# arpg/NID-Pose-Estimation

Hardware: NVIDIA B200
Metric: NID cost+Jacobian evals/s @640x480 (higher is better)
Workload: dtype f64

## Files before the change

### nid-pose-estimation_b200/csrc/nid_api.cu

```cuda
#include <math.h>
#include <stdio.h>
#include <string.h>

#include <algorithm>
#include <limits>
#include <string>
#include <chrono>
#include <vector>

#include "../host/nid_host_math.hpp"
#include "nid_ctx.h"

namespace nid {

static thread_local std::string g_err;
void set_error(const std::string& s) { g_err = s; }
int check_cuda(cudaError_t e, const char* what) {
  if (e == cudaSuccess) return NID_OK;
  g_err = std::string(what) + ": " + cudaGetErrorString(e);
  return NID_ERR_CUDA;
}

#define CU(call, what)                                   \
  do {                                                   \
    cudaError_t e_ = (call);                             \
    if (e_ != cudaSuccess) return check_cuda(e_, what);  \
  } while (0)
#define OKR(call)               \
  do {                          \
    int r_ = (call);            \
    if (r_ != NID_OK) return r_; \
  } while (0)

static int strips_for(const nid_ctx* c, int n_jobs) {
  int S;
  if (c->opt_force_strips > 0) S = std::min(c->opt_force_strips, c->rb);
  else {
    long long want = 2LL * c->sm_count;
    long long per = (long long)c->ncell * n_jobs;
    S = (int)((want + per - 1) / per);
    S = std::max(1, std::min(S, std::min(c->rb, 32)));
  }
  if (c->part_slots > 0 && n_jobs > 0) S = (int)std::max<size_t>(1, std::min<size_t>((size_t)S, c->part_slots / (size_t)n_jobs));
  return S;
}

EvalParams make_params(nid_ctx* c, int n_jobs) {
  EvalParams p;
  memset(&p, 0, sizeof(p));
  p.rows = c->rows; p.cols = c->cols; p.cell = c->cell; p.bins = c->bins;
  p.rb = c->rb; p.cb = c->cb; p.N = c->N; p.ncell = c->ncell;
  p.S = strips_for(c, n_jobs);
  p.strip_rows = (c->rb + p.S - 1) / p.S;
  p.hist_stride = c->bins * c->bins + c->bins;
  p.pwx = c->pwx; p.pwy = c->pwy; p.pwz = c->pwz;
  p.im0 = c->im0; p.im1 = c->im1; p.inb0 = c->inb0;
  p.n_c = c->n_c; p.href = c->href; p.cam = c->cam;
  p.lut_w = c->lut_w; p.lut_k = c->lut_k;
  p.poses = c->poses; p.job_pair = c->job_pair;
  const bool sorted = use_sorted(c);
  p.part = c->part; p.jpart = sorted ? c->jpart_s : c->jpart; p.hist = c->opt_keep_hist ? c->hist : nullptr;
  p.ht = c->ht; p.hj = c->hj; p.err = c->err; p.der = c->der; p.gn = c->gn;
  p.sd0 = c->sd0; p.sd1 = c->sd1; p.sd2 = c->sd2; p.sid = c->sid;
  p.stage_bulk = (c->opt_stage_bulk < 0 ? (long long)c->rb * c->cb < NID_SMALL_CELL_PX : c->opt_stage_bulk) ? 1 : 0;
  p.sl_off = c->sl_off; p.sl_task = c->sl_task; p.sl_desc = c->sl_desc; p.task_cls = c->task_cls; p.sl_cell = c->sl_cell; p.nslices = c->nslices;
  p.sell_cap = c->sell_cap; p.max_slices = c->max_slices; p.Twc0 = c->Twc0;
  p.tasks = c->tasks; p.ntasks = c->ntasks; p.cell_task_start = c->cell_task_start; p.cell_slice_start = c->cell_slice_start;
  p.cls_task_start = c->cls_task_start; p.span_start = c->span_start; p.wv = c->wv;
  p.max_tasks = c->max_tasks; p.g_stride = (int)c->g_stride;
  p.G = c->G; p.fp1 = c->fp1; p.tex2 = c->d_tex2; p.k1tex = c->d_k1tex;
  return p;
}

bool use_sorted(const nid_ctx* c) {
  if (c->bins > NID_SORTED_MAX_BINS || c->bins < NID_SORTED_MIN_BINS) return false;
  if (c->opt_path == 1) return false;
  return true;
}

template <typename T>
static int dalloc(T** p, size_t n, const char* what) {
  cudaError_t e = cudaMalloc((void**)p, sizeof(T) * (n ? n : 1));
  if (e != cudaSuccess) return check_cuda(e, what);
  return NID_OK;
}

int ensure_job_buffers(nid_ctx* c) {
  const size_t J = c->job_cap, NC = c->ncell;
  const size_t hs = (size_t)c->bins * c->bins + c->bins;
  if (c->opt_keep_hist && !c->hist) OKR(dalloc(&c->hist, J * NC * hs, "hist"));
  if (use_sorted(c)) {
    const size_t need = (size_t)std::max(c->max_ntasks_prepared, 1);
    if (c->g_stride < need) {
      CU(cudaStreamSynchronize(c->stream), "sync before growing job buffers");
      if (c->G) cudaFree(c->G);
      c->G = nullptr;
      OKR(dalloc(&c->G, J * need * c->bins, "G"));
      c->g_stride = need;
    }
    if (!c->jpart_s) OKR(dalloc(&c->jpart_s, J * (size_t)c->max_slices * 6, "jpart_s"));
    if (!c->wv) {
      OKR(dalloc(&c->wv, J * NC * (size_t)nid::wv_stride(c->bins), "wv"));
      CU(cudaMemset(c->wv, 0, sizeof(double) * J * NC * (size_t)nid::wv_stride(c->bins)), "memset wv");
    }
  } else if (!c->part) {
    c->part_slots = J + 2 * (size_t)c->sm_count + 64;
    OKR(dalloc(&c->part, c->part_slots * NC * hs, "part"));
    OKR(dalloc(&c->jpart, c->part_slots * NC * 6, "jpart"));
  }
  return NID_OK;
}

static int update_textures(nid_ctx* c, int pair0, int n) {
  for (int i = 0; i < n; i++) c->k1_ready[pair0 + i] = 0;
  for (int p0 = pair0; p0 < pair0 + n; p0 += c->setup_batch) {
    const int nb = std::min(c->setup_batch, pair0 + n - p0);
    OKR(launch_pack(c, p0, nb));
    for (int i = 0; i < nb; i++)
      CU(cudaMemcpy2DToArrayAsync(c->tex2_arrays[p0 + i], 0, 0, c->d_pack + (size_t)i * c->N, sizeof(unsigned) * c->cols,
                                  sizeof(unsigned) * c->cols, c->rows, cudaMemcpyDeviceToDevice, c->stream), "packed im1 -> texture array");
  }
  return NID_OK;
}
static int update_texture(nid_ctx* c, int pair) { return update_textures(c, pair, 1); }

static int arena_take(nid_ctx* c, size_t bytes, void** out) {
  bytes = (bytes + 63) & ~(size_t)63;
  if (bytes > c->h_arena_cap) {
    CU(cudaStreamSynchronize(c->stream), "sync before growing the staging arena");
    if (c->h_arena) cudaFreeHost(c->h_arena);
    c->h_arena = nullptr; c->h_arena_cap = 0; c->h_arena_used = 0;
    const size_t cap = std::max(bytes * 4, (size_t)1 << 20);
    CU(cudaMallocHost((void**)&c->h_arena, cap), "pinned staging arena");
    c->h_arena_cap = cap;
  }
  if (c->h_arena_used + bytes > c->h_arena_cap) {
    CU(cudaStreamSynchronize(c->stream), "sync to recycle the staging arena");
    c->h_arena_used = 0;
  }
  *out = c->h_arena + c->h_arena_used;
  c->h_arena_used += bytes;
  return NID_OK;
}

static int stage_jobs(nid_ctx* c, int n_jobs, const int* job_pair, const double* poses, int mode = 0) {
  if (n_jobs < 1 || n_jobs > c->max_jobs) { set_error("n_jobs out of range"); return NID_ERR_ARG; }
  for (int j = 0; j < n_jobs; j++) {
    int pr = job_pair ? job_pair[j] : 0;
    if (pr < 0 || pr >= c->n_pairs) { set_error("job_pair out of range"); return NID_ERR_ARG; }
    if (mode == 1) {
      if (!c->pair_set[pr]) { set_error("job_pair invalid or pair not set"); return NID_ERR_ARG; }
      continue;
    }
    if (!c->pair_prepared[pr]) { set_error("pair not prepared (call nid_prepare)"); return NID_ERR_STATE; }
    if (use_sorted(c) && !c->pair_sorted[pr]) {
      set_error("pair not prepared for the sorted path (call nid_prepare after selecting the path)");
      return NID_ERR_STATE;
    }
  }
  const int slot = (c->stage_slot + 1) % NID_STAGE_RING;
  CU(cudaEventSynchronize(c->stage_ev[slot]), "wait for the staging slot");
  c->stage_slot = slot;
  c->h_poses = c->h_poses_ring + (size_t)slot * 16 * c->job_cap;
  c->h_job_pair = c->h_job_pair_ring + (size_t)slot * c->job_cap;
  for (int j = 0; j < n_jobs; j++) c->h_job_pair[j] = job_pair ? job_pair[j] : 0;
  memcpy(c->h_poses, poses, sizeof(double) * 16 * n_jobs);
  CU(cudaMemcpyAsync(c->poses, c->h_poses, sizeof(double) * 16 * n_jobs, cudaMemcpyHostToDevice, c->stream), "H2D poses");
  CU(cudaMemcpyAsync(c->job_pair, c->h_job_pair, sizeof(int) * n_jobs, cudaMemcpyHostToDevice, c->stream), "H2D job_pair");
  CU(cudaEventRecord(c->stage_ev[slot], c->stream), "record staging event");
  c->staged_jobs = n_jobs;
  return NID_OK;
}

static int fetch(nid_ctx* c, int n_jobs, int want_jac, double* Ht, double* Hj, double* der) {
  const size_t nc = (size_t)n_jobs * c->ncell;
  double* h = c->h_out;
  if (Ht) CU(cudaMemcpyAsync(h, c->ht, sizeof(double) * nc, cudaMemcpyDeviceToHost, c->stream), "D2H ht");
  if (Hj) CU(cudaMemcpyAsync(h + nc, c->hj, sizeof(double) * nc, cudaMemcpyDeviceToHost, c->stream), "D2H hj");
  if (want_jac && der) CU(cudaMemcpyAsync(h + 2 * nc, c->der, sizeof(double) * 6 * nc, cudaMemcpyDeviceToHost, c->stream), "D2H der");
  CU(cudaStreamSynchronize(c->stream), "sync");
  if (Ht) memcpy(Ht, h, sizeof(double) * nc);
  if (Hj) memcpy(Hj, h + nc, sizeof(double) * nc);
  if (want_jac && der) memcpy(der, h + 2 * nc, sizeof(double) * 6 * nc);
  return NID_OK;
}

}

using namespace nid;

extern "C" {

const char* nid_last_error(void) { return g_err.c_str(); }
int nid_version(void) { return 100; }

int nid_create(nid_ctx** out, int device, int rows, int cols, int cell, int bins, int degree, int n_pairs, int max_jobs) {
  cudaGetLastError();
  if (!out) { set_error("ctx out pointer is NULL"); return NID_ERR_ARG; }
  *out = nullptr;
  if (degree != 3) { set_error("only bs_degree == 3 (order-4 B-splines) is supported, as in the reference"); return NID_ERR_UNSUPPORTED; }
  if (rows > 65535 || cols > 65535) { set_error("rows, cols must be < 65536"); return NID_ERR_ARG; }
  if (cell > 90) { set_error("cell must be <= 90 (the task descriptors keep the cell index in 13 bits)"); return NID_ERR_ARG; }
  if (rows < 8 || cols < 8 || cell < 1 || bins < 6 || bins > 64 || n_pairs < 1 || max_jobs < 1 || cell > rows || cell > cols) {
    set_error("bad geometry (need rows,cols>=8, 1<=cell<=min(rows,cols), 6<=bins<=64, n_pairs,max_jobs>=1)");
    return NID_ERR_ARG;
  }
  int ndev = 0;
  cudaError_t e = cudaGetDeviceCount(&ndev);
  if (e != cudaSuccess || ndev == 0) {
    set_error(std::string("no CUDA device: ") + cudaGetErrorString(e) + " (this library has no CPU path)");
    return NID_ERR_CUDA;
  }
  if (device < 0 || device >= ndev) { set_error("device index out of range"); return NID_ERR_ARG; }
  CU(cudaSetDevice(device), "cudaSetDevice");
  nid_ctx* c = new nid_ctx();
  c->device = device; c->rows = rows; c->cols = cols; c->cell = cell; c->bins = bins; c->degree = degree;
  c->N = rows * cols; c->ncell = cell * cell; c->rb = rows / cell; c->cb = cols / cell;
  c->n_pairs = n_pairs; c->max_jobs = max_jobs;
  c->job_cap = std::max(max_jobs, NID_MIN_JOB_SLOTS);
  cudaDeviceProp prop;
  CU(cudaGetDeviceProperties(&prop, device), "cudaGetDeviceProperties");
  c->sm_count = prop.multiProcessorCount;
  CU(cudaStreamCreateWithFlags(&c->stream, cudaStreamNonBlocking), "cudaStreamCreate");
  const size_t N = c->N, P = n_pairs, J = c->job_cap, NC = c->ncell;
  const size_t hs = (size_t)bins * bins + bins;
  OKR(dalloc(&c->pwx, P * N, "pwx")); OKR(dalloc(&c->pwy, P * N, "pwy")); OKR(dalloc(&c->pwz, P * N, "pwz"));
  OKR(dalloc(&c->im0, P * N, "im0")); OKR(dalloc(&c->im1, P * N, "im1")); OKR(dalloc(&c->inb0, P * N, "inb0"));
  OKR(dalloc(&c->n_c, P * NC, "n_c")); OKR(dalloc(&c->href, P * NC, "href"));
  OKR(dalloc(&c->cam, P * 4, "cam")); OKR(dalloc(&c->Twc0, P * 16, "Twc0"));
  OKR(dalloc(&c->cnt, P * NC * NID_NCLS, "cnt"));
  c->task_px = (long long)c->rb * c->cb < NID_SMALL_CELL_PX ? 16 : 32;
  const int min_task_px = 8;
  c->max_tasks = (int)(N / min_task_px + NC * NID_NCLS + 1);
  c->max_slices = c->max_tasks / 32 + (int)NC + 1;
  c->sell_cap = (N + 3 * (size_t)c->max_tasks + NC * 32 * (size_t)(NID_TASK_PX_MAX + 4) + 255) / 128 * 128;
  OKR(dalloc(&c->depth, P * N, "depth"));
  OKR(dalloc(&c->sl_off, P * ((size_t)c->max_slices + 1), "sl_off"));
  OKR(dalloc(&c->sl_task, P * (size_t)c->max_slices * 32, "sl_task"));
  OKR(dalloc(&c->sl_desc, P * (size_t)c->max_slices * 32, "sl_desc"));
  OKR(dalloc(&c->task_cls, P * (size_t)c->max_tasks, "task_cls"));
  OKR(dalloc(&c->sl_cell, P * (size_t)c->max_slices, "sl_cell"));
  OKR(dalloc(&c->task_pos, P * (size_t)c->max_tasks, "task_pos"));
  OKR(dalloc(&c->nslices, P, "nslices"));
  CU(cudaMemset(c->nslices, 0, sizeof(int) * P), "memset nslices");
  c->h_nslices.assign(P, 0);
  OKR(dalloc(&c->tasks, P * (size_t)c->max_tasks, "tasks"));
  OKR(dalloc(&c->ntasks, P, "ntasks"));
  CU(cudaMemset(c->ntasks, 0, sizeof(int) * P), "memset ntasks");
  OKR(dalloc(&c->cell_task_start, P * (NC + 1), "cell_task_start"));
  OKR(dalloc(&c->cell_slice_start, P * (NC + 1), "cell_slice_start"));
  OKR(dalloc(&c->cls_task_start, P * NC * (NID_NCLS + 1), "cls_task_start"));
  {
    const int NS = bins - 3;
    std::vector<int> ss(NS + 1, 256);
    auto kr = [bins](int v) { double o = v >= 255 ? 254.999 : (double)v; return (int)std::floor(o * (bins - 3) / 255.0); };
    for (int v = 255; v >= 0; v--)
      for (int k = 0; k <= kr(v) && k <= NS; k++) ss[k] = v;
    ss[NS] = 256;
    OKR(dalloc(&c->span_start, ss.size(), "span_start"));
    CU(cudaMemcpy(c->span_start, ss.data(), sizeof(int) * ss.size(), cudaMemcpyHostToDevice), "H2D span_start");
  }
  c->h_ntasks.assign(P, 0);
  {
    bool ok = true;
    c->tex2_arrays.assign(P, nullptr);
    c->h_tex2.assign(P, 0);
    cudaChannelFormatDesc cd2 = cudaCreateChannelDesc<unsigned int>();
    for (size_t i = 0; i < P && ok; i++) {
      if (cudaMallocArray(&c->tex2_arrays[i], &cd2, cols, rows, cudaArrayTextureGather) != cudaSuccess) { ok = false; break; }
      cudaResourceDesc rd;
      memset(&rd, 0, sizeof(rd));
      rd.resType = cudaResourceTypeArray;
      rd.res.array.array = c->tex2_arrays[i];
      cudaTextureDesc td;
      memset(&td, 0, sizeof(td));
      td.addressMode[0] = td.addressMode[1] = cudaAddressModeClamp;
      td.filterMode = cudaFilterModePoint;
      td.readMode = cudaReadModeElementType;
      td.normalizedCoords = 0;
      if (cudaCreateTextureObject(&c->h_tex2[i], &rd, &td, nullptr) != cudaSuccess) ok = false;
    }
    if (!ok) {
      cudaGetLastError();
      set_error("could not create the packed gather textures for the target images");
      return NID_ERR_CUDA;
    }
    OKR(dalloc(&c->d_tex2, P, "d_tex2"));
    OKR(dalloc(&c->d_k1tex, P, "d_k1tex"));
    CU(cudaMemset(c->d_k1tex, 0, sizeof(cudaTextureObject_t) * P), "memset k1tex");
    c->k1_arrays.assign(P, nullptr);
    c->h_k1tex.assign(P, 0);
    c->k1_ready.assign(P, 0);
    CU(cudaMemcpy(c->d_tex2, c->h_tex2.data(), sizeof(cudaTextureObject_t) * P, cudaMemcpyHostToDevice), "H2D tex2 handles");
    c->setup_batch = (int)std::min<size_t>(P, 32);
    OKR(dalloc(&c->d_pack, N * (size_t)c->setup_batch, "d_pack"));
    OKR(dalloc(&c->lay_tot, (size_t)c->setup_batch * NC * 3, "lay_tot"));
    OKR(dalloc(&c->lay_base, (size_t)c->setup_batch * NC * 3, "lay_base"));
    OKR(dalloc(&c->prep_poses, (size_t)c->setup_batch * 16, "prep_poses"));
    OKR(dalloc(&c->depth_factor, P, "depth_factor"));
    c->pair_u16.assign(P, 0);
    OKR(dalloc(&c->fp1, P * N, "fp1"));
    c->h_Twc0.assign(P * 16, 0.0);
    c->h_cam.assign(P * 4, 1.0);
  }
  OKR(dalloc(&c->d_depth, N, "d_depth")); OKR(dalloc(&c->d_img64, N, "d_img64")); OKR(dalloc(&c->d_flag, 2, "d_flag"));
  CU(cudaMemset(c->d_flag, 0, sizeof(int) * 2), "memset flag");
  OKR(dalloc(&c->lut_w, 256 * 4, "lut_w")); OKR(dalloc(&c->lut_k, 256, "lut_k"));
  OKR(dalloc(&c->poses, J * 16, "poses")); OKR(dalloc(&c->job_pair, J, "job_pair"));
  CU(cudaMemset(c->job_pair, 0, sizeof(int) * J), "memset job_pair");
  CU(cudaMemset(c->poses, 0, sizeof(double) * 16 * J), "memset poses");
  OKR(dalloc(&c->aux_pose, 16, "aux_pose"));
  (void)hs;
  OKR(dalloc(&c->ht, J * NC, "ht")); OKR(dalloc(&c->hj, J * NC, "hj")); OKR(dalloc(&c->err, J * NC, "err"));
  OKR(dalloc(&c->der, J * NC * 6, "der")); OKR(dalloc(&c->gn, J * 44, "gn"));
  OKR(dalloc(&c->hard, J * (NC + 1), "hard"));
  CU(cudaMallocHost((void**)&c->h_poses_ring, sizeof(double) * 16 * J * NID_STAGE_RING), "pinned poses");
  CU(cudaMallocHost((void**)&c->h_job_pair_ring, sizeof(int) * J * NID_STAGE_RING), "pinned job_pair");
  memset(c->h_poses_ring, 0, sizeof(double) * 16 * J * NID_STAGE_RING);
  memset(c->h_job_pair_ring, 0, sizeof(int) * J * NID_STAGE_RING);
  c->h_poses = c->h_poses_ring;
  c->h_job_pair = c->h_job_pair_ring;
  for (int i = 0; i < NID_STAGE_RING; i++) CU(cudaEventCreateWithFlags(&c->stage_ev[i], cudaEventDisableTiming), "cudaEventCreate (staging)");
  CU(cudaMallocHost((void**)&c->h_aux_pose, sizeof(double) * 16), "pinned aux pose");
  CU(cudaMallocHost((void**)&c->h_out, sizeof(double) * J * (NC * 8 + 44)), "pinned out");
  c->pair_set.assign(P, 0);
  c->pair_prepared.assign(P, 0);
  c->pair_sorted.assign(P, 0);
  OKR(launch_build_lut(c));
  OKR(sorted_init(c));
  CU(cudaStreamSynchronize(c->stream), "sync after lut");
  *out = c;
  return NID_OK;
}

int nid_destroy(nid_ctx* c) {
  if (!c) return NID_OK;
  cudaSetDevice(c->device);
  cudaStreamSynchronize(c->stream);
  void* ptrs[] = {c->pwx, c->pwy, c->pwz, c->im0, c->im1, c->inb0, c->n_c, c->href, c->cam, c->Twc0, c->cnt, c->d_depth,
                  c->d_img64, c->d_flag, c->d_pix, c->d_pix4, c->d_pix4_jobs, c->chunk_cnt, c->d_bsv, c->d_bsi, c->lut_w, c->lut_k, c->poses,
                  c->job_pair, c->aux_pose, c->part, c->jpart, c->hist, c->ht, c->hj, c->err, c->der, c->gn, c->hard,
                  c->depth, c->sd0, c->sd1, c->sd2, c->sid, c->sl_off, c->sl_task, c->sl_desc, c->task_cls, c->sl_cell, c->nslices, c->task_pos,
                  c->lay_tot, c->lay_base, c->prep_poses, c->depth16, c->depth_factor, c->d_tex2, c->d_pack, c->tasks, c->ntasks, c->cell_task_start, c->cell_slice_start, c->G, c->jpart_s, c->fp1, c->cls_task_start, c->span_start, c->wv};
  for (auto t : c->h_k1tex) if (t) cudaDestroyTextureObject(t);
  for (auto arr : c->k1_arrays) if (arr) cudaFreeArray(arr);
  if (c->d_k1tex) cudaFree(c->d_k1tex);
  if (c->d_k1pack) cudaFree(c->d_k1pack);
  for (auto t : c->h_tex2) if (t) cudaDestroyTextureObject(t);
  for (auto arr : c->tex2_arrays) if (arr) cudaFreeArray(arr);
  for (void* p : ptrs) if (p) cudaFree(p);
  if (c->h_poses_ring) cudaFreeHost(c->h_poses_ring);
  if (c->h_job_pair_ring) cudaFreeHost(c->h_job_pair_ring);
  if (c->h_aux_pose) cudaFreeHost(c->h_aux_pose);
  if (c->h_lm_lists) cudaFreeHost(c->h_lm_lists);
  destroy_latency_graph(c);
  if (c->h_lm_stage) cudaFreeHost(c->h_lm_stage);
  if (c->d_lm_stage) cudaFree(c->d_lm_stage);
  if (c->d_lm_lists) cudaFree(c->d_lm_lists);
  for (int i = 0; i < NID_STAGE_RING; i++) if (c->stage_ev[i]) cudaEventDestroy(c->stage_ev[i]);
  if (c->h_out) cudaFreeHost(c->h_out);
  if (c->h_arena) cudaFreeHost(c->h_arena);
  if (c->h_res) cudaFreeHost(c->h_res);
  for (int i = 0; i < 2; i++) if (c->ev[i]) cudaEventDestroy(c->ev[i]);
  for (int i = 0; i < 2; i++) if (c->ds_ev[i]) cudaEventDestroy(c->ds_ev[i]);
  for (int i = 0; i < 5; i++) if (c->kev[i]) cudaEventDestroy(c->kev[i]);
  cudaStreamDestroy(c->stream);
  if (c->stream2) cudaStreamDestroy(c->stream2);
  delete c;
  return NID_OK;
}

int nid_sync(nid_ctx* c) {
  if (!c) { set_error("NULL ctx"); return NID_ERR_ARG; }
  CU(cudaSetDevice(c->device), "cudaSetDevice");
  CU(cudaStreamSynchronize(c->stream), "nid_sync");
  c->h_arena_used = 0;
  return NID_OK;
}

static int set_pairs_geometry(nid_ctx* c, int pair0, int n, const double* depth64, const uint16_t* depth16, const double* T_wc0,
                              const double* intr) {
  if (pair0 < 0 || n < 1 || pair0 + n > c->n_pairs) { set_error("pair range out of bounds"); return NID_ERR_ARG; }
  if ((!depth64 && !depth16) || !T_wc0 || !intr) { set_error("NULL argument"); return NID_ERR_ARG; }
  CU(cudaSetDevice(c->device), "cudaSetDevice");
  const size_t N = c->N;
  if (depth16) {
    if (!c->depth16) OKR(dalloc(&c->depth16, (size_t)c->n_pairs * N, "depth16"));
    CU(cudaMemcpyAsync(c->depth16 + (size_t)pair0 * N, depth16, sizeof(uint16_t) * N * n, cudaMemcpyDefault, c->stream), "H2D depth (u16)");
  } else {
    CU(cudaMemcpyAsync(c->depth + (size_t)pair0 * N, depth64, sizeof(double) * N * n, cudaMemcpyDefault, c->stream), "H2D depth");
  }
  double* a = nullptr;
  OKR(arena_take(c, sizeof(double) * 21 * n, (void**)&a));
  double *aT = a, *acam = a + 16 * (size_t)n, *afac = a + 20 * (size_t)n;
  memcpy(aT, T_wc0, sizeof(double) * 16 * n);
  for (int i = 0; i < n; i++) {
    memcpy(acam + 4 * i, intr + 5 * (size_t)i, sizeof(double) * 4);
    afac[i] = intr[5 * (size_t)i + 4];
  }
  CU(cudaMemcpyAsync(c->Twc0 + 16 * (size_t)pair0, aT, sizeof(double) * 16 * n, cudaMemcpyHostToDevice, c->stream), "H2D Twc0");
  CU(cudaMemcpyAsync(c->cam + 4 * (size_t)pair0, acam, sizeof(double) * 4 * n, cudaMemcpyHostToDevice, c->stream), "H2D intr");
  CU(cudaMemcpyAsync(c->depth_factor + pair0, afac, sizeof(double) * n, cudaMemcpyHostToDevice, c->stream), "H2D depth factor");
  memcpy(c->h_Twc0.data() + 16 * (size_t)pair0, aT, sizeof(double) * 16 * n);
  memcpy(c->h_cam.data() + 4 * (size_t)pair0, acam, sizeof(double) * 4 * n);
  OKR(launch_points(c, pair0, n, depth16 != nullptr));
  for (int i = 0; i < n; i++) { c->pair_prepared[pair0 + i] = 0; c->pair_u16[pair0 + i] = depth16 ? 1 : 0; }
  return NID_OK;
}
static int set_pair_common(nid_ctx* c, int pair, const double* depth, const double T_wc0[16], const double intr[5]) {
  if (pair < 0 || pair >= c->n_pairs) { set_error("pair index out of range"); return NID_ERR_ARG; }
  return set_pairs_geometry(c, pair, 1, depth, nullptr, T_wc0, intr);
}

int nid_set_pair(nid_ctx* c, int pair, const double* depth, const uint8_t* im0, const uint8_t* im1, const double T_wc0[16],
                 const double intr[5]) {
  if (!c) { set_error("NULL ctx"); return NID_ERR_ARG; }
  if (!im0 || !im1) { set_error("NULL image"); return NID_ERR_ARG; }
  OKR(set_pair_common(c, pair, depth, T_wc0, intr));
  CU(cudaMemcpyAsync(c->im0 + (size_t)pair * c->N, im0, c->N, cudaMemcpyDefault, c->stream), "H2D im0");
  CU(cudaMemcpyAsync(c->im1 + (size_t)pair * c->N, im1, c->N, cudaMemcpyDefault, c->stream), "H2D im1");
  OKR(update_texture(c, pair));
  CU(cudaStreamSynchronize(c->stream), "sync set_pair");
  c->pair_set[pair] = 1;
  return NID_OK;
}

int nid_set_pairs_u16(nid_ctx* c, int pair0, int n, const uint16_t* depth_raw, const uint8_t* im0, const uint8_t* im1,
                      const double* T_wc0, const double* intr) {
  if (!c) { set_error("NULL ctx"); return NID_ERR_ARG; }
  if (!im0 || !im1 || !depth_raw) { set_error("NULL image"); return NID_ERR_ARG; }
  if (c->sell_points) { set_error("this context holds caller-supplied world points (nid_set_pair_points)"); return NID_ERR_STATE; }
  OKR(set_pairs_geometry(c, pair0, n, nullptr, depth_raw, T_wc0, intr));
  const size_t N = c->N;
  CU(cudaMemcpyAsync(c->im0 + (size_t)pair0 * N, im0, N * n, cudaMemcpyDefault, c->stream), "H2D im0");
  CU(cudaMemcpyAsync(c->im1 + (size_t)pair0 * N, im1, N * n, cudaMemcpyDefault, c->stream), "H2D im1");
  OKR(update_textures(c, pair0, n));
  for (int i = 0; i < n; i++) c->pair_set[pair0 + i] = 1;
  return NID_OK;
}

int nid_set_pairs_downsampled(nid_ctx* dst, int dst_pair0, const nid_ctx* src, int src_pair0, int n) {
  if (!dst || !src) { set_error("NULL context"); return NID_ERR_ARG; }
  if (dst->rows != src->rows / 2 || dst->cols != src->cols / 2) {
    set_error("destination geometry must be (source rows / 2, source cols / 2)");
    return NID_ERR_ARG;
  }
  if (n < 1 || n > dst->n_pairs || n > src->n_pairs || dst_pair0 < 0 || src_pair0 < 0 || dst_pair0 > dst->n_pairs - n ||
      src_pair0 > src->n_pairs - n) {
    set_error("pair range out of bounds");
    return NID_ERR_ARG;
  }
  if (dst->device != src->device) { set_error("source and destination contexts live on different devices"); return NID_ERR_ARG; }
  if (src->sell_points || dst->sell_points) {
    set_error("downsampling needs depth pairs on both sides, not caller-supplied world points (nid_set_pair_points)");
    return NID_ERR_STATE;
  }
  for (int i = 0; i < n; i++)
    if (!src->pair_set[src_pair0 + i]) { set_error("source pair not set"); return NID_ERR_STATE; }
  CU(cudaSetDevice(dst->device), "cudaSetDevice");
  for (int i = 0; i < 2; i++)
    if (!dst->ds_ev[i]) CU(cudaEventCreateWithFlags(&dst->ds_ev[i], cudaEventDisableTiming), "cudaEventCreate (downsample)");
  double* a = nullptr;
  OKR(arena_take(dst, sizeof(double) * 5 * n, (void**)&a));
  double *acam = a, *afac = a + 4 * (size_t)n;
  for (int i = 0; i < n; i++) {
    const double* k = src->h_cam.data() + 4 * (size_t)(src_pair0 + i);
    acam[4 * i] = k[0] * 0.5; acam[4 * i + 1] = k[1] * 0.5;
    acam[4 * i + 2] = (k[2] - 0.5) * 0.5; acam[4 * i + 3] = (k[3] - 0.5) * 0.5;
    afac[i] = 1.0;
  }
  CU(cudaEventRecord(dst->ds_ev[0], src->stream), "record source event");
  CU(cudaStreamWaitEvent(dst->stream, dst->ds_ev[0], 0), "wait for the source");
  CU(cudaMemcpyAsync(dst->cam + 4 * (size_t)dst_pair0, acam, sizeof(double) * 4 * n, cudaMemcpyHostToDevice, dst->stream), "H2D intr");
  CU(cudaMemcpyAsync(dst->depth_factor + dst_pair0, afac, sizeof(double) * n, cudaMemcpyHostToDevice, dst->stream), "H2D depth factor");
  CU(cudaMemcpyAsync(dst->Twc0 + 16 * (size_t)dst_pair0, src->Twc0 + 16 * (size_t)src_pair0, sizeof(double) * 16 * n,
                     cudaMemcpyDeviceToDevice, dst->stream), "D2D Twc0");
  memcpy(dst->h_cam.data() + 4 * (size_t)dst_pair0, acam, sizeof(double) * 4 * n);
  memcpy(dst->h_Twc0.data() + 16 * (size_t)dst_pair0, src->h_Twc0.data() + 16 * (size_t)src_pair0, sizeof(double) * 16 * n);
  OKR(launch_downsample2(dst, dst_pair0, src, src_pair0, n));
  OKR(launch_points(dst, dst_pair0, n, false));
  OKR(update_textures(dst, dst_pair0, n));
  CU(cudaEventRecord(dst->ds_ev[1], dst->stream), "record destination event");
  CU(cudaStreamWaitEvent(src->stream, dst->ds_ev[1], 0), "order the source after the kernel");
  for (int i = 0; i < n; i++) {
    dst->pair_set[dst_pair0 + i] = 1;
    dst->pair_prepared[dst_pair0 + i] = 0;
    dst->pair_u16[dst_pair0 + i] = 0;
  }
  return NID_OK;
}

int nid_set_target(nid_ctx* c, int pair, const uint8_t* im1) {
  if (!c || !im1) { set_error("bad argument"); return NID_ERR_ARG; }
  if (pair < 0 || pair >= c->n_pairs) { set_error("pair index out of range"); return NID_ERR_ARG; }
  if (!c->pair_set[pair]) { set_error("pair not set (nid_set_target replaces the target of an existing pair)"); return NID_ERR_STATE; }
  CU(cudaSetDevice(c->device), "cudaSetDevice");
  CU(cudaMemcpyAsync(c->im1 + (size_t)pair * c->N, im1, c->N, cudaMemcpyDefault, c->stream), "H2D im1");
  OKR(update_texture(c, pair));
  CU(cudaStreamSynchronize(c->stream), "sync set_target");
  c->pair_prepared[pair] = 0;
  return NID_OK;
}

static int upload_images_f64(nid_ctx* c, int pair, const double* im0, const double* im1);
static int build_sorted_layout(nid_ctx* c, int pair0, int n);
static int finish_sorted_layout(nid_ctx* c, int pair0, int n, int* bs_counter, double* Href);

int nid_set_pair_f64(nid_ctx* c, int pair, const double* depth, const double* im0, const double* im1,
                     const double T_wc0[16], const double intr[5]) {
  if (!c) { set_error("NULL ctx"); return NID_ERR_ARG; }
  OKR(set_pair_common(c, pair, depth, T_wc0, intr));
  OKR(upload_images_f64(c, pair, im0, im1));
  c->pair_set[pair] = 1;
  return NID_OK;
}

static int upload_images_f64(nid_ctx* c, int pair, const double* im0, const double* im1) {
  CU(cudaMemsetAsync(c->d_flag, 0, sizeof(int), c->stream), "memset flag");
  if (im0) {
    CU(cudaMemcpyAsync(c->d_img64, im0, sizeof(double) * c->N, cudaMemcpyDefault, c->stream), "H2D im0 f64");
    OKR(launch_check_integral(c, c->d_img64, c->im0 + (size_t)pair * c->N, 1));
  }
  if (im1) {
    CU(cudaMemcpyAsync(c->d_img64, im1, sizeof(double) * c->N, cudaMemcpyDefault, c->stream), "H2D im1 f64");
    OKR(launch_check_integral(c, c->d_img64, c->im1 + (size_t)pair * c->N, 0));
    OKR(update_texture(c, pair));
  }
  int flag = 0;
  CU(cudaMemcpyAsync(&flag, c->d_flag, sizeof(int), cudaMemcpyDeviceToHost, c->stream), "D2H flag");
  CU(cudaStreamSynchronize(c->stream), "sync upload images");
  if (flag) {
    set_error("image holds non-8-bit values (non-integral or outside [0,255]); only 8-bit gray is supported");
    return NID_ERR_UNSUPPORTED;
  }
  return NID_OK;
}

int nid_set_pair_points(nid_ctx* c, int pair, const double* points_3d, const double* im0, const double* im1,
                        const double intr[5]) {
  if (!c || pair < 0 || pair >= c->n_pairs) { set_error("bad argument"); return NID_ERR_ARG; }
  CU(cudaSetDevice(c->device), "cudaSetDevice");
  if (points_3d) {
    if (!intr) { set_error("intr required with points"); return NID_ERR_ARG; }
    if (!c->d_pix) OKR(dalloc(&c->d_pix, (size_t)8 * c->N, "d_pix"));
    CU(cudaMemcpyAsync(c->d_pix, points_3d, sizeof(double) * 3 * c->N, cudaMemcpyDefault, c->stream), "H2D points3d");
    CU(cudaMemcpyAsync(c->cam + 4 * pair, intr, sizeof(double) * 4, cudaMemcpyDefault, c->stream), "H2D intr");
    memcpy(c->h_cam.data() + 4 * (size_t)pair, intr, sizeof(double) * 4);
    OKR(launch_points_soa(c, pair, c->d_pix));
    c->pair_prepared[pair] = 0;
    if (!c->sell_points) {
      CU(cudaStreamSynchronize(c->stream), "sync before switching to the point form");
      c->sell_points = true;
      std::fill(c->pair_prepared.begin(), c->pair_prepared.end(), 0);
    }
  }
  OKR(upload_images_f64(c, pair, im0, im1));
  c->pair_set[pair] = 1;
  return NID_OK;
}

int nid_import_prepare(nid_ctx* c, int pair, const double* bs_value, const int* bs_counter, const double* Href) {
  if (!c || pair < 0 || pair >= c->n_pairs || !bs_value || !bs_counter || !Href) { set_error("bad argument"); return NID_ERR_ARG; }
  if (!c->pair_set[pair]) { set_error("pair not set"); return NID_ERR_STATE; }
  CU(cudaSetDevice(c->device), "cudaSetDevice");
  if (!c->d_bsv) { OKR(dalloc(&c->d_bsv, (size_t)4 * c->N, "d_bsv")); OKR(dalloc(&c->d_bsi, (size_t)c->N, "d_bsi")); }
  CU(cudaMemcpyAsync(c->d_bsv, bs_value, sizeof(double) * 4 * c->N, cudaMemcpyDefault, c->stream), "H2D bs_value");
  OKR(launch_import_flags(c, pair, c->d_bsv));
  CU(cudaMemcpyAsync(c->n_c + pair * c->ncell, bs_counter, sizeof(int) * c->ncell, cudaMemcpyDefault, c->stream), "H2D n_c");
  CU(cudaMemcpyAsync(c->href + pair * c->ncell, Href, sizeof(double) * c->ncell, cudaMemcpyDefault, c->stream), "H2D href");
  CU(cudaMemsetAsync(c->cnt + (size_t)pair * c->ncell * NID_NCLS, 0, sizeof(unsigned int) * c->ncell * NID_NCLS, c->stream), "memset cnt");
  OKR(launch_count_classes(c, pair));
  OKR(build_sorted_layout(c, pair, 1));
  OKR(finish_sorted_layout(c, pair, 1, nullptr, nullptr));
  c->pair_prepared[pair] = 1;
  return NID_OK;
}

int nid_get_inbounds(nid_ctx* c, int pair, uint8_t* flags) {
  if (!c || pair < 0 || pair >= c->n_pairs || !flags) { set_error("bad argument"); return NID_ERR_ARG; }
  if (!c->pair_prepared[pair]) { set_error("pair not prepared"); return NID_ERR_STATE; }
  CU(cudaSetDevice(c->device), "cudaSetDevice");
  CU(cudaMemcpyAsync(flags, c->inb0 + (size_t)pair * c->N, c->N, cudaMemcpyDefault, c->stream), "D2H inb0");
  CU(cudaStreamSynchronize(c->stream), "sync inb0");
  return NID_OK;
}

int nid_get_points3d(nid_ctx* c, int pair, double* points_3d) {
  if (!c || pair < 0 || pair >= c->n_pairs || !points_3d) { set_error("bad argument"); return NID_ERR_ARG; }
  if (!c->pair_set[pair]) { set_error("pair not set"); return NID_ERR_STATE; }
  CU(cudaSetDevice(c->device), "cudaSetDevice");
  if (!c->d_pix) OKR(dalloc(&c->d_pix, (size_t)8 * c->N, "d_pix"));
  OKR(launch_points_aos(c, pair, c->d_pix));
  CU(cudaMemcpyAsync(points_3d, c->d_pix, sizeof(double) * 3 * c->N, cudaMemcpyDefault, c->stream), "copy points3d");
  CU(cudaStreamSynchronize(c->stream), "sync points3d");
  return NID_OK;
}

static int build_sorted_layout(nid_ctx* c, int pair0, int n) {
  for (int i = 0; i < n; i++) c->pair_sorted[pair0 + i] = 0;
  if (!use_sorted(c)) return NID_OK;
  if (!c->sd0) {
    OKR(dalloc(&c->sd0, (size_t)c->n_pairs * c->sell_cap, "sd0"));
    OKR(dalloc(&c->sid, (size_t)c->n_pairs * c->sell_cap, "sid"));
  }
  if (c->sell_points && !c->sd1) {
    OKR(dalloc(&c->sd1, (size_t)c->n_pairs * c->sell_cap, "sd1"));
    OKR(dalloc(&c->sd2, (size_t)c->n_pairs * c->sell_cap, "sd2"));
  }
  if (!c->chunk_cnt) {
    const size_t nchunks = ((size_t)c->rb * c->cb + 255) / 256;
    OKR(dalloc(&c->chunk_cnt, (size_t)c->setup_batch * c->ncell * nchunks * NID_NCLS, "chunk_cnt"));
  }
  for (int p0 = pair0; p0 < pair0 + n; p0 += c->setup_batch)
    OKR(launch_layout_and_scatter(c, p0, std::min(c->setup_batch, pair0 + n - p0)));
  return NID_OK;
}

static int finish_sorted_layout(nid_ctx* c, int pair0, int n, int* bs_counter, double* Href) {
  const size_t NC = c->ncell;
  const size_t bytes = (size_t)n * (NC * (sizeof(double) + sizeof(int)) + 2 * sizeof(int)) + sizeof(int) + 64;
  if (c->h_res_cap < bytes) {
    CU(cudaStreamSynchronize(c->stream), "sync before growing the result buffer");
    if (c->h_res) cudaFreeHost(c->h_res);
    c->h_res = nullptr; c->h_res_cap = 0;
    CU(cudaMallocHost((void**)&c->h_res, bytes * 2), "pinned prepare results");
    c->h_res_cap = bytes * 2;
  }
  double* h_href = (double*)c->h_res;
  int* h_nc = (int*)(h_href + (size_t)n * NC);
  int* h_nt = h_nc + (size_t)n * NC;
  int* h_ns = h_nt + n;
  int* h_ovf = h_ns + n;
  CU(cudaMemcpyAsync(h_nc, c->n_c + (size_t)pair0 * NC, sizeof(int) * NC * n, cudaMemcpyDeviceToHost, c->stream), "D2H n_c");
  CU(cudaMemcpyAsync(h_href, c->href + (size_t)pair0 * NC, sizeof(double) * NC * n, cudaMemcpyDeviceToHost, c->stream), "D2H href");
  const bool sorted = use_sorted(c);
  if (sorted) {
    CU(cudaMemcpyAsync(h_nt, c->ntasks + pair0, sizeof(int) * n, cudaMemcpyDeviceToHost, c->stream), "D2H ntasks");
    CU(cudaMemcpyAsync(h_ns, c->nslices + pair0, sizeof(int) * n, cudaMemcpyDeviceToHost, c->stream), "D2H nslices");
    CU(cudaMemcpyAsync(h_ovf, c->d_flag + 1, sizeof(int), cudaMemcpyDeviceToHost, c->stream), "D2H overflow flag");
  }
  CU(cudaStreamSynchronize(c->stream), "sync prepare");
  c->h_arena_used = 0;
  if (sorted) {
    if (*h_ovf) { set_error("sliced pixel store overflow"); return NID_ERR_STATE; }
    for (int i = 0; i < n; i++) {
      c->h_ntasks[pair0 + i] = h_nt[i];
// ... 624 lines not shown
```

### nid-pose-estimation_b200/csrc/nid_ctx.h

```cpp
#pragma once
#include <cuda_runtime.h>
#include <stdint.h>
#include <string>
#include <vector>

#include "../../include/nid_b200.h"

#define NID_NCLS 257
#define NID_SORTED_MIN_BINS 6
#define NID_SORTED_MAX_BINS 40
#define NID_STAGE_RING 4
#define NID_MIN_JOB_SLOTS 8
#define NID_TASK_PX_MAX 256

namespace nid {

struct EvalParams {
  int rows, cols, cell, bins, rb, cb, N, ncell;
  int job0;
  const int* job_list;
  int S;
  int strip_rows;
  int hist_stride;
  const double* pwx;
  const double* pwy;
  const double* pwz;
  const uint8_t* im0;
  const uint8_t* im1;
  const uint8_t* inb0;
  const int* n_c;
  const double* href;
  const double* cam;
  const double* lut_w;
  const int* lut_k;
  const double* poses;
  const int* job_pair;
  double* part;
  double* jpart;
  double* hist;
  double* ht;
  double* hj;
  double* err;
  double* der;
  double* gn;
  double huber_delta;
  double huber_dsqr;
  const double* sd0;
  const double* sd1;
  const double* sd2;
  const unsigned* sid;
  int stage_bulk;
  const int* sl_off;
  const int* sl_task;
  const int* sl_desc;
  const unsigned short* task_cls;
  const int* sl_cell;
  const int* nslices;
  size_t sell_cap;
  int max_slices;
  const double* Twc0;
  const int2* tasks;
  const int* ntasks;
  const int* cell_task_start;
  const int* cell_slice_start;
  const int* cls_task_start;
  const int* span_start;
  double* wv;
  int max_tasks;
  int g_stride;
  double* G;
  const unsigned* fp1;
  const cudaTextureObject_t* tex2;
  const cudaTextureObject_t* k1tex;
};

}

namespace nid { struct LatencyGraph; }
struct nid_ctx {
  int device = 0;
  int rows = 0, cols = 0, cell = 0, bins = 0, degree = 3;
  int N = 0, ncell = 0, rb = 0, cb = 0;
  int n_pairs = 0, max_jobs = 0;
  int job_cap = 0;
  int sm_count = 148;
  cudaStream_t stream = nullptr;
  int* chunk_cnt = nullptr;
  int setup_batch = 1;
  int* lay_tot = nullptr;
  int* lay_base = nullptr;
  double* prep_poses = nullptr;
  uint16_t* depth16 = nullptr;
  double* depth_factor = nullptr;
  std::vector<char> pair_u16;
  char* h_arena = nullptr;
  size_t h_arena_cap = 0, h_arena_used = 0;
  char* h_res = nullptr;
  size_t h_res_cap = 0;
  cudaStream_t stream2 = nullptr;
  long long launches = 0;

  double *pwx = nullptr, *pwy = nullptr, *pwz = nullptr;
  uint8_t *im0 = nullptr, *im1 = nullptr, *inb0 = nullptr;
  int* n_c = nullptr;
  double* href = nullptr;
  double* cam = nullptr;
  double* Twc0 = nullptr;
  unsigned int* cnt = nullptr;
  double* depth = nullptr;
  double *sd0 = nullptr, *sd1 = nullptr, *sd2 = nullptr;
  unsigned* sid = nullptr;
  size_t sell_cap = 0;
  int* sl_desc = nullptr;
  unsigned short* task_cls = nullptr;
  int *sl_off = nullptr, *sl_task = nullptr, *sl_cell = nullptr, *nslices = nullptr, *task_pos = nullptr;
  int max_slices = 0;
  std::vector<int> h_nslices;
  int max_nslices_prepared = 0;
  int task_px = 32;
  bool sell_points = false;
  int2* tasks = nullptr;
  int* ntasks = nullptr;
  int* cell_task_start = nullptr;
  int* cell_slice_start = nullptr;
  int* cls_task_start = nullptr;
  int* span_start = nullptr;
  double* wv = nullptr;
  int max_tasks = 0;
  std::vector<int> h_ntasks;
  int max_ntasks_prepared = 0;
  double *G = nullptr, *jpart_s = nullptr;
  std::vector<cudaArray_t> tex2_arrays;
  std::vector<cudaTextureObject_t> h_tex2;
  cudaTextureObject_t* d_tex2 = nullptr;
  std::vector<cudaArray_t> k1_arrays;
  std::vector<cudaTextureObject_t> h_k1tex;
  cudaTextureObject_t* d_k1tex = nullptr;
  std::vector<char> k1_ready;
  unsigned short* d_k1pack = nullptr;
  unsigned* fp1 = nullptr;
  std::vector<double> h_Twc0, h_cam;
  unsigned* d_pack = nullptr;
  size_t g_stride = 0;
  int opt_path = 0;
  int opt_keep_hist = 0;
  std::vector<char> pair_set, pair_prepared, pair_sorted;
  double* d_depth = nullptr;
  double* d_img64 = nullptr;
  int* d_flag = nullptr;
  double* d_pix = nullptr;
  float* d_pix4 = nullptr;
  float* d_pix4_jobs = nullptr;
  double* d_bsv = nullptr;
  int* d_bsi = nullptr;
  double* lut_w = nullptr;
  int* lut_k = nullptr;
  double* poses = nullptr;
  int* job_pair = nullptr;
  double *part = nullptr, *jpart = nullptr, *hist = nullptr;
  double *ht = nullptr, *hj = nullptr, *err = nullptr, *der = nullptr, *gn = nullptr;
  double* hard = nullptr;
  size_t part_slots = 0;
  double* h_poses = nullptr;
  int* h_job_pair = nullptr;
  double* h_poses_ring = nullptr;
  int* h_job_pair_ring = nullptr;
  cudaEvent_t stage_ev[NID_STAGE_RING] = {};
  int stage_slot = 0;
  int staged_jobs = 0;
  double* h_aux_pose = nullptr;
  double* aux_pose = nullptr;
  double* h_out = nullptr;
  int opt_force_strips = 0;
  int* h_lm_lists = nullptr;
  int* d_lm_lists = nullptr;
  void* h_lm_stage = nullptr;
  void* d_lm_stage = nullptr;
  nid::LatencyGraph* lm_graph = nullptr;
  const void* last_hist_func = nullptr;
  const void* last_jac_func = nullptr;
  int opt_lm_graph = 1;
  int opt_stage_bulk = -1;
  int opt_asm_wide = 1;
  int opt_lm_spec = 4;
  int opt_lm_reuse = 1;
  double* lm_trace = nullptr;
  int lm_trace_cap = 0;
  cudaEvent_t ev[2] = {nullptr, nullptr};
  cudaEvent_t ds_ev[2] = {nullptr, nullptr};
  int opt_time_kernels = 0;
  cudaEvent_t kev[5] = {nullptr, nullptr, nullptr, nullptr, nullptr};
  double kernel_ms[4] = {0, 0, 0, 0};
  long long kernel_calls[4] = {0, 0, 0, 0};
};

namespace nid {
#define NID_FEW_BINS(bins) ((bins) <= 20)
#ifndef NID_SMALL_CELL_PX
#define NID_SMALL_CELL_PX 2560
#endif
__host__ __device__ inline int wv_row(int B) { return NID_FEW_BINS(B) ? B + 1 : B; }
__host__ __device__ inline int wv_stride(int B) { return (B * wv_row(B) + B + 1) & ~1; }
__host__ __device__ inline int job_at(const EvalParams& p, int i) { return p.job_list ? p.job_list[p.job0 + i] : p.job0 + i; }
#ifdef __CUDACC__
__device__ __forceinline__ void huber_weights(double ec, double dsqr, double delta, double& rho0, double& rho1) {
  const double chi = ec * ec;
  if (chi <= dsqr) { rho0 = chi; rho1 = 1.0; }
  else { const double sq = sqrt(chi); rho0 = 2 * sq * delta - dsqr; rho1 = delta / sq; }
}
__device__ __forceinline__ void gn_accumulate(double& acc, const double* e, const double* r0, const double* r1, const double* act,
                                              const double* J, int n, int ent) {
  if (ent == 0) {
    for (int c = 0; c < n; c++) acc += r0[c];
  } else if (ent <= 36) {
    const int i = (ent - 1) / 6, j = (ent - 1) % 6;
    for (int c = 0; c < n; c++) acc += J[6 * c + i] * r1[c] * J[6 * c + j];
  } else if (ent <= 42) {
    const int i = ent - 37;
    for (int c = 0; c < n; c++) acc -= r1[c] * J[6 * c + i] * e[c];
  } else {
    for (int c = 0; c < n; c++) acc += act[c];
  }
}
#define NID_GN_CHUNK 256
__device__ __forceinline__ void gn_block(const EvalParams& p, int job, int want_jac, double* __restrict__ out) {
  __shared__ double s_e[NID_GN_CHUNK], s_r0[NID_GN_CHUNK], s_r1[NID_GN_CHUNK], s_act[NID_GN_CHUNK];
  __shared__ double s_J[6 * NID_GN_CHUNK];
  const double* e = p.err + (size_t)job * p.ncell;
  const double* J = p.der + (size_t)job * p.ncell * 6;
  const int t = threadIdx.x;
  const int ent = t < 36 ? t + 1 : (t >= 64 && t < 70) ? t - 64 + 37 : t == 96 ? 0 : t == 97 ? 43 : -1;
  const bool mine = ent >= 0 && (want_jac || ent == 0 || ent == 43);
  double acc = 0.0;
  for (int c0 = 0; c0 < p.ncell; c0 += NID_GN_CHUNK) {
    const int n = min(NID_GN_CHUNK, p.ncell - c0);
    for (int i = threadIdx.x; i < n; i += blockDim.x) {
      const double ec = e[c0 + i];
      const bool active = !isnan(ec);
      double rho0 = 0.0, rho1 = 0.0;
      if (active) huber_weights(ec, p.huber_dsqr, p.huber_delta, rho0, rho1);
      s_e[i] = active ? ec : 0.0; s_r0[i] = rho0; s_r1[i] = rho1; s_act[i] = active ? 1.0 : 0.0;
    }
    if (want_jac)
      for (int i = threadIdx.x; i < 6 * n; i += blockDim.x) {
        const double v = J[6 * c0 + i];
        s_J[i] = isnan(e[c0 + i / 6]) ? 0.0 : v;
      }
    __syncthreads();
    if (mine) gn_accumulate(acc, s_e, s_r0, s_r1, s_act, s_J, n, ent);
    __syncthreads();
  }
  if (mine) out[job * 44 + ent] = acc;
}
#endif
void set_error(const std::string& s);
int check_cuda(cudaError_t e, const char* what);
EvalParams make_params(nid_ctx* c, int n_jobs);

inline void ktime_mark(nid_ctx* c, int i) {
  if (!c->opt_time_kernels) return;
  if (!c->kev[i]) cudaEventCreate(&c->kev[i]);
  cudaEventRecord(c->kev[i], c->stream);
}
inline void ktime_collect(nid_ctx* c, int n, const int* slot) {
  if (!c->opt_time_kernels) return;
  cudaEventSynchronize(c->kev[n]);
  for (int i = 0; i < n; i++) {
    if (slot[i] < 0) continue;
    float ms = 0.f;
    cudaEventElapsedTime(&ms, c->kev[i], c->kev[i + 1]);
    c->kernel_ms[slot[i]] += ms;
    c->kernel_calls[slot[i]]++;
  }
}
bool use_sorted(const nid_ctx* c);
int ensure_job_buffers(nid_ctx* c);

struct JobSet { const int* d_list; const int* h_list; int first, n; int slots; };
enum class Pass2 { none, some, all };
int launch_pass1(nid_ctx* c, const JobSet& js, Pass2 p2);
int launch_pass2(nid_ctx* c, const JobSet& js);
int launch_gn(nid_ctx* c, const JobSet& js, double delta, int want_jac);

int sorted_init(nid_ctx* c);
int launch_count_classes(nid_ctx* c, int pair);
int launch_layout_and_scatter(nid_ctx* c, int pair0, int n);
int launch_pack(nid_ctx* c, int pair0, int n);
int launch_pack_k1(nid_ctx* c, int pair, unsigned short* d_out);
int launch_sorted_tail_gn(nid_ctx* c, const int* d_list, const int* h_list, int first, int n, double delta, double* gn_out);
int launch_latency_round(nid_ctx* c, int nslots, const int* d_list, const int* h_list, size_t h2d_bytes, double delta, double* gn_out);
void destroy_latency_graph(nid_ctx* c);
int launch_href(nid_ctx* c, int pair0, int n);

int launch_build_lut(nid_ctx* c);
int launch_points(nid_ctx* c, int pair0, int n, bool u16);
int launch_downsample2(nid_ctx* dst, int dst_pair0, const nid_ctx* src, int src_pair0, int n);
int launch_prepare(nid_ctx* c, int pair0, int n, const double* d_poses16);
int launch_ref_weights(nid_ctx* c, int pair);
int launch_points_aos(nid_ctx* c, int pair, double* d_out);
int launch_hard(nid_ctx* c, int n_jobs);
int launch_warp_sample(nid_ctx* c, int pair, const double* d_pose16, int f64);
int launch_warp_sample_jobs(nid_ctx* c, int n_jobs, float4* d_out, bool u16);
int launch_check_integral(nid_ctx* c, const double* d_src, uint8_t* d_dst, int is_ref);
int launch_points_soa(nid_ctx* c, int pair, const double* d_in);
int launch_import_flags(nid_ctx* c, int pair, const double* d_bsv);
}
```

### nid-pose-estimation_b200/csrc/nid_sorted.cu

```cuda
#include <cuda_fp16.h>
#include <math.h>
#include <stdlib.h>

#include <algorithm>
#include <vector>

#include "nid_ctx.h"
#include "nid_device.cuh"

namespace nid {

#define NID_LAUNCH_CHECK(c, what)                         \
  do {                                                    \
    (c)->launches++;                                      \
    cudaError_t e__ = cudaGetLastError();                 \
    if (e__ != cudaSuccess) return check_cuda(e__, what); \
  } while (0)

#define NID_PAD_ID 0xFFFFFFFFu
#define NID_BLK_JOB blockIdx.x
#define NID_BLK_CHUNK blockIdx.y
#define NID_GRID(jobs, chunks) dim3(jobs, chunks)
#ifndef NID_PREFETCH_L2
#define NID_PREFETCH_L2 2
#endif

__global__ void k_count_classes(EvalParams p, int pair, unsigned int* __restrict__ cnt) {
  const size_t base = (size_t)pair * p.N;
  for (int i = blockIdx.x * blockDim.x + threadIdx.x; i < p.N; i += gridDim.x * blockDim.x) {
    int row = i / p.cols, col = i % p.cols;
    if (isnan(p.pwx[base + i]) || row >= p.rb * p.cell || col >= p.cb * p.cell) continue;
    int c = (row / p.rb) * p.cell + (col / p.cb);
    int key = p.inb0[base + i] ? (int)p.im0[base + i] : 256;
    atomicAdd(&cnt[((size_t)pair * p.ncell + c) * NID_NCLS + key], 1u);
  }
}

__device__ __forceinline__ int sell_key(const EvalParams& p, size_t base, int c, int t, int& row, int& col) {
  const int npx = p.rb * p.cb;
  if (t >= npx) return -1;
  row = (c / p.cell) * p.rb + t / p.cb;
  col = (c % p.cell) * p.cb + t % p.cb;
  const size_t i = base + (size_t)row * p.cols + col;
  if (isnan(p.pwx[i])) return -1;
  return p.inb0[i] ? (int)p.im0[i] : 256;
}

__global__ void __launch_bounds__(256) k_chunk_count(EvalParams p, int pair0, int* __restrict__ chunk_cnt_all) {
  __shared__ int s_cnt[NID_NCLS];
  const int chunk = blockIdx.x, c = blockIdx.y, pair = pair0 + blockIdx.z;
  int* chunk_cnt = chunk_cnt_all + (size_t)blockIdx.z * p.ncell * gridDim.x * NID_NCLS;
  for (int k = threadIdx.x; k < NID_NCLS; k += blockDim.x) s_cnt[k] = 0;
  __syncthreads();
  int row, col;
  const int key = sell_key(p, (size_t)pair * p.N, c, chunk * 256 + threadIdx.x, row, col);
  if (key >= 0) atomicAdd(&s_cnt[key], 1);
  __syncthreads();
  int* out = chunk_cnt + ((size_t)c * gridDim.x + chunk) * NID_NCLS;
  for (int k = threadIdx.x; k < NID_NCLS; k += blockDim.x) out[k] = s_cnt[k];
}

__global__ void __launch_bounds__(256) k_chunk_scan(int ncell, int nchunks, int* __restrict__ chunk_cnt_all) {
  const int i = blockIdx.x * blockDim.x + threadIdx.x;
  if (i >= ncell * NID_NCLS) return;
  int* chunk_cnt = chunk_cnt_all + (size_t)blockIdx.y * ncell * nchunks * NID_NCLS;
  const int c = i / NID_NCLS, k = i - c * NID_NCLS;
  int* q = chunk_cnt + (size_t)c * nchunks * NID_NCLS + k;
  int run = 0, j = 0;
  for (; j + 16 <= nchunks; j += 16) {
    int v[16];
#pragma unroll
    for (int u = 0; u < 16; u++) v[u] = q[(size_t)(j + u) * NID_NCLS];
#pragma unroll
    for (int u = 0; u < 16; u++) { q[(size_t)(j + u) * NID_NCLS] = run; run += v[u]; }
  }
  for (; j < nchunks; j++) { const int v = q[(size_t)j * NID_NCLS]; q[(size_t)j * NID_NCLS] = run; run += v; }
}

template <bool PTS>
__global__ void __launch_bounds__(256) k_scatter_sell(EvalParams p, int pair0, int L, const double* __restrict__ depth_all,
                                                      const int* __restrict__ task_pos_all, const int* __restrict__ chunk_off_all,
                                                      double* __restrict__ sd0, double* __restrict__ sd1,
                                                      double* __restrict__ sd2, unsigned* __restrict__ sid) {
  __shared__ int run[NID_NCLS];
  __shared__ int s_cts[NID_NCLS + 1];
  const int chunk = blockIdx.x, c = blockIdx.y, pair = pair0 + blockIdx.z;
  const double* depth = depth_all + (size_t)pair * p.N;
  const int* task_pos = task_pos_all + (size_t)pair * p.max_tasks;
  const int* chunk_off = chunk_off_all + (size_t)blockIdx.z * p.ncell * gridDim.x * NID_NCLS;
  if (p.n_c[pair * p.ncell + c] < NID_MIN_CELL_POINTS) return;
  const size_t base = (size_t)pair * p.N;
  const int* cts = p.cls_task_start + ((size_t)pair * p.ncell + c) * (NID_NCLS + 1);
  const int* off = chunk_off + ((size_t)c * gridDim.x + chunk) * NID_NCLS;
  for (int k = threadIdx.x; k < NID_NCLS; k += blockDim.x) run[k] = off[k];
  for (int k = threadIdx.x; k <= NID_NCLS; k += blockDim.x) s_cts[k] = cts[k];
  __syncthreads();
  const int lane = threadIdx.x & 31, warp = threadIdx.x >> 5;
  const size_t sbase = (size_t)pair * p.sell_cap;
  int row = 0, col = 0;
  const int key = sell_key(p, base, c, chunk * 256 + threadIdx.x, row, col);
  const unsigned mask = __match_any_sync(0xffffffffu, key);
  const int leader = __ffs(mask) - 1;
  const int rank = __popc(mask & ((1u << lane) - 1u));
  const int cnt = __popc(mask);
  int pos = 0;
  for (int w = 0; w < (int)(blockDim.x >> 5); w++) {
    if (warp == w && lane == leader && key >= 0) {
      pos = run[key];
      run[key] = pos + cnt;
    }
    __syncthreads();
  }
  pos = __shfl_sync(0xffffffffu, pos, leader) + rank;
  if (key >= 0) {
    const size_t i = base + (size_t)row * p.cols + col;
    const int task = s_cts[key] + pos / L, o = pos % L;
    const size_t dst = sbase + (size_t)task_pos[task] + (size_t)(o >> 2) * 128 + (o & 3);
    if (PTS) { sd0[dst] = p.pwx[i]; sd1[dst] = p.pwy[i]; sd2[dst] = p.pwz[i]; }
    else sd0[dst] = depth[(size_t)row * p.cols + col];
    sid[dst] = ((unsigned)row << 16) | (unsigned)col;
  }
}


#define NID_LAYOUT_THREADS 288
struct CellLayoutSm {
  int ts[NID_NCLS + 1];
  int fs[NID_NCLS + 1];
  int nf[NID_NCLS];
  int r[NID_NCLS];
  int prank[NID_NCLS];
  int sorted_r[NID_NCLS];
  int tail_off[NID_NCLS / 32 + 4];
  int wsum[2][NID_LAYOUT_THREADS / 32];
  int T, F, S, SF, slots;
};

__device__ __forceinline__ void cell_layout(const unsigned* __restrict__ cnt, int L, CellLayoutSm& s) {
  const int v = threadIdx.x, lane = v & 31, w = v >> 5;
  constexpr int NW = NID_LAYOUT_THREADS / 32;
  const int c = v < NID_NCLS ? (int)cnt[v] : 0;
  {
    int n = v < 256 ? c : 0;
#pragma unroll
    for (int o = 16; o > 0; o >>= 1) n += __shfl_xor_sync(0xffffffffu, n, o);
    if (lane == 0) s.wsum[0][w] = n;
  }
  __syncthreads();
  int n_c = 0;
#pragma unroll
  for (int i = 0; i < NW; i++) n_c += s.wsum[0][i];
  __syncthreads();
  const int cc = n_c >= NID_MIN_CELL_POINTS ? c : 0;
  const int nf = cc / L, r = cc - nf * L, nt = nf + (r > 0 ? 1 : 0);
  int a = nt, b = nf;
#pragma unroll
  for (int o = 1; o < 32; o <<= 1) {
    const int x = __shfl_up_sync(0xffffffffu, a, o), y = __shfl_up_sync(0xffffffffu, b, o);
    if (lane >= o) { a += x; b += y; }
  }
  if (lane == 31) { s.wsum[0][w] = a; s.wsum[1][w] = b; }
  __syncthreads();
  int oa = 0, ob = 0;
  for (int i = 0; i < w; i++) { oa += s.wsum[0][i]; ob += s.wsum[1][i]; }
  if (v < NID_NCLS) {
    s.ts[v] = oa + a - nt; s.fs[v] = ob + b - nf;
    s.nf[v] = nf; s.r[v] = r;
    if (v == NID_NCLS - 1) { s.ts[NID_NCLS] = oa + a; s.fs[NID_NCLS] = ob + b; }
  }
  __syncthreads();
  if (v < NID_NCLS && r > 0) {
    int g = 0;
    for (int q = 0; q < NID_NCLS; q++) {
      const int rq = s.r[q];
      g += (rq > r || (rq == r && q < v)) ? 1 : 0;
    }
    s.prank[v] = g;
    s.sorted_r[g] = r;
  }
  __syncthreads();
  if (v == 0) {
    const int T = s.ts[NID_NCLS], F = s.fs[NID_NCLS];
    const int S = (T + 31) >> 5, SF = (F + 31) >> 5;
    int off = SF * 32 * L;
    s.tail_off[0] = off;
    for (int j = 0; SF + j < S; j++) {
      off += ((s.sorted_r[32 * (SF + j) - F] + 3) >> 2) * 128;
      s.tail_off[j + 1] = off;
    }
    s.T = T; s.F = F; s.S = S; s.SF = SF; s.slots = off;
  }
  __syncthreads();
}

__global__ void __launch_bounds__(NID_LAYOUT_THREADS) k_layout_totals(int pair0, int ncell, int L, const unsigned* __restrict__ cnt,
                                                                      int* __restrict__ tot) {
  __shared__ CellLayoutSm s;
  const int c = blockIdx.x, pair = pair0 + blockIdx.y;
  cell_layout(cnt + ((size_t)pair * ncell + c) * NID_NCLS, L, s);
  if (threadIdx.x == 0) {
    int* o = tot + ((size_t)blockIdx.y * ncell + c) * 3;
    o[0] = s.T; o[1] = s.S; o[2] = s.slots;
  }
}

__global__ void __launch_bounds__(256) k_layout_scan(EvalParams p, int pair0, const int* __restrict__ tot, int* __restrict__ base,
                                                     int* __restrict__ cell_task_start, int* __restrict__ cell_slice_start,
                                                     int* __restrict__ ntasks, int* __restrict__ nslices, int* __restrict__ sl_off,
                                                     int* __restrict__ overflow) {
  __shared__ int wsum[3][8];
  __shared__ int carry[3];
  const int pair = pair0 + blockIdx.x, lane = threadIdx.x & 31, w = threadIdx.x >> 5;
  const int* t = tot + (size_t)blockIdx.x * p.ncell * 3;
  int* bs = base + (size_t)blockIdx.x * p.ncell * 3;
  if (threadIdx.x < 3) carry[threadIdx.x] = 0;
  __syncthreads();
  for (int c0 = 0; c0 < p.ncell; c0 += 256) {
    const int c = c0 + threadIdx.x;
    int x[3], a[3];
#pragma unroll
    for (int k = 0; k < 3; k++) { x[k] = c < p.ncell ? t[3 * c + k] : 0; a[k] = x[k]; }
#pragma unroll
    for (int o = 1; o < 32; o <<= 1)
#pragma unroll
      for (int k = 0; k < 3; k++) {
        const int y = __shfl_up_sync(0xffffffffu, a[k], o);
        if (lane >= o) a[k] += y;
      }
    if (lane == 31)
#pragma unroll
      for (int k = 0; k < 3; k++) wsum[k][w] = a[k];
    __syncthreads();
#pragma unroll
    for (int k = 0; k < 3; k++) {
      int o = carry[k];
      for (int i = 0; i < w; i++) o += wsum[k][i];
      a[k] += o - x[k];
    }
    if (c < p.ncell) {
      bs[3 * c] = a[0]; bs[3 * c + 1] = a[1]; bs[3 * c + 2] = a[2];
      cell_task_start[(size_t)pair * (p.ncell + 1) + c] = a[0];
      cell_slice_start[(size_t)pair * (p.ncell + 1) + c] = a[1];
    }
    __syncthreads();
    if (threadIdx.x == 255)
#pragma unroll
      for (int k = 0; k < 3; k++) carry[k] = a[k] + x[k];
    __syncthreads();
  }
  if (threadIdx.x == 0) {
    const int nt = carry[0], ns = carry[1], slots = carry[2];
    cell_task_start[(size_t)pair * (p.ncell + 1) + p.ncell] = nt;
    cell_slice_start[(size_t)pair * (p.ncell + 1) + p.ncell] = ns;
    ntasks[pair] = nt;
    nslices[pair] = ns;
    sl_off[(size_t)pair * (p.max_slices + 1) + min(ns, p.max_slices)] = slots;
    if (nt > p.max_tasks || ns > p.max_slices || (size_t)slots > p.sell_cap) atomicExch(overflow, 1);
  }
}

__global__ void __launch_bounds__(NID_LAYOUT_THREADS) k_layout_write(EvalParams p, int pair0, int L, const unsigned* __restrict__ cnt,
                                                                     const int* __restrict__ base, int2* __restrict__ tasks,
                                                                     int* __restrict__ task_pos, int* __restrict__ sl_task,
                                                                     int* __restrict__ sl_off, int* __restrict__ sl_cell,
                                                                     int* __restrict__ cls_task_start) {
  __shared__ CellLayoutSm s;
  const int c = blockIdx.x, pair = pair0 + blockIdx.y;
  cell_layout(cnt + ((size_t)pair * p.ncell + c) * NID_NCLS, L, s);
  const int* bs = base + ((size_t)blockIdx.y * p.ncell + c) * 3;
  const int tb = bs[0], sb = bs[1], pb = bs[2];
  if (tb + s.T > p.max_tasks || sb + s.S > p.max_slices) return;
  for (int v = threadIdx.x; v <= NID_NCLS; v += blockDim.x)
    cls_task_start[((size_t)pair * p.ncell + c) * (NID_NCLS + 1) + v] = tb + s.ts[v];
  int2* tk = tasks + (size_t)pair * p.max_tasks + tb;
  int* tp = task_pos + (size_t)pair * p.max_tasks + tb;
  int* st = sl_task + ((size_t)pair * p.max_slices + sb) * 32;
  int* sd = const_cast<int*>(p.sl_desc) + ((size_t)pair * p.max_slices + sb) * 32;
  unsigned short* tc = const_cast<unsigned short*>(p.task_cls) + (size_t)pair * p.max_tasks + tb;
  for (int t = threadIdx.x; t < s.T; t += blockDim.x) {
    int lo = 0, hi = NID_NCLS;
    while (hi - lo > 1) {
      const int mid = (lo + hi) >> 1;
      if (s.ts[mid] <= t) lo = mid; else hi = mid;
    }
    const int v = lo, i = t - s.ts[v];
    const bool full = i < s.nf[v];
    const int len = full ? L : s.r[v];
    const int rank = full ? s.fs[v] + i : s.F + s.prank[v];
    const int slice = rank >> 5, ln = rank & 31;
    const int off = slice < s.SF ? slice * 32 * L : s.tail_off[slice - s.SF];
    tk[t] = make_int2(i * L, len | (v << 9) | (c << 18));
    tp[t] = pb + off + 4 * ln;
    st[rank] = tb + t;
    sd[rank] = len | (v << 9) | (c << 18);
    tc[t] = (unsigned short)v;
  }
  for (int q = s.T + threadIdx.x; q < s.S * 32; q += blockDim.x) { st[q] = -1; sd[q] = 0; }
  for (int sl = threadIdx.x; sl < s.S; sl += blockDim.x) {
    sl_off[(size_t)pair * (p.max_slices + 1) + sb + sl] = pb + (sl < s.SF ? sl * 32 * L : s.tail_off[sl - s.SF]);
    sl_cell[(size_t)pair * p.max_slices + sb + sl] = c;
  }
}

__global__ void k_pack_tex(int rows, int cols, int pair0, const uint8_t* __restrict__ im_all, unsigned* __restrict__ out_all) {
  const int N = rows * cols;
  const uint8_t* im = im_all + (size_t)(pair0 + blockIdx.y) * N;
  unsigned* out = out_all + (size_t)blockIdx.y * N;
  for (int i = blockIdx.x * blockDim.x + threadIdx.x; i < N; i += gridDim.x * blockDim.x) {
    const int y = i / cols, x = i % cols;
    const int xm = max(x - 1, 0), xp = min(x + 1, cols - 1), ym = max(y - 1, 0), yp = min(y + 1, rows - 1);
    const int I = im[i];
    const int gx = (int)im[y * cols + xp] - (int)im[y * cols + xm];
    const int gy = (int)im[yp * cols + x] - (int)im[ym * cols + x];
    out[i] = (unsigned)I | ((unsigned)(gx + 256) << 8) | ((unsigned)(gy + 256) << 17);
  }
}

__global__ void k_pack_fp(int rows, int cols, int pair0, const uint8_t* __restrict__ im_all, unsigned* __restrict__ out_all) {
  const int N = rows * cols;
  const uint8_t* im = im_all + (size_t)(pair0 + blockIdx.y) * N;
  unsigned* out = out_all + (size_t)(pair0 + blockIdx.y) * N;
  for (int i = blockIdx.x * blockDim.x + threadIdx.x; i < N; i += gridDim.x * blockDim.x) {
    const int y = i / cols, x = i % cols;
    const int xp = min(x + 1, cols - 1), yp = min(y + 1, rows - 1);
    out[i] = (unsigned)im[y * cols + x] | ((unsigned)im[y * cols + xp] << 8) | ((unsigned)im[yp * cols + x] << 16) |
             ((unsigned)im[yp * cols + xp] << 24);
  }
}

#define NID_GEO_STRIDE 20
template <int NG>
struct GeoTable {
  double g[NG][NID_GEO_STRIDE];
  unsigned long long tex[NG];
  int job[NG], pair[NG], nsl[NG];
};

template <bool PTS>
__device__ __noinline__ void exact_uv(const double* __restrict__ T1g, const double* __restrict__ T0g,
                                      const double* __restrict__ camg, double a0, double a1, double a2, unsigned id,
                                      double* out5) {
  const Cam cam{camg[0], camg[1], camg[2], camg[3]};
  double xw = a0, yw = a1, zw = a2;
  if (!PTS) backproject(T0g, cam, a0, (int)(id >> 16), (int)(id & 0xffffu), xw, yw, zw);
  const Pose P = load_pose(T1g);
  double x1, y1, z1, u, v;
  warp_project(P, cam, xw, yw, zw, x1, y1, z1, u, v);
  out5[0] = x1; out5[1] = y1; out5[2] = z1; out5[3] = u; out5[4] = v;
}

struct Px {
  double xn, yn, rz;
  double dx, dy;
  int ix, iy;
  bool ok;
  bool jac;
  bool exact;
  bool fix;
};

__device__ __forceinline__ bool frac_is_safe(double d) {
  return (unsigned)(__double2hiint(d) - 0x3E700000) < (unsigned)(0x3FEFFFFF - 0x3E700000);
}

__device__ __forceinline__ void px_from_exact(const double* e, int rows, int cols, Px& r) {
  r.rz = 1.0 / e[2];
  r.xn = e[0] * r.rz; r.yn = e[1] * r.rz;
  const double u = e[3], v = e[4];
  r.ok = inb_cost(u, v, rows, cols);
  r.jac = inb_jac(u, v, rows, cols);
  r.ix = 0; r.iy = 0; r.dx = 0.0; r.dy = 0.0;
  if (r.ok) {
    r.ix = (int)u; r.iy = (int)v;
    r.dx = u - (double)r.ix; r.dy = v - (double)r.iy;
  }
  r.exact = true;
  r.fix = false;
}

template <bool PTS, bool P1>
__device__ __forceinline__ void front(const double* __restrict__ g, int rows, int cols, double a0, double a1, double a2,
                                      unsigned id, Px& r) {
  double x1, y1, z1;
  if (PTS) {
    x1 = fma(g[0], a0, fma(g[3], a1, fma(g[6], a2, g[9])));
    y1 = fma(g[1], a0, fma(g[4], a1, fma(g[7], a2, g[10])));
    z1 = fma(g[2], a0, fma(g[5], a1, fma(g[8], a2, g[11])));
  } else {
    const double cxn = fma(u2d(id & 0xffffu), g[12], g[13]);
    const double cyn = fma(u2d(id >> 16), g[14], g[15]);
    const double d0 = fma(g[0], cxn, fma(g[3], cyn, g[6]));
    const double d1 = fma(g[1], cxn, fma(g[4], cyn, g[7]));
    const double d2 = fma(g[2], cxn, fma(g[5], cyn, g[8]));
    x1 = fma(a0, d0, g[9]);
    y1 = fma(a0, d1, g[10]);
    z1 = fma(a0, d2, g[11]);
  }
  double y;
  asm("rcp.approx.ftz.f64 %0, %1;" : "=d"(y) : "d"(z1));
  double e = fma(-z1, y, 1.0);
  y = fma(y, e, y);
  e = fma(-z1, y, 1.0);
  y = fma(y, e, y);
  double u, v;
  if (P1) {
    u = fma(x1, y, g[18]);
    v = fma(y1, y, g[19]);
  } else {
    r.xn = x1 * y; r.yn = y1 * y; r.rz = y;
    u = fma(g[16], r.xn, g[18]);
    v = fma(g[17], r.yn, g[19]);
  }
  r.exact = false;
  const int ix = __double2int_rz(u), iy = __double2int_rz(v);
  const double dx = u - u2d((unsigned)ix), dy = v - u2d((unsigned)iy);
  const bool inr = id != NID_PAD_ID && (unsigned)ix <= (unsigned)(cols - 3) && (unsigned)iy <= (unsigned)(rows - 3);
  const bool safe = frac_is_safe(dx) && frac_is_safe(dy);
  r.ok = inr && safe && ix <= cols - 4 && iy <= rows - 4;
  r.jac = r.ok && ix <= cols - 5;
  r.fix = inr && !safe;
  const bool keep = P1 ? r.ok : r.jac;
  r.ix = keep ? ix : 0; r.iy = keep ? iy : 0;
  r.dx = dx; r.dy = dy;
}

__device__ __forceinline__ double bilinear_ref(double dx, double dy, unsigned p00, unsigned p01, unsigned p10, unsigned p11) {
  const double dxdy = __dmul_rn(dx, dy);
  const double w00 = __dadd_rn(__dsub_rn(__dsub_rn(1.0, dx), dy), dxdy);
  double a = __dmul_rn(dxdy, u2d(p11));
  a = __dadd_rn(a, __dmul_rn(__dsub_rn(dy, dxdy), u2d(p10)));
  a = __dadd_rn(a, __dmul_rn(__dsub_rn(dx, dxdy), u2d(p01)));
  return __dadd_rn(a, __dmul_rn(w00, u2d(p00)));
}

__device__ __forceinline__ double bilinear_fast(double dx, double dy, double p00, double d0, double p10, double d1) {
  const double a = fma(dx, d0, p00), b = fma(dx, d1, p10);
  return fma(dy, b - a, a);
}

__device__ __forceinline__ uint4 gather_u32(cudaTextureObject_t tex, int ix, int iy) {
  return tex2Dgather<uint4>(tex, (float)(ix + 1), (float)(iy + 1), 0);
}

__device__ __forceinline__ void bspline4_uniform(double f, double w[4]) {
  const double s6 = 1.0 / 6.0, h = 0.5;
  w[0] = fma(f, fma(f, fma(f, -s6, h), -h), s6);
  w[1] = fma(f * f, fma(f, h, -1.0), 2.0 / 3.0);
  w[2] = fma(f, fma(f, fma(f, -h, h), h), s6);
  w[3] = f * f * f * s6;
}
__device__ __forceinline__ void fold_row(double* h, int stride, int B, double n0) {
  const double u0 = h[0], u1 = h[stride], u2 = h[2 * stride];
  h[0] = fma(6.0, u0, n0);
  h[stride] = fma(1.5, u1, -6.0 * u0);
  h[2 * stride] = (u0 - 0.5 * u1) + u2;
  const double t1 = h[(B - 1) * stride], t2 = h[(B - 2) * stride], t3 = h[(B - 3) * stride];
  h[(B - 1) * stride] = 6.0 * t1;
  h[(B - 2) * stride] = fma(1.5, t2, -6.0 * t1);
  h[(B - 3) * stride] = (t1 - 0.5 * t2) + t3;
}
__device__ __forceinline__ void fold_table(double* w, int stride, int B) {
  const double w0 = w[0], w1 = w[stride], w2 = w[2 * stride];
  w[0] = fma(6.0, w0 - w1, w2);
  w[stride] = fma(1.5, w1, -0.5 * w2);
  const double v1 = w[(B - 1) * stride], v2 = w[(B - 2) * stride], v3 = w[(B - 3) * stride];
  w[(B - 1) * stride] = fma(6.0, v1 - v2, v3);
  w[(B - 2) * stride] = fma(1.5, v2, -0.5 * v3);
}

template <bool PTS>
struct Group {
  unsigned id[4];
  double a0[4], a1[4], a2[4];
  __device__ __forceinline__ void load(const double* q0, const double* q1, const double* q2, const unsigned* qi, size_t o) {
    const uint4 i4 = __ldcs(reinterpret_cast<const uint4*>(qi + o));
    id[0] = i4.x; id[1] = i4.y; id[2] = i4.z; id[3] = i4.w;
    const double2 xa = __ldcs(reinterpret_cast<const double2*>(q0 + o)), xb = __ldcs(reinterpret_cast<const double2*>(q0 + o + 2));
    a0[0] = xa.x; a0[1] = xa.y; a0[2] = xb.x; a0[3] = xb.y;
    if (PTS) {
      const double2 ya = __ldcs(reinterpret_cast<const double2*>(q1 + o)), yb = __ldcs(reinterpret_cast<const double2*>(q1 + o + 2));
      const double2 za = __ldcs(reinterpret_cast<const double2*>(q2 + o)), zb = __ldcs(reinterpret_cast<const double2*>(q2 + o + 2));
      a1[0] = ya.x; a1[1] = ya.y; a1[2] = yb.x; a1[3] = yb.y;
      a2[0] = za.x; a2[1] = za.y; a2[2] = zb.x; a2[3] = zb.y;
    } else {
#pragma unroll
      for (int j = 0; j < 4; j++) { a1[j] = 0.0; a2[j] = 0.0; }
    }
  }
};

__device__ __forceinline__ unsigned smem_u32(const void* ptr) { return (unsigned)__cvta_generic_to_shared(ptr); }
__device__ __forceinline__ void mbar_init(unsigned long long* bar, int count) {
  asm volatile("mbarrier.init.shared::cta.b64 [%0], %1;" ::"r"(smem_u32(bar)), "r"(count) : "memory");
}
__device__ __forceinline__ void mbar_expect_tx(unsigned long long* bar, unsigned bytes) {
  asm volatile("mbarrier.arrive.expect_tx.shared::cta.b64 _, [%0], %1;" ::"r"(smem_u32(bar)), "r"(bytes) : "memory");
}
__device__ __forceinline__ void bulk_g2s(void* dst, const void* src, unsigned bytes, unsigned long long* bar) {
  asm volatile("cp.async.bulk.shared::cluster.global.mbarrier::complete_tx::bytes [%0], [%1], %2, [%3];"
               ::"r"(smem_u32(dst)), "l"(src), "r"(bytes), "r"(smem_u32(bar)) : "memory");
}
__device__ __forceinline__ void mbar_wait(unsigned long long* bar, unsigned parity) {
  asm volatile(
      "{\n"
      ".reg .pred P1;\n"
      "LAB_WAIT:\n"
      "mbarrier.try_wait.parity.shared::cta.b64 P1, [%0], %1;\n"
      "@P1 bra DONE;\n"
      "bra LAB_WAIT;\n"
      "DONE:\n"
      "}" ::"r"(smem_u32(bar)), "r"(parity) : "memory");
}

struct ExactSrc {
  const double* T1;
  const double* T0;
  const double* cam;
};

struct GroupAddr {
  const double *q0, *q1, *q2;
  const unsigned* qi;
};

template <bool PTS>
__device__ __forceinline__ void make_exact(const ExactSrc& xs, int rows, int cols, const GroupAddr& ga, int j, Px& r) {
  double ex[5];
  const double a0 = ga.q0[j], a1 = PTS ? ga.q1[j] : 0.0, a2 = PTS ? ga.q2[j] : 0.0;
  const unsigned id = ga.qi[j];
  exact_uv<PTS>(xs.T1, xs.T0, xs.cam, a0, a1, a2, id, ex);
  px_from_exact(ex, rows, cols, r);
}

template <bool PTS, int W, int T>
__device__ __forceinline__ void hist_pixels(const double* __restrict__ g, const ExactSrc& xs, int rows, int cols,
                                            const Group<PTS>& G, int j0, const GroupAddr& ga,
                                            const unsigned* __restrict__ fp, double s, int NS, double* __restrict__ h,
                                            int& n0) {
  Px r[W];
  bool anyexact = false;
#pragma unroll
  for (int j = 0; j < W; j++) {
    front<PTS, true>(g, rows, cols, G.a0[j0 + j], G.a1[j0 + j], G.a2[j0 + j], G.id[j0 + j], r[j]);
    anyexact |= r[j].fix;
  }
  if (anyexact) {
#pragma unroll
    for (int j = 0; j < W; j++)
      if (r[j].fix) make_exact<PTS>(xs, rows, cols, ga, j0 + j, r[j]);
  }
  unsigned t[W];
#pragma unroll
  for (int j = 0; j < W; j++) t[j] = __ldg(fp + (unsigned)(r[j].iy * cols + r[j].ix));
  bool sat = false;
#pragma unroll
  for (int j = 0; j < W; j++) sat |= t[j] == 0xffffffffu;
  if (sat) {
#pragma unroll
    for (int j = 0; j < W; j++)
      if (r[j].ok && !r[j].exact && t[j] == 0xffffffffu) {
        anyexact = true;
        make_exact<PTS>(xs, rows, cols, ga, j0 + j, r[j]);
        t[j] = __ldg(fp + (unsigned)(r[j].iy * cols + r[j].ix));
      }
  }
  double ic[W];
#pragma unroll
  for (int j = 0; j < W; j++) {
    const int p00 = t[j] & 0xffu, p01 = (t[j] >> 8) & 0xffu, p10 = (t[j] >> 16) & 0xffu, p11 = t[j] >> 24;
    ic[j] = bilinear_fast(r[j].dx, r[j].dy, u2d(p00), i2d_small(p01 - p00), u2d(p10), i2d_small(p11 - p10));
  }
  if (anyexact) {
#pragma unroll
    for (int j = 0; j < W; j++)
      if (r[j].exact) {
        const unsigned p00 = t[j] & 0xffu, p01 = (t[j] >> 8) & 0xffu, p10 = (t[j] >> 16) & 0xffu, p11 = t[j] >> 24;
        ic[j] = clamp_intensity(bilinear_ref(r[j].dx, r[j].dy, p00, p01, p10, p11));
      }
  }
  double wt[W][4];
  int kt[W];
  bool acc[W];
#pragma unroll
  for (int j = 0; j < W; j++) {
    const double ub = ic[j] * s;
    kt[j] = min((int)ub, NS - 1);
    bspline4_uniform(ub - u2d((unsigned)kt[j]), wt[j]);
    const bool zero = ub == 0.0;
    acc[j] = r[j].ok && !zero;
    n0 += (r[j].ok && zero) ? 1 : 0;
  }
#pragma unroll
  for (int j = 0; j < W; j++) {
    if (!acc[j]) continue;
    double* hk = h + kt[j] * T;
#pragma unroll
    for (int n = 0; n < 4; n++) hk[n * T] += wt[j][n];
  }
}

template <int T>
__device__ __forceinline__ void store_task_rows(double* hw, int B, int lane, int task, double* __restrict__ Gj, size_t gstride) {
  for (int b0 = 0; b0 < B; b0 += 8) {
    double v[8];
#pragma unroll
    for (int i = 0; i < 8; i++) v[i] = (b0 + i < B) ? hw[(b0 + i) * T + lane] : 0.0;
    __syncwarp();
#pragma unroll
    for (int i = 0; i < 8; i++)
      if (b0 + i < B) hw[(b0 + i) * T + ((lane + b0 + i) & 31)] = v[i];
  }
  __syncwarp();
  const int BP2 = B <= 8 ? 8 : (B <= 16 ? 16 : 32);
  const int rpi = 32 / BP2;
  const int b = lane & (BP2 - 1), sub = lane / BP2;
  {
    const double* src = hw + min(b, B - 1) * T;
    double* dst = Gj + b;
    const int nit = 32 / rpi;
    for (int i0 = 0; i0 < nit; i0 += 8) {
      double v[8];
      int tk[8];
#pragma unroll
      for (int i = 0; i < 8; i++) {
        const int tl = (i0 + i) * rpi + sub;
        tk[i] = __shfl_sync(0xffffffffu, task, tl);
        v[i] = src[(tl + b) & 31];
      }
#pragma unroll
      for (int i = 0; i < 8; i++)
        if (b < B && tk[i] >= 0) dst[(size_t)tk[i] * gstride] = v[i];
    }
  }
  for (int b1 = BP2; b1 < B; b1 += BP2) {
    for (int t0 = 0; t0 < 32; t0 += rpi) {
      const int tl = t0 + sub, bb = b1 + b;
      const int tk = __shfl_sync(0xffffffffu, task, tl);
      if (bb < B && tk >= 0) Gj[(size_t)tk * gstride + bb] = hw[bb * T + ((tl + bb) & 31)];
    }
  }
  __syncwarp();
}

#ifndef NID_HIST_W
#define NID_HIST_W 4
#endif
#ifndef NID_JAC_W
#define NID_JAC_W 2
#endif
#ifndef NID_HIST_TMAX
#define NID_HIST_TMAX 32
#endif
#ifndef NID_JAC_TMAX
#define NID_JAC_TMAX 64
#endif
#ifndef NID_HIST_MINB
#define NID_HIST_MINB 2
#endif
#ifndef NID_JAC_MINB
#define NID_JAC_MINB 4
#endif
#ifndef NID_HIST_WARPS
#define NID_HIST_WARPS 18
#endif
#ifndef NID_JAC_WARPS
#define NID_JAC_WARPS (NID_JAC_MINB * 4)
#endif
#ifndef NID_JAC_REGS_SMALL
#define NID_JAC_REGS_SMALL 96
#endif
#define NID_JAC_WARPS_SMALL (2048 / NID_JAC_REGS_SMALL)
template <bool PTS, int NG, int T>
__global__ void __launch_bounds__(T, NID_HIST_WARPS * 32 / T)
k_hist_sell(const __grid_constant__ EvalParams p, const __grid_constant__ GeoTable<NG> gt) {
  extern __shared__ __align__(16) double sm[];
  const int B = p.bins, NS = B - 3;
  const int lane = threadIdx.x & 31, warp = threadIdx.x >> 5;
  const int job = job_at(p, NID_BLK_JOB);
  const int pair = p.job_pair[job];
  const double* g = gt.g[NID_BLK_JOB];
  const int slice = NID_BLK_CHUNK * (T >> 5) + warp;
  if (slice >= p.nslices[pair]) return;
  const int* so = p.sl_off + (size_t)pair * (p.max_slices + 1) + slice;
  const int off0 = so[0], ngroups = (so[1] - off0) >> 7;
  const int task = p.sl_task[((size_t)pair * p.max_slices + slice) * 32 + lane];
  double* h = sm + threadIdx.x;
  for (int b = 0; b < B; b++) h[b * T] = 0.0;
  const size_t sbase = (size_t)pair * p.sell_cap + off0 + lane * 4;
  const double* q0 = p.sd0 + sbase;
  const double* q1 = PTS ? p.sd1 + sbase : nullptr;
  const double* q2 = PTS ? p.sd2 + sbase : nullptr;
  const unsigned* qi = p.sid + sbase;
  const unsigned* fp = p.fp1 + (size_t)pair * p.N;
  const ExactSrc xs{p.poses + 16 * job, p.Twc0 + 16 * pair, p.cam + 4 * pair};
  const double s = (double)NS / 255.0;
  int n0 = 0;
  Group<PTS> G;
  G.load(q0, q1, q2, qi, 0);
  for (int gi = 0; gi < ngroups; gi++) {
    Group<PTS> Gn = G;
    if (gi + 1 < ngroups) Gn.load(q0, q1, q2, qi, (size_t)(gi + 1) * 128);
#if NID_PREFETCH_L2 > 0
    if (gi + 1 + NID_PREFETCH_L2 < ngroups) {
      const size_t po = (size_t)(gi + 1 + NID_PREFETCH_L2) * 128;
      asm volatile("prefetch.global.L2 [%0];" ::"l"(q0 + po));
      asm volatile("prefetch.global.L2 [%0];" ::"l"(qi + po));
    }
#endif
    const size_t go = (size_t)gi * 128;
    const GroupAddr ga{q0 + go, PTS ? q1 + go : nullptr, PTS ? q2 + go : nullptr, qi + go};
#pragma unroll
    for (int j0 = 0; j0 < 4; j0 += NID_HIST_W) hist_pixels<PTS, NID_HIST_W, T>(g, xs, p.rows, p.cols, G, j0, ga, fp, s, NS, h, n0);
    G = Gn;
  }
  fold_row(h, T, B, (double)n0);
  __syncwarp();
  store_task_rows<T>(sm + (threadIdx.x & ~31), B, lane, task, p.G + (size_t)job * p.g_stride * B, B);
}

#ifndef NID_ASM_THREADS
#define NID_ASM_THREADS 256
#endif
#define NID_ASM_SMALL 128
#ifndef NID_ASM_BATCH
#define NID_ASM_BATCH 12
#endif
#ifndef NID_ASM_CHUNK
#define NID_ASM_CHUNK 16
#endif
#ifndef NID_ASM_MINB
#define NID_ASM_MINB 4
#endif
template <int NT>
__device__ __forceinline__ void assemble_body(const EvalParams& p, int want_jac) {
  extern __shared__ __align__(16) double sm[];
  __shared__ double scratch[8];
  __shared__ int s_cts[NID_NCLS + 1];
  __shared__ int s_bnd[NT / 3 + 2];
  __shared__ int s_span[NID_SORTED_MAX_BINS];
  const int B = p.bins, BB = B * B, NS = B - 3;
  double* Pall = sm;
  double* red = sm + BB + B;
  double* hvs = red + NT;
  double* part = hvs + NID_NCLS * B;
  double* wl = part + 4 * BB;
  const int c = blockIdx.x, job = job_at(p, blockIdx.y);
  const int pair = p.job_pair[job];
  const int nc = p.n_c[pair * p.ncell + c];
  const size_t o = (size_t)job * p.ncell + c;
  if (nc < NID_MIN_CELL_POINTS) {
    if (threadIdx.x == 0) { p.ht[o] = nan(""); p.hj[o] = nan(""); p.err[o] = nan(""); }
    return;
  }
  {
    const int* cts = p.cls_task_start + ((size_t)pair * p.ncell + c) * (NID_NCLS + 1);
    for (int i = threadIdx.x; i <= NID_NCLS; i += blockDim.x) s_cts[i] = cts[i];
    for (int i = threadIdx.x; i <= NS; i += blockDim.x) s_span[i] = p.span_start[i];
    if (NID_FEW_BINS(B)) for (int i = threadIdx.x; i < 1024; i += blockDim.x) wl[i] = p.lut_w[i];
    __syncthreads();
    const bool pairs = (B & 1) == 0;
    const int tpr = pairs ? B >> 1 : B;
    const int ng = NT / tpr;
    const int tfirst = s_cts[0], tlast = s_cts[NID_NCLS], ntask = tlast - tfirst;
    if ((int)threadIdx.x <= ng) {
      int bnd = tlast;
      if ((int)threadIdx.x < ng) {
        const int target = tfirst + (int)(((long long)threadIdx.x * ntask) / ng);
        int lo = 0, hi = NID_NCLS;
        while (hi - lo > 1) {
          const int mid = (lo + hi) >> 1;
          if (s_cts[mid] <= target) lo = mid; else hi = mid;
        }
        bnd = s_cts[lo] + ((target - s_cts[lo]) / NID_ASM_CHUNK) * NID_ASM_CHUNK;
      }
      s_bnd[threadIdx.x] = bnd;
    }
    for (int i = threadIdx.x; i < NID_NCLS * B; i += blockDim.x) {
      const int v = (int)(((unsigned)i * ((1048576u + (unsigned)B - 1u) / (unsigned)B)) >> 20);
      if (s_cts[v + 1] == s_cts[v]) hvs[i] = 0.0;
    }
    __syncthreads();
    const int g = threadIdx.x / tpr, tt = (threadIdx.x % tpr) * (pairs ? 2 : 1);
    double* Gjob = p.G + (size_t)job * p.g_stride * B;
    if (g < ng && s_bnd[g] < s_bnd[g + 1]) {
      int t = s_bnd[g];
      const int tend = s_bnd[g + 1];
      int v;
      {
        int lo = 0, hi = NID_NCLS;
        while (hi - lo > 1) {
          const int mid = (lo + hi) >> 1;
          if (s_cts[mid] <= t) lo = mid; else hi = mid;
        }
        v = lo;
      }
      int cend = s_cts[v + 1];
      bool multi = cend - s_cts[v] > NID_ASM_CHUNK;
      int seg0 = t, nxt = min(cend, seg0 + NID_ASM_CHUNK);
      const double* gp = Gjob + (size_t)t * B + tt;
      double a0 = 0.0, a1 = 0.0;
      auto close_segment = [&]() {
        double* dst = multi ? Gjob + (size_t)seg0 * B + tt : hvs + v * B + tt;
        if (pairs) *reinterpret_cast<double2*>(dst) = make_double2(a0, a1);
        else *dst = a0;
        a0 = 0.0; a1 = 0.0;
      };
      auto next_segment = [&]() {
        seg0 = nxt;
        if (nxt == cend) {
          do v++; while (s_cts[v + 1] == s_cts[v]);
          cend = s_cts[v + 1];
          multi = cend - s_cts[v] > NID_ASM_CHUNK;
        }
        nxt = min(cend, seg0 + NID_ASM_CHUNK);
      };
      if (pairs) {
        while (t < tend) {
          const int rem = tend - t;
          double2 x[8];
#pragma unroll
          for (int i = 0; i < 8; i++) x[i] = (i < rem) ? *reinterpret_cast<const double2*>(gp + i * B) : make_double2(0.0, 0.0);
#pragma unroll
          for (int i = 0; i < 8; i++) {
            if (i < rem) {
              if (t + i >= nxt) { close_segment(); next_segment(); }
              a0 += x[i].x; a1 += x[i].y;
            }
          }
          t += 8;
          gp += 8 * B;
        }
      } else {
        while (t < tend) {
          const int rem = tend - t;
          double x[NID_ASM_BATCH];
#pragma unroll
          for (int i = 0; i < NID_ASM_BATCH; i++) x[i] = (i < rem) ? __ldcs(gp + i * B) : 0.0;
#pragma unroll
          for (int i = 0; i < NID_ASM_BATCH; i++) {
            if (i < rem) {
              if (t + i >= nxt) { close_segment(); next_segment(); }
              a0 += x[i];
            }
          }
          t += NID_ASM_BATCH;
          gp += NID_ASM_BATCH * B;
        }
      }
      close_segment();
    }
    __syncthreads();
    if (g < ng) {
      for (int v = g; v < NID_NCLS; v += ng) {
        const int m = s_cts[v + 1] - s_cts[v];
        if (m <= NID_ASM_CHUNK) continue;
        const int nch = (m + NID_ASM_CHUNK - 1) / NID_ASM_CHUNK;
        const double* gp = Gjob + (size_t)s_cts[v] * B + tt;
        double a0 = 0.0, a1 = 0.0;
        for (int j0 = 0; j0 < nch; j0 += 8) {
          double2 x[8];
#pragma unroll
          for (int i = 0; i < 8; i++) {
            x[i] = make_double2(0.0, 0.0);
            if (j0 + i < nch) {
              const double* q = gp + (size_t)(j0 + i) * NID_ASM_CHUNK * B;
              if (pairs) x[i] = __ldcg(reinterpret_cast<const double2*>(q));
              else x[i].x = __ldcg(q);
            }
          }
#pragma unroll
          for (int i = 0; i < 8; i++)
            if (j0 + i < nch) { a0 += x[i].x; a1 += x[i].y; }
        }
        if (pairs) *reinterpret_cast<double2*>(hvs + v * B + tt) = make_double2(a0, a1);
        else hvs[v * B + tt] = a0;
      }
    }
  }
  __syncthreads();
  {
    const unsigned mdiv = (1048576u + (unsigned)B - 1u) / (unsigned)B;
    for (int item = threadIdx.x; item < 4 * BB; item += blockDim.x) {
      const int kk = item / BB, idx = item - kk * BB;
      {
        const int r = (int)(((unsigned)idx * mdiv) >> 20), tt = idx - r * B;
        const int k = r - kk;
        double a = 0.0;
        if (k >= 0 && k < NS) {
          const int vlo = s_span[k], vhi = s_span[k + 1];
          const double* ph = hvs + vlo * B + tt;
          int n = vhi - vlo;
          if (NID_FEW_BINS(B)) {
            const double* pw = wl + 4 * vlo + kk;
            for (; n >= 4; n -= 4, pw += 16, ph += 4 * B) {
              a = fma(pw[0], ph[0], a); a = fma(pw[4], ph[B], a); a = fma(pw[8], ph[2 * B], a); a = fma(pw[12], ph[3 * B], a);
            }
            for (; n > 0; n--, pw += 4, ph += B) a = fma(pw[0], ph[0], a);
          } else {
            const double* pw = p.lut_w + 4 * vlo + kk;
            for (; n > 0; n--, pw += 4, ph += B) a = fma(__ldg(pw), ph[0], a);
          }
        }
        part[kk * BB + idx] = a;
      }
    }
  }
  const int ngt = max(1, 128 / B);
  if ((int)threadIdx.x < ngt * B) {
    const int g = threadIdx.x / B, tt = threadIdx.x % B;
    double a = 0.0;
    for (int v = g; v < NID_NCLS; v += ngt) a += hvs[v * B + tt];
    red[threadIdx.x] = a;
  }
  __syncthreads();
  for (int idx = threadIdx.x; idx < BB; idx += blockDim.x) {
    const double a = ((part[idx] + part[BB + idx]) + part[2 * BB + idx]) + part[3 * BB + idx];
    const double q = a / (double)nc;
    Pall[idx] = q;
    const double lg = (q < kSigma) ? 0.0 : log2(q);
    part[BB + idx] = -(q * lg);
    part[idx] = (q < kSigma) ? 0.0 : 1.0 + lg;
  }
  if ((int)threadIdx.x >= NT - B) {
    const int tt = threadIdx.x - (NT - B);
    double a = 0.0;
    for (int g = 0; g < ngt; g++) a += red[g * B + tt];
    const double q = a / (double)nc;
    Pall[BB + tt] = q;
    const double lg = (q < kSigma) ? 0.0 : log2(q);
    red[B + tt] = -(q * lg);
    red[tt] = (q < kSigma) ? 0.0 : 1.0 + lg;
  }
  __syncthreads();
  {
    double ej = 0.0, et = 0.0;
    if (threadIdx.x < 128) {
      for (int idx = threadIdx.x; idx < BB; idx += 128) ej += part[BB + idx];
      if (threadIdx.x < 32)
        for (int tt = threadIdx.x; tt < B; tt += 32) et += red[B + tt];
#pragma unroll
      for (int off = 16; off > 0; off >>= 1) {
        ej += __shfl_xor_sync(0xffffffffu, ej, off);
        et += __shfl_xor_sync(0xffffffffu, et, off);
      }
      if ((threadIdx.x & 31) == 0) scratch[threadIdx.x >> 5] = ej;
      if (threadIdx.x == 0) scratch[4] = et;
    }
  }
  __syncthreads();
  const double Hj = ((scratch[0] + scratch[1]) + scratch[2]) + scratch[3];
  const double Ht = scratch[4];
  const double Href = p.href[pair * p.ncell + c];
  if (threadIdx.x == 0) {
    p.ht[o] = Ht; p.hj[o] = Hj;
    p.err[o] = (2 * Hj - Href - Ht) / Hj;
  }
  __syncthreads();
  if (p.hist) for (int i = threadIdx.x; i < BB + B; i += blockDim.x) p.hist[o * (BB + B) + i] = Pall[i];
  if (want_jac) {
    const double s_over = ((double)(B - 3) / 255.0) / ((double)nc * Hj * Hj);
    const double coefJ = -s_over * (Ht + Href);
    const double coefT = s_over * Hj;
    const int BP = wv_row(B);
    const unsigned mdiv = (1048576u + (unsigned)B - 1u) / (unsigned)B;
    double* wv = p.wv + o * (size_t)wv_stride(B);
    for (int i = threadIdx.x; i < BB; i += blockDim.x) {
      const int r = (int)(((unsigned)i * mdiv) >> 20);
      wv[r * BP + (i - r * B)] = part[i] * coefJ;
    }
    if ((int)threadIdx.x < B) wv[B * BP + threadIdx.x] = red[threadIdx.x] * coefT;
  }
}

__global__ void __launch_bounds__(NID_ASM_THREADS, NID_ASM_MINB) k_assemble(EvalParams p, int want_jac) {
  assemble_body<NID_ASM_THREADS>(p, want_jac);
}
__global__ void __launch_bounds__(NID_ASM_SMALL, 2 * NID_ASM_MINB) k_assemble_small(EvalParams p, int want_jac) {
  assemble_body<NID_ASM_SMALL>(p, want_jac);
}
#define NID_ASM_WIDE 1024
__global__ void __launch_bounds__(NID_ASM_WIDE, 1) k_assemble_wide(EvalParams p, int want_jac) {
  assemble_body<NID_ASM_WIDE>(p, want_jac);
}

#define NID_ASMW_WARPS 8
#ifndef NID_ASMW_BATCH
#define NID_ASMW_BATCH 4
#endif
#ifndef NID_ASMW_MINB
#define NID_ASMW_MINB 4
#endif
#ifndef NID_ASMW_BATCH_LAT
#define NID_ASMW_BATCH_LAT 16
#endif
template <int BATCH>
__global__ void __launch_bounds__(NID_ASMW_WARPS * 32, BATCH > 8 ? 1 : NID_ASMW_MINB) k_assemble_warp(EvalParams p, int want_jac, int n_jobs) {
  extern __shared__ __align__(16) double sm[];
  const int B = p.bins, BB = B * B;
  const int lane = threadIdx.x & 31, warp = threadIdx.x >> 5;
  const int unit = blockIdx.x * NID_ASMW_WARPS + warp;
  if (unit >= n_jobs * p.ncell) return;
  const int c = unit % p.ncell, job = job_at(p, unit / p.ncell);
  const int pair = p.job_pair[job];
  const int nc = p.n_c[pair * p.ncell + c];
  const size_t o = (size_t)job * p.ncell + c;
  if (nc < NID_MIN_CELL_POINTS) {
    if (lane == 0) { p.ht[o] = nan(""); p.hj[o] = nan(""); p.err[o] = nan(""); }
    return;
  }
  const int NG = 32 / B;
  const int g = lane / B, t = lane - g * B;
  const bool mine = g < NG;
  const int stride = BB + B;
  double* cp = sm + (size_t)warp * NG * stride;
  for (int i = lane; i < NG * stride; i += 32) cp[i] = 0.0;
  __syncwarp();
  double* Pj = cp + (mine ? g : 0) * stride + t;
  double pt = 0.0;
  double acc[4] = {0.0, 0.0, 0.0, 0.0};
  int cur = -1;
  const int t0 = p.cell_task_start[pair * (p.ncell + 1) + c], t1 = p.cell_task_start[pair * (p.ncell + 1) + c + 1];
  const unsigned short* tcp = p.task_cls + (size_t)pair * p.max_tasks + t0 + g;
  const double* gp = p.G + ((size_t)job * p.g_stride + t0 + g) * B + t;
  const int rstep = NG * B;
  for (int tb = t0; tb < t1; tb += BATCH * NG, tcp += BATCH * NG, gp += BATCH * rstep) {
    double x[BATCH];
    int cls[BATCH];
#pragma unroll
    for (int i = 0; i < BATCH; i++) {
      const bool in = mine && tb + i * NG + g < t1;
      x[i] = in ? __ldcs(gp + i * rstep) : 0.0;
      cls[i] = in ? (int)__ldg(tcp + i * NG) : 256;
    }
#pragma unroll
    for (int i = 0; i < BATCH; i++) {
      pt += x[i];
      if (cls[i] < 256) {
        const int k = __ldg(p.lut_k + cls[i]);
        if (k != cur) {
          if (cur >= 0) {
            double* q = Pj + cur * B;
#pragma unroll
            for (int m = 0; m < 4; m++) { q[m * B] += acc[m]; acc[m] = 0.0; }
          }
          cur = k;
        }
        const double2* w = reinterpret_cast<const double2*>(p.lut_w + 4 * cls[i]);
        const double2 w01 = __ldg(w), w23 = __ldg(w + 1);
        acc[0] = fma(w01.x, x[i], acc[0]); acc[1] = fma(w01.y, x[i], acc[1]);
        acc[2] = fma(w23.x, x[i], acc[2]); acc[3] = fma(w23.y, x[i], acc[3]);
      }
    }
  }
  if (cur >= 0) {
    double* q = Pj + cur * B;
#pragma unroll
    for (int m = 0; m < 4; m++) q[m * B] += acc[m];
  }
  if (mine) cp[g * stride + BB + t] = pt;
  __syncwarp();
  for (int i = lane; i < stride; i += 32) {
    double a = cp[i];
    for (int k = 1; k < NG; k++) a += cp[k * stride + i];
    cp[i] = a;
  }
  __syncwarp();
  double ej = 0.0, et = 0.0;
  const double dn = (double)nc;
  double* hist = p.hist ? p.hist + o * (size_t)(BB + B) : nullptr;
  for (int i = lane; i < stride; i += 32) {
    const double q = cp[i] / dn;
    const double lg = (q < kSigma) ? 0.0 : log2(q);
    if (i < BB) ej -= q * lg; else et -= q * lg;
    cp[i] = (q < kSigma) ? 0.0 : 1.0 + lg;
    if (hist) hist[i] = q;
  }
#pragma unroll
  for (int off = 16; off > 0; off >>= 1) {
    ej += __shfl_xor_sync(0xffffffffu, ej, off);
    et += __shfl_xor_sync(0xffffffffu, et, off);
  }
  const double Hj = ej, Ht = et;
  const double Href = p.href[pair * p.ncell + c];
  if (lane == 0) {
    p.ht[o] = Ht; p.hj[o] = Hj;
    p.err[o] = (2 * Hj - Href - Ht) / Hj;
  }
  __syncwarp();
  if (want_jac) {
    const double s_over = ((double)(B - 3) / 255.0) / ((double)nc * Hj * Hj);
    const double coefJ = -s_over * (Ht + Href);
    const double coefT = s_over * Hj;
    const int BP = wv_row(B);
    const unsigned mdiv = (1048576u + (unsigned)B - 1u) / (unsigned)B;
    double* wv = p.wv + o * (size_t)wv_stride(B);
    for (int i = lane; i < stride; i += 32) {
      const int r = (int)(((unsigned)i * mdiv) >> 20);
      wv[r * BP + (i - r * B)] = cp[i] * (i < BB ? coefJ : coefT);
    }
  }
}

template <bool PTS>
__device__ __noinline__ bool jac_pixel_literal(const double* __restrict__ T1g, const double* __restrict__ T0g,
                                               const double* __restrict__ camg, int rows, int cols,
                                               const uint8_t* __restrict__ im, double a0, double a1, double a2, unsigned id,
                                               double* out6) {
  double e[5];
  exact_uv<PTS>(T1g, T0g, camg, a0, a1, a2, id, e);
  const Cam cam{camg[0], camg[1], camg[2], camg[3]};
  const double u = e[3], v = e[4];
  double u2, v2;
  project_jac(cam, e[0], e[1], e[2], u2, v2);
  if (!inb_cost(u, v, rows, cols) || !inb_jac(u2, v2, rows, cols)) return false;
  const double iz = 1.0 / e[2];
  out6[0] = e[0] * iz; out6[1] = e[1] * iz; out6[2] = iz;
  out6[3] = clamp_intensity(interp_u8(im, cols, u, v));
  out6[4] = interp_u8(im, cols, u2 + 1.0, v2) - interp_u8(im, cols, u2 - 1.0, v2);
  out6[5] = interp_u8(im, cols, u2, v2 + 1.0) - interp_u8(im, cols, u2, v2 - 1.0);
  return true;
}

__device__ __forceinline__ double tapd(unsigned v) { return __hiloint2double(0x43300000, (int)v); }

template <bool PTS, int W, int T>
__device__ __forceinline__ void jac_pixels(const double* __restrict__ g, const ExactSrc& xs, int rows, int cols,
                                           const Group<PTS>& G, int j0, cudaTextureObject_t tex2,
                                           const uint8_t* __restrict__ im1, double s, int NS, double hfx, double hfy,
                                           const double* __restrict__ wq, double acc[6]) {
  Px r[W];
#pragma unroll
  for (int j = 0; j < W; j++) front<PTS, false>(g, rows, cols, G.a0[j0 + j], G.a1[j0 + j], G.a2[j0 + j], G.id[j0 + j], r[j]);
  uint4 t[W];
#pragma unroll
  for (int j = 0; j < W; j++) t[j] = gather_u32(tex2, r[j].ix, r[j].iy);
#pragma unroll
  for (int j = 0; j < W; j++) {
    const double two52 = 4503599627370496.0;
    const double i00 = tapd(t[j].w & 0xffu), i01 = tapd(t[j].z & 0xffu), i10 = tapd(t[j].x & 0xffu), i11 = tapd(t[j].y & 0xffu);
    const double x00 = tapd((t[j].w >> 8) & 0x1ffu), x01 = tapd((t[j].z >> 8) & 0x1ffu);
    const double x10 = tapd((t[j].x >> 8) & 0x1ffu), x11 = tapd((t[j].y >> 8) & 0x1ffu);
    const double y00 = tapd(t[j].w >> 17), y01 = tapd(t[j].z >> 17), y10 = tapd(t[j].x >> 17), y11 = tapd(t[j].y >> 17);
    double ic = bilinear_fast(r[j].dx, r[j].dy, i00 - two52, i01 - i00, i10 - two52, i11 - i10);
    double gx2 = bilinear_fast(r[j].dx, r[j].dy, x00 - (two52 + 256.0), x01 - x00, x10 - (two52 + 256.0), x11 - x10);
    double gy2 = bilinear_fast(r[j].dx, r[j].dy, y00 - (two52 + 256.0), y01 - y00, y10 - (two52 + 256.0), y11 - y10);
    const bool sat = (t[j].w & t[j].z & t[j].x & t[j].y & 0xffu) == 0xffu;
    if (r[j].fix || (r[j].jac && (sat || r[j].ix < 1 || r[j].iy < 1))) {
      double o6[6];
      r[j].jac = jac_pixel_literal<PTS>(xs.T1, xs.T0, xs.cam, rows, cols, im1, G.a0[j0 + j], G.a1[j0 + j], G.a2[j0 + j], G.id[j0 + j], o6);
      if (r[j].jac) {
        r[j].xn = o6[0]; r[j].yn = o6[1]; r[j].rz = o6[2];
        ic = o6[3]; gx2 = o6[4]; gy2 = o6[5];
      }
    }
    const double ub = r[j].jac ? ic * s : 0.0;
    const int k = min((int)ub, NS - 1);
    const double f = ub - u2d((unsigned)k);
    const double dw0 = fma(f, fma(f, -0.5, 1.0), -0.5);
    const double dw1 = f * fma(f, 1.5, -2.0);
    const double dw2 = fma(f, fma(f, -1.5, 1.0), 0.5);
    const double dw3 = 0.5 * f * f;
    const double* q = wq + k * T;
    double ci = fma(dw3, q[3 * T], fma(dw2, q[2 * T], fma(dw1, q[T], dw0 * q[0])));
    if (ub == 0.0) ci = 0.0;
    if (!r[j].jac) continue;
    const double iz = r[j].rz, xn = r[j].xn, yn = r[j].yn;
    const double a = ci * gx2 * hfx, b = ci * gy2 * hfy;
    const double xy = xn * yn;
    acc[0] = fma(-b, fma(yn, yn, 1.0), fma(-a, xy, acc[0]));
    acc[1] = fma(b, xy, fma(a, fma(xn, xn, 1.0), acc[1]));
    acc[2] = fma(b, xn, fma(-a, yn, acc[2]));
    const double aiz = a * iz, biz = b * iz;
    acc[3] += aiz;
    acc[4] += biz;
    acc[5] = fma(-yn, biz, fma(-xn, aiz, acc[5]));
  }
}

template <bool PTS, int NG, int T, bool BULK>
__global__ void __launch_bounds__(T) __maxnreg__(BULK ? NID_JAC_REGS_SMALL : 65536 / (NID_JAC_WARPS * 32))
k_jac_sell(const __grid_constant__ EvalParams p, const __grid_constant__ GeoTable<NG> gt) {
  extern __shared__ __align__(16) double sm[];
  const int B = p.bins, NS = B - 3;
  const int lane = threadIdx.x & 31, warp = threadIdx.x >> 5;
  const int job = gt.job[NID_BLK_JOB], pair = gt.pair[NID_BLK_JOB];
  const double* g = gt.g[NID_BLK_JOB];
  const int slice = NID_BLK_CHUNK * (T >> 5) + warp;
  if (slice >= gt.nsl[NID_BLK_JOB]) return;
  const int* so = p.sl_off + (size_t)pair * (p.max_slices + 1) + slice;
  const int off0 = so[0], ngroups = (so[1] - off0) >> 7;
  const int desc = p.sl_desc[((size_t)pair * p.max_slices + slice) * 32 + lane];
  const int task = desc != 0 ? 0 : -1;
  const bool half_last = (((__shfl_sync(0xffffffffu, desc, 0) & 0x1ff) - 1) & 3) < 2;
  double* wq = sm + threadIdx.x;
  const size_t sbase = (size_t)pair * p.sell_cap + off0 + lane * 4;
  const double* q0 = p.sd0 + sbase;
  const double* q1 = PTS ? p.sd1 + sbase : nullptr;
  const double* q2 = PTS ? p.sd2 + sbase : nullptr;
  const unsigned* qi = p.sid + sbase;
  Group<PTS> G;
  G.load(q0, q1, q2, qi, 0);
  {
    const int cell = p.sl_cell[(size_t)pair * p.max_slices + slice];
    const double* wvg = p.wv + ((size_t)job * p.ncell + cell) * (size_t)wv_stride(B);
    double* Ww = sm + B * T + warp * wv_stride(B);
    unsigned long long* bar = reinterpret_cast<unsigned long long*>(sm + B * T + (T >> 5) * wv_stride(B)) + warp;
    constexpr bool bulk = BULK;
    if (bulk) {
      if (lane == 0) {
        mbar_init(bar, 1);
        asm volatile("fence.mbarrier_init.release.cluster;" ::: "memory");
        mbar_expect_tx(bar, (unsigned)(wv_stride(B) * sizeof(double)));
        bulk_g2s(Ww, wvg, (unsigned)(wv_stride(B) * sizeof(double)), bar);
      }
      __syncwarp();
    }
    const int cls = (desc >> 9) & 0x1ff;
    double wr[4] = {0.0, 0.0, 0.0, 0.0};
    int kr = 0;
    if (task >= 0 && cls < 256) {
      kr = p.lut_k[cls];
#pragma unroll
      for (int kk = 0; kk < 4; kk++) wr[kk] = p.lut_w[4 * cls + kk];
    }
    if (NID_FEW_BINS(B)) {
      const int BP = B + 1;
      const double* Vw = Ww + B * BP;
      if (bulk) {
        mbar_wait(bar, 0u);
      } else {
        for (int i = lane; i < B * BP + B; i += 32) Ww[i] = wvg[i];
        __syncwarp();
      }
      if (task >= 0) {
        const double* Wr = Ww + kr * BP;
        for (int t = 0; t < B; t++) {
          double a = Vw[t];
#pragma unroll
          for (int kk = 0; kk < 4; kk++) a += wr[kk] * Wr[kk * BP + t];
          wq[t * T] = a;
        }
      }
    } else if (task >= 0) {
      const double* Wr = wvg + kr * B;
      for (int t = 0; t < B; t++) {
        double a = __ldg(wvg + B * B + t);
#pragma unroll
        for (int kk = 0; kk < 4; kk++) a += wr[kk] * __ldg(Wr + kk * B + t);
        wq[t * T] = a;
      }
    }
    if (task >= 0) fold_table(wq, T, B);
  }
  const cudaTextureObject_t tex2 = (cudaTextureObject_t)gt.tex[NID_BLK_JOB];
  const uint8_t* im1 = p.im1 + (size_t)pair * p.N;
  const ExactSrc xs{p.poses + 16 * job, p.Twc0 + 16 * pair, p.cam + 4 * pair};
  const double s = (double)NS / 255.0;
  const double hfx = 0.5 * g[16], hfy = 0.5 * g[17];
  double acc[6] = {0, 0, 0, 0, 0, 0};
  for (int gi = 0; gi < ngroups; gi++) {
    Group<PTS> Gn = G;
    if (gi + 1 < ngroups) Gn.load(q0, q1, q2, qi, (size_t)(gi + 1) * 128);
#if NID_PREFETCH_L2 > 0
    if (gi + 1 + NID_PREFETCH_L2 < ngroups) {
      const size_t po = (size_t)(gi + 1 + NID_PREFETCH_L2) * 128;
      asm volatile("prefetch.global.L2 [%0];" ::"l"(q0 + po));
      asm volatile("prefetch.global.L2 [%0];" ::"l"(qi + po));
    }
#endif
#pragma unroll
    for (int j0 = 0; j0 < 4; j0 += NID_JAC_W) {
      if (BULK && j0 >= 2 && half_last && gi + 1 == ngroups) break;
      jac_pixels<PTS, NID_JAC_W, T>(g, xs, p.rows, p.cols, G, j0, tex2, im1, s, NS, hfx, hfy, wq, acc);
    }
    G = Gn;
  }
#pragma unroll
  for (int k = 0; k < 6; k++) {
    double vv = acc[k];
#pragma unroll
    for (int off = 16; off > 0; off >>= 1) vv += __shfl_xor_sync(0xffffffffu, vv, off);
    acc[k] = vv;
  }
  if (lane < 6) {
    double vv = acc[0];
#pragma unroll
    for (int k = 1; k < 6; k++) vv = lane == k ? acc[k] : vv;
    p.jpart[((size_t)job * p.max_slices + slice) * 6 + lane] = vv;
  }
}

__device__ __forceinline__ void jac_tail_cell(const EvalParams& p, int job, int pair, int c, int lane) {
  double* der = p.der + ((size_t)job * p.ncell + c) * 6;
  if (p.n_c[pair * p.ncell + c] < NID_MIN_CELL_POINTS) {
    if (lane < 6) der[lane] = nan("");
    return;
  }
  const int s0 = p.cell_slice_start[pair * (p.ncell + 1) + c];
  const int s1 = p.cell_slice_start[pair * (p.ncell + 1) + c + 1];
  const double* jp = p.jpart + (size_t)job * p.max_slices * 6;
  double acc[6] = {0, 0, 0, 0, 0, 0};
  for (int t = s0 + lane; t < s1; t += 32) {
#pragma unroll
    for (int k = 0; k < 6; k++) acc[k] += jp[(size_t)t * 6 + k];
  }
#pragma unroll
  for (int k = 0; k < 6; k++) {
    double vv = acc[k];
#pragma unroll
    for (int off = 16; off > 0; off >>= 1) vv += __shfl_xor_sync(0xffffffffu, vv, off);
    if (lane == 0) der[k] = vv;
  }
}

__device__ __forceinline__ void jac_tail_entry(const EvalParams& p, int job, int pair, int c, int k) {
  double* der = p.der + ((size_t)job * p.ncell + c) * 6;
  if (p.n_c[pair * p.ncell + c] < NID_MIN_CELL_POINTS) { der[k] = nan(""); return; }
  const int s0 = p.cell_slice_start[pair * (p.ncell + 1) + c];
  const int s1 = p.cell_slice_start[pair * (p.ncell + 1) + c + 1];
  const double* jp = p.jpart + ((size_t)job * p.max_slices + s0) * 6 + k;
  double acc = 0.0;
  int t = s0;
  for (; t + 8 <= s1; t += 8, jp += 48) {
    double v[8];
#pragma unroll
    for (int u = 0; u < 8; u++) v[u] = jp[6 * u];
#pragma unroll
    for (int u = 0; u < 8; u++) acc += v[u];
  }
  for (; t < s1; t++, jp += 6) acc += jp[0];
  der[k] = acc;
}

#define NID_TAIL_PER_THREAD(ncell) ((ncell) >= 64)
__global__ void __launch_bounds__(256) k_jac_final_sorted(EvalParams p, int n_jobs) {
  const int idx = blockIdx.x * blockDim.x + threadIdx.x;
  if (NID_TAIL_PER_THREAD(p.ncell)) {
    if (idx >= n_jobs * p.ncell * 6) return;
    const int k = idx % 6, c = (idx / 6) % p.ncell;
    const int job = job_at(p, idx / (6 * p.ncell));
    jac_tail_entry(p, job, p.job_pair[job], c, k);
  } else {
    const int wid = idx >> 5;
    if (wid >= n_jobs * p.ncell) return;
    const int job = job_at(p, wid / p.ncell), c = wid % p.ncell;
    jac_tail_cell(p, job, p.job_pair[job], c, threadIdx.x & 31);
  }
}
static int jac_final_blocks(const nid_ctx* c, int n) {
  const long long threads = NID_TAIL_PER_THREAD(c->ncell) ? (long long)n * c->ncell * 6 : (long long)n * c->ncell * 32;
  return (int)((threads + 255) / 256);
}

__global__ void __launch_bounds__(128) k_gn_out(EvalParams p, double* __restrict__ gn_out) {
  gn_block(p, job_at(p, blockIdx.x), 1, gn_out);
}

__global__ void __launch_bounds__(256) k_tail_gn(EvalParams p, double* __restrict__ gn_out) {
  const int job = job_at(p, blockIdx.x);
  const int pair = p.job_pair[job];
  for (int c = threadIdx.x >> 5; c < p.ncell; c += blockDim.x >> 5) jac_tail_cell(p, job, pair, c, threadIdx.x & 31);
  __syncthreads();
  gn_block(p, job, 1, gn_out);
}

__global__ void k_pack_k1(int rows, int cols, const uint8_t* __restrict__ im, unsigned short* __restrict__ out) {
  const int N = rows * cols;
  for (int i = blockIdx.x * blockDim.x + threadIdx.x; i < N; i += gridDim.x * blockDim.x) {
    const int y = i / cols, x = i % cols;
    const int xm = max(x - 1, 0), xp = min(x + 1, cols - 1), ym = max(y - 1, 0), yp = min(y + 1, rows - 1);
    const int gx = (int)im[y * cols + xp] - (int)im[y * cols + xm];
    const int gy = (int)im[yp * cols + x] - (int)im[ym * cols + x];
    out[i] = __half_as_ushort(__float2half_rn((float)im[i]));
    out[N + i] = __half_as_ushort(__float2half_rn(0.5f * (float)gx));
    out[2 * N + i] = __half_as_ushort(__float2half_rn(0.5f * (float)gy));
  }
}

#ifndef NID_WS_MINB
#define NID_WS_MINB 8
#endif
template <bool U16>
__device__ __noinline__ unsigned warp_sample_literal(const EvalParams& p, int job, int pair, int i, const double* __restrict__ depth64,
                                                     const uint16_t* __restrict__ depth16, const double* __restrict__ factor_all,
                                                     float* out3) {
  const size_t pbase = (size_t)pair * p.N;
  const double z = U16 ? __dmul_rn((double)depth16[pbase + i], factor_all[pair]) : depth64[pbase + i];
  const int row = i / p.cols, col = i - row * p.cols;
  const unsigned id = ((unsigned)row << 16) | (unsigned)col;
  const double* T1 = p.poses + 16 * job;
  const double* T0 = p.Twc0 + 16 * pair;
  const double* camg = p.cam + 4 * pair;
  double e[5];
  exact_uv<false>(T1, T0, camg, z, 0.0, 0.0, id, e);
  out3[0] = 0.f; out3[1] = 0.f; out3[2] = 0.f;
  if (!inb_cost(e[3], e[4], p.rows, p.cols)) return 0u;
  const uint8_t* im1 = p.im1 + pbase;
  out3[0] = (float)clamp_intensity(interp_u8(im1, p.cols, e[3], e[4]));
  double o6[6];
  if (!jac_pixel_literal<false>(T1, T0, camg, p.rows, p.cols, im1, z, 0.0, 0.0, id, o6)) return 1u;
  out3[1] = (float)o6[4]; out3[2] = (float)o6[5];
  return 3u;
}
#ifndef NID_WS_W
#define NID_WS_W 4
#endif
template <int NG, bool U16>
__global__ void __launch_bounds__(128, NID_WS_MINB)
k_warp_sample_jobs(const __grid_constant__ EvalParams p, const __grid_constant__ GeoTable<NG> gt,
                   const double* __restrict__ depth64, const uint16_t* __restrict__ depth16,
                   const double* __restrict__ factor_all, float4* __restrict__ out) {
  constexpr int W = NID_WS_W;
  const int jb = blockIdx.x, cb_ = blockIdx.y;
  const int job = job_at(p, jb);
  const int pair = p.job_pair[job];
  const double* g = gt.g[jb];
  const int i0 = cb_ * (128 * W) + threadIdx.x;
  const bool full = (cb_ + 1) * (128 * W) <= p.N;
  const size_t pbase = (size_t)pair * p.N;
  double z[W];
  if (U16) {
    const double factor = factor_all[pair];
    unsigned raw[W];
#pragma unroll
    for (int j = 0; j < W; j++) raw[j] = (full || i0 + j * 128 < p.N) ? (unsigned)__ldcs(depth16 + pbase + i0 + j * 128) : 0u;
#pragma unroll
    for (int j = 0; j < W; j++) z[j] = __dmul_rn(u2d(raw[j]), factor);
  } else {
#pragma unroll
    for (int j = 0; j < W; j++) z[j] = (full || i0 + j * 128 < p.N) ? __ldcs(depth64 + pbase + i0 + j * 128) : 0.0;
  }
  int row = i0 / p.cols, col = i0 - row * p.cols;
  double d0, d1, d2;
  {
    const double fc = u2d((unsigned)col), fr = u2d((unsigned)row);
    d0 = fma(g[0], fc, fma(g[3], fr, g[6]));
    d1 = fma(g[1], fc, fma(g[4], fr, g[7]));
    d2 = fma(g[2], fc, fma(g[5], fr, g[8]));
  }
  int jxs[W], jys[W];
  unsigned flags = 0;
  float dxf[W], dyf[W];
  const int c3 = p.cols - 3, r3 = p.rows - 3;
#pragma unroll
  for (int j = 0; j < W; j++) {
    const unsigned valid = (z[j] >= 0.01) & (z[j] <= 100.0);
    const double x1 = fma(z[j], d0, g[9]), y1 = fma(z[j], d1, g[10]), z1 = fma(z[j], d2, g[11]);
    double y;
    asm("rcp.approx.ftz.f64 %0, %1;" : "=d"(y) : "d"(z1));
    y = fma(y, fma(-z1, y, 1.0), y);
    const double u = fma(x1, y, g[18]), v = fma(y1, y, g[19]);
    const int jx = __double2int_rz(u), jy = __double2int_rz(v);
    const double dx = u - u2d((unsigned)jx), dy = v - u2d((unsigned)jy);
    const unsigned band = valid & ((unsigned)jx <= (unsigned)c3) & ((unsigned)jy <= (unsigned)r3);
    const unsigned safe = (unsigned)frac_is_safe(dx) & (unsigned)frac_is_safe(dy);
    const unsigned ok = band & safe & (jx < c3) & (jy < r3);
    const unsigned jac = ok & (jx < c3 - 1);
    const unsigned lit = (band & (safe ^ 1u)) | (ok & ((jx < 1) | (jy < 1)));
    flags |= (ok | (jac << 1) | (lit << 2)) << (4 * j);
    jxs[j] = ok ? jx : 0; jys[j] = ok ? jy : 0;
    dxf[j] = (float)dx; dyf[j] = (float)dy;
    if (j + 1 < W) {
      col += 128;
      d0 += g[12]; d1 += g[13]; d2 += g[14];
      while (col >= p.cols) { col -= p.cols; d0 += g[15]; d1 += g[16]; d2 += g[17]; }
    }
  }
  const cudaTextureObject_t tex = p.k1tex[pair];
  float4* o = out + (size_t)job * p.N + i0;
#pragma unroll
  for (int j = 0; j < W; j++) {
    const float gxc = (float)(jxs[j] + 1), gyc = (float)(jys[j] + 1);
    const float4 I = tex2Dgather<float4>(tex, gxc, gyc, 0);
    const float4 X = tex2Dgather<float4>(tex, gxc, gyc + (float)p.rows, 0);
    const float4 Y = tex2Dgather<float4>(tex, gxc, gyc + (float)(2 * p.rows), 0);
    const float fx_ = dxf[j], fy_ = dyf[j];
    const float w11 = fx_ * fy_, w01 = fx_ - w11, w10 = fy_ - w11, w00 = (1.0f - fx_) - w10;
    float ic = fmaf(w11, I.y, fmaf(w10, I.x, fmaf(w01, I.z, w00 * I.w)));
    float gx = fmaf(w11, X.y, fmaf(w10, X.x, fmaf(w01, X.z, w00 * X.w)));
    float gy = fmaf(w11, Y.y, fmaf(w10, Y.x, fmaf(w01, Y.z, w00 * Y.w)));
    const unsigned f = flags >> (4 * j);
    unsigned vc = f & 1u, vj = (f >> 1) & 1u;
    const unsigned sat = fminf(fminf(I.x, I.y), fminf(I.z, I.w)) == 255.0f;
    if (((f >> 2) | (vc & sat)) & 1u) {
      if (full || i0 + j * 128 < p.N) {
        float r3_[3];
        const unsigned vv = warp_sample_literal<U16>(p, job, pair, i0 + j * 128, depth64, depth16, factor_all, r3_);
        vc = vv & 1u; vj = (vv >> 1) & 1u;
        ic = r3_[0]; gx = 0.5f * r3_[1]; gy = 0.5f * r3_[2];
      }
    }
    ic = vc ? ic : 0.f;
    gx = vj ? gx : 0.f; gy = vj ? gy : 0.f;
    const float fl = vc ? (vj ? 3.f : 1.f) : 0.f;
    if (full || i0 + j * 128 < p.N) __stcs(o + j * 128, make_float4(ic, gx, gy, fl));
  }
}

int launch_count_classes(nid_ctx* c, int pair) {
  EvalParams p = make_params(c, 1);
  int g = (c->N + 255) / 256;
  if (g > c->sm_count * 8) g = c->sm_count * 8;
  k_count_classes<<<g, 256, 0, c->stream>>>(p, pair, c->cnt);
  NID_LAUNCH_CHECK(c, "k_count_classes");
  return NID_OK;
}

int launch_layout_and_scatter(nid_ctx* c, int pair0, int n) {
  EvalParams p = make_params(c, 1);
  const int L = c->task_px;
  const dim3 gcell(c->ncell, n);
  k_layout_totals<<<gcell, NID_LAYOUT_THREADS, 0, c->stream>>>(pair0, c->ncell, L, c->cnt, c->lay_tot);
  NID_LAUNCH_CHECK(c, "k_layout_totals");
  k_layout_scan<<<n, 256, 0, c->stream>>>(p, pair0, c->lay_tot, c->lay_base, c->cell_task_start, c->cell_slice_start, c->ntasks,
                                         c->nslices, c->sl_off, c->d_flag + 1);
  NID_LAUNCH_CHECK(c, "k_layout_scan");
  k_layout_write<<<gcell, NID_LAYOUT_THREADS, 0, c->stream>>>(p, pair0, L, c->cnt, c->lay_base, c->tasks, c->task_pos, c->sl_task,
                                                             c->sl_off, c->sl_cell, c->cls_task_start);
  NID_LAUNCH_CHECK(c, "k_layout_write");
  const size_t sb = (size_t)pair0 * c->sell_cap;
  cudaError_t e = cudaMemsetAsync(c->sid + sb, 0xFF, sizeof(unsigned) * c->sell_cap * n, c->stream);
  if (e != cudaSuccess) return check_cuda(e, "memset sid");
  e = cudaMemsetAsync(c->sd0 + sb, 0, sizeof(double) * c->sell_cap * n, c->stream);
  if (e != cudaSuccess) return check_cuda(e, "memset sd0");
  const int nchunks = (c->rb * c->cb + 255) / 256;
  const dim3 grid(nchunks, c->ncell, n);
  k_chunk_count<<<grid, 256, 0, c->stream>>>(p, pair0, c->chunk_cnt);
  NID_LAUNCH_CHECK(c, "k_chunk_count");
  k_chunk_scan<<<dim3((c->ncell * NID_NCLS + 255) / 256, n), 256, 0, c->stream>>>(c->ncell, nchunks, c->chunk_cnt);
  NID_LAUNCH_CHECK(c, "k_chunk_scan");
  if (c->sell_points) {
    cudaMemsetAsync(c->sd1 + sb, 0, sizeof(double) * c->sell_cap * n, c->stream);
    cudaMemsetAsync(c->sd2 + sb, 0, sizeof(double) * c->sell_cap * n, c->stream);
    k_scatter_sell<true><<<grid, 256, 0, c->stream>>>(p, pair0, L, c->depth, c->task_pos, c->chunk_cnt, c->sd0, c->sd1, c->sd2, c->sid);
  } else {
    k_scatter_sell<false><<<grid, 256, 0, c->stream>>>(p, pair0, L, c->depth, c->task_pos, c->chunk_cnt, c->sd0, nullptr, nullptr, c->sid);
  }
  NID_LAUNCH_CHECK(c, "k_scatter_sell");
  return NID_OK;
}

int launch_pack(nid_ctx* c, int pair0, int n) {
  int g = (c->N + 255) / 256;
  g = std::min(g, std::max(8, c->sm_count * 8 / n));
  k_pack_fp<<<dim3(g, n), 256, 0, c->stream>>>(c->rows, c->cols, pair0, c->im1, c->fp1);
  NID_LAUNCH_CHECK(c, "k_pack_fp");
  k_pack_tex<<<dim3(g, n), 256, 0, c->stream>>>(c->rows, c->cols, pair0, c->im1, c->d_pack);
  NID_LAUNCH_CHECK(c, "k_pack_tex");
  return NID_OK;
}

size_t hist_sell_smem(const nid_ctx* c, int T = 256) { return sizeof(double) * ((size_t)c->bins * T); }
size_t jac_sell_smem(const nid_ctx* c, int T = 128) {
  const size_t B = c->bins;
  return sizeof(double) * (B * T + (NID_FEW_BINS(c->bins) ? (size_t)(T / 32) * (wv_stride(c->bins) + 1) : 0));
}

static int pick_block(const nid_ctx* c, int ns, int n_jobs, int tmax) {
  for (int T = tmax; T > 32; T >>= 1)
    if ((long long)n_jobs * ((ns + T / 32 - 1) / (T / 32)) >= 2LL * c->sm_count) return T;
  return 32;
}
#ifndef NID_ASM_SMALL_PX
#define NID_ASM_SMALL_PX 8192
#endif
static bool assemble_small(const nid_ctx* c) { return (long long)c->rb * c->cb < NID_ASM_SMALL_PX; }
static bool assemble_warp(const nid_ctx* c) { return assemble_small(c) && c->bins <= 32; }
static size_t assemble_warp_smem(const nid_ctx* c) {
  return sizeof(double) * (size_t)NID_ASMW_WARPS * (32 / c->bins) * ((size_t)c->bins * c->bins + c->bins);
}
size_t assemble_smem(const nid_ctx* c, int threads) {
  return sizeof(double) * ((size_t)5 * c->bins * c->bins + c->bins + threads + (size_t)NID_NCLS * c->bins + (NID_FEW_BINS(c->bins) ? 1024 : 0));
}

template <int NG>
static void fill_geo(const nid_ctx* c, GeoTable<NG>& gt, int first, int n, bool pass1, const int* h_list = nullptr) {
  for (int i = 0; i < n; i++) {
    const int job = h_list ? h_list[first + i] : first + i;
    const double* T1 = c->h_poses + 16 * (size_t)job;
    const int pair = c->h_job_pair[job];
    const double* T0 = c->h_Twc0.data() + 16 * (size_t)pair;
    const double* cam = c->h_cam.data() + 4 * (size_t)pair;
    double* g = gt.g[i];
    gt.job[i] = job; gt.pair[i] = pair;
    gt.nsl[i] = c->h_nslices[pair];
    gt.tex[i] = c->h_tex2.empty() ? 0ull : (unsigned long long)c->h_tex2[pair];
    for (int col = 0; col < 4; col++)
      for (int r = 0; r < 3; r++) {
        double m;
        if (c->sell_points) m = T1[4 * col + r];
        else {
          m = T1[r] * T0[4 * col] + T1[4 + r] * T0[4 * col + 1] + T1[8 + r] * T0[4 * col + 2];
          if (col == 3) m += T1[12 + r];
        }
        if (pass1 && r < 2) m *= cam[r];
        g[3 * col + r] = m;
      }
    g[12] = 1.0 / cam[0]; g[13] = -cam[2] / cam[0]; g[14] = 1.0 / cam[1]; g[15] = -cam[3] / cam[1];
    g[16] = cam[0]; g[17] = cam[1]; g[18] = cam[2]; g[19] = cam[3];
  }
}

template <bool PTS, int NG>
static void launch_hist_chunks(nid_ctx* c, const EvalParams& p, int ns, int job0, int n_jobs, const int* h_list) {
  const int T = pick_block(c, ns, n_jobs, c->bins > 20 ? 128 : NID_HIST_TMAX);
  const size_t sm = hist_sell_smem(c, T);
  for (int s0 = 0; s0 < n_jobs; s0 += NG) {
    const int n = std::min(NG, n_jobs - s0);
    GeoTable<NG> gt;
    fill_geo(c, gt, job0 + s0, n, true, h_list);
    EvalParams q = p;
    q.job0 = job0 + s0;
    const dim3 grid = NID_GRID(n, (ns + T / 32 - 1) / (T / 32));
    switch (T) {
      case 256: k_hist_sell<PTS, NG, 256><<<grid, 256, sm, c->stream>>>(q, gt); c->last_hist_func = (const void*)k_hist_sell<PTS, NG, 256>; break;
      case 128: k_hist_sell<PTS, NG, 128><<<grid, 128, sm, c->stream>>>(q, gt); c->last_hist_func = (const void*)k_hist_sell<PTS, NG, 128>; break;
      case 64: k_hist_sell<PTS, NG, 64><<<grid, 64, sm, c->stream>>>(q, gt); c->last_hist_func = (const void*)k_hist_sell<PTS, NG, 64>; break;
      default: k_hist_sell<PTS, NG, 32><<<grid, 32, sm, c->stream>>>(q, gt); c->last_hist_func = (const void*)k_hist_sell<PTS, NG, 32>; break;
    }
    c->launches++;
  }
}
template <bool PTS, int NG>
static void launch_jac_chunks(nid_ctx* c, const EvalParams& p, int ns, int job0, int n_jobs, const int* h_list) {
  const int T = pick_block(c, ns, n_jobs, (long long)c->rb * c->cb < NID_SMALL_CELL_PX ? 32 : NID_JAC_TMAX);
  const size_t sm = jac_sell_smem(c, T);
  for (int s0 = 0; s0 < n_jobs; s0 += NG) {
    const int n = std::min(NG, n_jobs - s0);
    GeoTable<NG> gt;
    fill_geo(c, gt, job0 + s0, n, false, h_list);
    EvalParams q = p;
    q.job0 = job0 + s0;
    const dim3 grid = NID_GRID(n, (ns + T / 32 - 1) / (T / 32));
#define NID_JAC_LAUNCH(TT, BK)                                                 \
  do {                                                                         \
    k_jac_sell<PTS, NG, TT, BK><<<grid, TT, sm, c->stream>>>(q, gt);           \
    c->last_jac_func = (const void*)k_jac_sell<PTS, NG, TT, BK>;               \
  } while (0)
    const bool bulk = q.stage_bulk && NID_FEW_BINS(c->bins);
    switch (T) {
      case 128: if (bulk) NID_JAC_LAUNCH(128, true); else NID_JAC_LAUNCH(128, false); break;
      case 64: if (bulk) NID_JAC_LAUNCH(64, true); else NID_JAC_LAUNCH(64, false); break;
      default: if (bulk) NID_JAC_LAUNCH(32, true); else NID_JAC_LAUNCH(32, false); break;
    }
#undef NID_JAC_LAUNCH
    c->launches++;
  }
}
#define NID_GEO_SMALL 8
#define NID_GEO_LARGE 96
static void launch_hist_w(nid_ctx* c, const EvalParams& p, int ns, int job0, int n_jobs, const int* h_list) {
  if (c->sell_points) {
    if (n_jobs <= NID_GEO_SMALL) launch_hist_chunks<true, NID_GEO_SMALL>(c, p, ns, job0, n_jobs, h_list);
    else launch_hist_chunks<true, NID_GEO_LARGE>(c, p, ns, job0, n_jobs, h_list);
  } else {
    if (n_jobs <= NID_GEO_SMALL) launch_hist_chunks<false, NID_GEO_SMALL>(c, p, ns, job0, n_jobs, h_list);
    else launch_hist_chunks<false, NID_GEO_LARGE>(c, p, ns, job0, n_jobs, h_list);
  }
}
static void launch_jac_w(nid_ctx* c, const EvalParams& p, int ns, int job0, int n_jobs, const int* h_list) {
  if (c->sell_points) {
    if (n_jobs <= NID_GEO_SMALL) launch_jac_chunks<true, NID_GEO_SMALL>(c, p, ns, job0, n_jobs, h_list);
    else launch_jac_chunks<true, NID_GEO_LARGE>(c, p, ns, job0, n_jobs, h_list);
  } else {
    if (n_jobs <= NID_GEO_SMALL) launch_jac_chunks<false, NID_GEO_SMALL>(c, p, ns, job0, n_jobs, h_list);
    else launch_jac_chunks<false, NID_GEO_LARGE>(c, p, ns, job0, n_jobs, h_list);
  }
}

__global__ void k_hist(EvalParams p);
__global__ void k_entropy(EvalParams p);
__global__ void k_jac(EvalParams p);
__global__ void k_jac_final(EvalParams p, int n_jobs);

int launch_pass1(nid_ctx* c, const JobSet& js, Pass2 p2) {
  EvalParams p = make_params(c, js.slots);
  p.job0 = js.first;
  p.job_list = js.d_list;
  const int n = js.n;
  if (!use_sorted(c)) {
    const size_t smem = sizeof(double) * p.hist_stride;
    ktime_mark(c, 0);
    k_hist<<<dim3(p.S, p.ncell, n), 256, smem, c->stream>>>(p);
    NID_LAUNCH_CHECK(c, "k_hist");
    ktime_mark(c, 1);
    if (p2 != Pass2::all) {
      k_entropy<<<dim3(p.ncell, n), 256, smem, c->stream>>>(p);
      NID_LAUNCH_CHECK(c, "k_entropy");
    }
    ktime_mark(c, 2);
    return NID_OK;
  }
  const int tables = p2 != Pass2::none;
  const int ns = c->max_nslices_prepared;
  ktime_mark(c, 0);
  if (ns > 0) {
    launch_hist_w(c, p, ns, js.first, n, js.h_list);
    c->launches--;
    NID_LAUNCH_CHECK(c, "k_hist_sell");
  }
  ktime_mark(c, 1);
  if (assemble_warp(c)) {
    const int units = c->ncell * n;
    if (units <= 2 * c->sm_count * NID_ASMW_WARPS)
      k_assemble_warp<NID_ASMW_BATCH_LAT><<<(units + NID_ASMW_WARPS - 1) / NID_ASMW_WARPS, NID_ASMW_WARPS * 32, assemble_warp_smem(c), c->stream>>>(p, tables, n);
    else
      k_assemble_warp<NID_ASMW_BATCH><<<(units + NID_ASMW_WARPS - 1) / NID_ASMW_WARPS, NID_ASMW_WARPS * 32, assemble_warp_smem(c), c->stream>>>(p, tables, n);
  } else if (c->opt_asm_wide && (c->ncell * n <= c->sm_count || c->opt_asm_wide == 2 ||
                                 (!assemble_small(c) && assemble_smem(c, NID_ASM_THREADS) > (size_t)100 * 1024))) {
    k_assemble_wide<<<dim3(c->ncell, n), NID_ASM_WIDE, assemble_smem(c, NID_ASM_WIDE), c->stream>>>(p, tables);
  } else if (assemble_small(c)) k_assemble_small<<<dim3(c->ncell, n), NID_ASM_SMALL, assemble_smem(c, NID_ASM_THREADS), c->stream>>>(p, tables);
  else k_assemble<<<dim3(c->ncell, n), NID_ASM_THREADS, assemble_smem(c, NID_ASM_THREADS), c->stream>>>(p, tables);
  NID_LAUNCH_CHECK(c, "k_assemble");
  ktime_mark(c, 2);
  return NID_OK;
}

int launch_pass2(nid_ctx* c, const JobSet& js) {
  EvalParams p = make_params(c, js.slots);
  p.job0 = js.first;
  p.job_list = js.d_list;
  const int n = js.n;
  if (!use_sorted(c)) {
    k_jac<<<dim3(p.S, p.ncell, n), 256, sizeof(double) * p.hist_stride, c->stream>>>(p);
    NID_LAUNCH_CHECK(c, "k_jac");
    ktime_mark(c, 3);
    k_jac_final<<<(n * p.ncell * 6 + 255) / 256, 256, 0, c->stream>>>(p, n);
    NID_LAUNCH_CHECK(c, "k_jac_final");
    ktime_mark(c, 4);
    return NID_OK;
  }
  const int ns = c->max_nslices_prepared;
  if (ns > 0) {
    launch_jac_w(c, p, ns, js.first, n, js.h_list);
    c->launches--;
    NID_LAUNCH_CHECK(c, "k_jac_sell");
  }
  ktime_mark(c, 3);
  k_jac_final_sorted<<<jac_final_blocks(c, n), 256, 0, c->stream>>>(p, n);
  NID_LAUNCH_CHECK(c, "k_jac_final_sorted");
  ktime_mark(c, 4);
  return NID_OK;
}

int launch_sorted_tail_gn(nid_ctx* c, const int* d_list, const int* h_list, int first, int n, double delta, double* gn_out) {
  EvalParams p = make_params(c, n);
  p.job0 = first;
  p.job_list = d_list;
  p.huber_delta = delta;
  p.huber_dsqr = (double)(float)(delta * delta);
  const int ns = c->max_nslices_prepared;
  if (ns > 0) {
    launch_jac_w(c, p, ns, first, n, h_list);
    c->launches--;
    NID_LAUNCH_CHECK(c, "k_jac_sell");
  }
  if (c->ncell <= 32) {
    k_tail_gn<<<n, 256, 0, c->stream>>>(p, gn_out);
    NID_LAUNCH_CHECK(c, "k_tail_gn");
  } else {
    k_jac_final_sorted<<<jac_final_blocks(c, n), 256, 0, c->stream>>>(p, n);
    NID_LAUNCH_CHECK(c, "k_jac_final_sorted");
    k_gn_out<<<n, 128, 0, c->stream>>>(p, gn_out);
    NID_LAUNCH_CHECK(c, "k_gn_out");
  }
  return NID_OK;
}

struct LatencyGraph {
  cudaGraph_t graph = nullptr;
  cudaGraphExec_t exec = nullptr;
  cudaGraphNode_t hist_node = nullptr, jac_node = nullptr;
  cudaKernelNodeParams hist_np{}, jac_np{};
  EvalParams hist_q, jac_q;
  EvalParams sig;
  int nslots = 0, ns = 0, task_px = 0;
  size_t h2d_bytes = 0;
  double delta = 0.0;
  const int* d_list = nullptr;
  const double* gn_out = nullptr;
  const void* h_src = nullptr;
  cudaStream_t stream = nullptr;
};

void destroy_latency_graph(nid_ctx* c) {
  LatencyGraph* g = c->lm_graph;
  if (!g) return;
  if (g->exec) cudaGraphExecDestroy(g->exec);
  if (g->graph) cudaGraphDestroy(g->graph);
  delete g;
  c->lm_graph = nullptr;
}

static int capture_latency_graph(nid_ctx* c, LatencyGraph* g, int nslots, const int* d_list, const int* h_list, size_t h2d_bytes,
                                 double delta, double* gn_out) {
  if (g->exec) { cudaGraphExecDestroy(g->exec); g->exec = nullptr; }
  if (g->graph) { cudaGraphDestroy(g->graph); g->graph = nullptr; }
  cudaError_t e = cudaStreamBeginCapture(c->stream, cudaStreamCaptureModeThreadLocal);
  if (e != cudaSuccess) return check_cuda(e, "cudaStreamBeginCapture");
  int r = NID_OK;
  e = cudaMemcpyAsync(c->poses, c->h_poses, h2d_bytes, cudaMemcpyHostToDevice, c->stream);
  if (e != cudaSuccess) r = check_cuda(e, "H2D poses + list (capture)");
  if (r == NID_OK) r = launch_pass1(c, JobSet{d_list, h_list, 0, nslots, nslots}, Pass2::some);
  if (r == NID_OK) r = launch_sorted_tail_gn(c, d_list, h_list, 0, nslots, delta, gn_out);
  e = cudaStreamEndCapture(c->stream, &g->graph);
  if (r != NID_OK) return r;
  if (e != cudaSuccess) return check_cuda(e, "cudaStreamEndCapture");
  size_t nn = 0;
  e = cudaGraphGetNodes(g->graph, nullptr, &nn);
  if (e != cudaSuccess) return check_cuda(e, "cudaGraphGetNodes");
  std::vector<cudaGraphNode_t> nodes(nn);
  e = cudaGraphGetNodes(g->graph, nodes.data(), &nn);
  if (e != cudaSuccess) return check_cuda(e, "cudaGraphGetNodes");
  g->hist_node = g->jac_node = nullptr;
  for (cudaGraphNode_t nd : nodes) {
    cudaGraphNodeType ty;
    if (cudaGraphNodeGetType(nd, &ty) != cudaSuccess || ty != cudaGraphNodeTypeKernel) continue;
    cudaKernelNodeParams np{};
    if (cudaGraphKernelNodeGetParams(nd, &np) != cudaSuccess) continue;
    if (np.func == c->last_hist_func && !g->hist_node) {
      g->hist_node = nd; g->hist_np = np;
      memcpy(&g->hist_q, np.kernelParams[0], sizeof(EvalParams));
    } else if (np.func == c->last_jac_func && !g->jac_node) {
      g->jac_node = nd; g->jac_np = np;
      memcpy(&g->jac_q, np.kernelParams[0], sizeof(EvalParams));
    }
  }
  if (!g->hist_node || !g->jac_node) { set_error("latency graph: pixel-kernel nodes not found"); return NID_ERR_STATE; }
  e = cudaGraphInstantiate(&g->exec, g->graph, 0);
  if (e != cudaSuccess) return check_cuda(e, "cudaGraphInstantiate");
  return NID_OK;
}

int launch_latency_round(nid_ctx* c, int nslots, const int* d_list, const int* h_list, size_t h2d_bytes, double delta, double* gn_out) {
  const int ns = c->max_nslices_prepared;
  const bool graph_ok = c->opt_lm_graph && !c->opt_time_kernels && ns > 0 && nslots <= NID_GEO_SMALL;
  if (!graph_ok) {
    cudaError_t e = cudaMemcpyAsync(c->poses, c->h_poses, h2d_bytes, cudaMemcpyHostToDevice, c->stream);
    if (e != cudaSuccess) return check_cuda(e, "H2D poses + list");
    int r = launch_pass1(c, JobSet{d_list, h_list, 0, nslots, nslots}, Pass2::some);
    if (r != NID_OK) return r;
    return launch_sorted_tail_gn(c, d_list, h_list, 0, nslots, delta, gn_out);
  }
  if (!c->lm_graph) c->lm_graph = new LatencyGraph();
  LatencyGraph* g = c->lm_graph;
  const EvalParams sig = make_params(c, nslots);
  const bool same = g->exec && memcmp(&sig, &g->sig, sizeof(sig)) == 0 && g->nslots == nslots && g->ns == ns && g->task_px == c->task_px &&
                    g->h2d_bytes == h2d_bytes && g->delta == delta && g->d_list == d_list && g->gn_out == gn_out &&
                    g->h_src == (const void*)c->h_poses && g->stream == c->stream;
  if (!same) {
    const int r = capture_latency_graph(c, g, nslots, d_list, h_list, h2d_bytes, delta, gn_out);
    if (r != NID_OK) { destroy_latency_graph(c); return r; }
    g->sig = sig; g->nslots = nslots; g->ns = ns; g->task_px = c->task_px; g->h2d_bytes = h2d_bytes; g->delta = delta;
    g->d_list = d_list; g->gn_out = gn_out; g->h_src = c->h_poses; g->stream = c->stream;
  } else {
    GeoTable<NID_GEO_SMALL> gt;
    for (int pass = 0; pass < 2; pass++) {
      fill_geo(c, gt, 0, nslots, pass == 0, h_list);
      cudaKernelNodeParams np = pass == 0 ? g->hist_np : g->jac_np;
      void* args[2] = {pass == 0 ? (void*)&g->hist_q : (void*)&g->jac_q, (void*)&gt};
      np.kernelParams = args;
      np.extra = nullptr;
      const cudaError_t e = cudaGraphExecKernelNodeSetParams(g->exec, pass == 0 ? g->hist_node : g->jac_node, &np);
      if (e != cudaSuccess) return check_cuda(e, "cudaGraphExecKernelNodeSetParams");
    }
  }
  const cudaError_t e = cudaGraphLaunch(g->exec, c->stream);
  if (e != cudaSuccess) return check_cuda(e, "cudaGraphLaunch");
  c->launches += 4;
  return NID_OK;
}

template <int NG>
static void fill_geo_k1(const nid_ctx* c, GeoTable<NG>& gt, int first, int n) {
  fill_geo(c, gt, first, n, true);
  for (int i = 0; i < n; i++) {
    double* g = gt.g[i];
    const double ifx = g[12], cxo = g[13], ify = g[14], cyo = g[15], cx = g[18], cy = g[19];
    double A[3], B[3], C[3];
    for (int r = 0; r < 3; r++) {
      A[r] = g[r] * ifx;
      B[r] = g[3 + r] * ify;
      C[r] = g[r] * cxo + g[3 + r] * cyo + g[6 + r];
    }
    for (int r = 0; r < 3; r++) {
      g[r] = A[r]; g[3 + r] = B[r]; g[6 + r] = C[r];
      g[12 + r] = 128.0 * A[r];
      g[15 + r] = B[r] - (double)c->cols * A[r];
    }
    g[18] = cx; g[19] = cy;
  }
}

int launch_pack_k1(nid_ctx* c, int pair, unsigned short* d_out) {
  int g = (c->N + 255) / 256;
  if (g > c->sm_count * 8) g = c->sm_count * 8;
  k_pack_k1<<<g, 256, 0, c->stream>>>(c->rows, c->cols, c->im1 + (size_t)pair * c->N, d_out);
  NID_LAUNCH_CHECK(c, "k_pack_k1");
  return NID_OK;
}

int launch_warp_sample_jobs(nid_ctx* c, int n_jobs, float4* d_out, bool u16) {
  EvalParams p = make_params(c, n_jobs);
  const int chunks = (c->N + 128 * NID_WS_W - 1) / (128 * NID_WS_W);
  for (int s0 = 0; s0 < n_jobs; s0 += NID_GEO_LARGE) {
    const int n = std::min(NID_GEO_LARGE, n_jobs - s0);
    GeoTable<NID_GEO_LARGE> gt;
    fill_geo_k1(c, gt, s0, n);
    EvalParams q = p;
    q.job0 = s0;
    const dim3 grid(n, chunks);
    if (u16) k_warp_sample_jobs<NID_GEO_LARGE, true><<<grid, 128, 0, c->stream>>>(q, gt, nullptr, c->depth16, c->depth_factor, d_out);
    else k_warp_sample_jobs<NID_GEO_LARGE, false><<<grid, 128, 0, c->stream>>>(q, gt, c->depth, nullptr, nullptr, d_out);
    NID_LAUNCH_CHECK(c, "k_warp_sample_jobs");
  }
  return NID_OK;
}

int sorted_init(nid_ctx* c) {
  cudaError_t e;
  if (c->bins > NID_SORTED_MAX_BINS || c->bins < NID_SORTED_MIN_BINS) return NID_OK;
#define NID_SMEM_ATTR(k, bytes)                                                                     \
  e = cudaFuncSetAttribute(k, cudaFuncAttributeMaxDynamicSharedMemorySize, (int)(bytes));            \
  if (e != cudaSuccess) return check_cuda(e, "smem attr " #k);
#define NID_CARVE(k, bytes, ctas)                                                                                  \
  {                                                                                                                 \
    const int pct = (int)std::min<size_t>(100, (((bytes) + 1024) * (size_t)(ctas) * 100 + 228 * 1024 - 1) / (228 * 1024)); \
    cudaFuncSetAttribute(k, cudaFuncAttributePreferredSharedMemoryCarveout, pct);                                   \
  }
#define NID_SMEM_ATTR_PX(PTS, NG)                                           \
  NID_SMEM_ATTR((k_hist_sell<PTS, NG, 256>), hist_sell_smem(c, 256));       \
  NID_SMEM_ATTR((k_hist_sell<PTS, NG, 128>), hist_sell_smem(c, 128));       \
  NID_SMEM_ATTR((k_hist_sell<PTS, NG, 64>), hist_sell_smem(c, 64));         \
  NID_SMEM_ATTR((k_hist_sell<PTS, NG, 32>), hist_sell_smem(c, 32));         \
  NID_SMEM_ATTR((k_jac_sell<PTS, NG, 128, false>), jac_sell_smem(c, 128));  \
  NID_SMEM_ATTR((k_jac_sell<PTS, NG, 64, false>), jac_sell_smem(c, 64));    \
  NID_SMEM_ATTR((k_jac_sell<PTS, NG, 32, false>), jac_sell_smem(c, 32));    \
  NID_SMEM_ATTR((k_jac_sell<PTS, NG, 128, true>), jac_sell_smem(c, 128));   \
  NID_SMEM_ATTR((k_jac_sell<PTS, NG, 64, true>), jac_sell_smem(c, 64));     \
  NID_SMEM_ATTR((k_jac_sell<PTS, NG, 32, true>), jac_sell_smem(c, 32));     \
  NID_CARVE((k_hist_sell<PTS, NG, 128>), hist_sell_smem(c, 128), NID_HIST_WARPS / 4);  \
  NID_CARVE((k_hist_sell<PTS, NG, 64>), hist_sell_smem(c, 64), NID_HIST_WARPS / 2);    \
  NID_CARVE((k_hist_sell<PTS, NG, 32>), hist_sell_smem(c, 32), NID_HIST_WARPS);        \
  NID_CARVE((k_jac_sell<PTS, NG, 64, false>), jac_sell_smem(c, 64), NID_JAC_WARPS / 2);  \
  NID_CARVE((k_jac_sell<PTS, NG, 32, false>), jac_sell_smem(c, 32), NID_JAC_WARPS);      \
  NID_CARVE((k_jac_sell<PTS, NG, 64, true>), jac_sell_smem(c, 64), NID_JAC_WARPS_SMALL / 2);   \
  NID_CARVE((k_jac_sell<PTS, NG, 32, true>), jac_sell_smem(c, 32), NID_JAC_WARPS_SMALL);
  NID_SMEM_ATTR_PX(true, NID_GEO_SMALL)
  NID_SMEM_ATTR_PX(false, NID_GEO_SMALL)
  NID_SMEM_ATTR_PX(true, NID_GEO_LARGE)
  NID_SMEM_ATTR_PX(false, NID_GEO_LARGE)
#undef NID_SMEM_ATTR_PX
  NID_SMEM_ATTR(k_assemble, assemble_smem(c, NID_ASM_THREADS));
  NID_SMEM_ATTR(k_assemble_small, assemble_smem(c, NID_ASM_THREADS));
  NID_SMEM_ATTR(k_assemble_wide, assemble_smem(c, NID_ASM_WIDE));
  if (c->bins <= 32) {
    NID_SMEM_ATTR(k_assemble_warp<NID_ASMW_BATCH>, assemble_warp_smem(c));
    NID_SMEM_ATTR(k_assemble_warp<NID_ASMW_BATCH_LAT>, assemble_warp_smem(c));
  }
#undef NID_SMEM_ATTR
  return NID_OK;
}

}
```

Baseline: 151,500.

## Fold per-slice histogram rows into joint partials with FP64 MMA in hist kernel

The histogram kernel no longer scatters per-task bin rows into a global G buffer for the assembly kernels to weight by B-spline LUT coefficients. Each warp now multiplies its slice's bin rows by the per-task weight matrix using FP64 mma.sync m8n8k4 and writes a dense per-slice (B*B+B) partial histogram. The assembly kernels then only sum the slice partials, which drops the class-sorted task scan, the LUT gathers and the shared-memory accumulation. In exchange the hist kernel does more work and the intermediate buffer scales with slices times B^2 rather than tasks times B.

```diff
diff --git a/nid-pose-estimation_b200/csrc/nid_api.cu b/nid-pose-estimation_b200/csrc/nid_api.cu
--- a/nid-pose-estimation_b200/csrc/nid_api.cu
+++ b/nid-pose-estimation_b200/csrc/nid_api.cu
@@ -63,12 +63,12 @@
   p.ht = c->ht; p.hj = c->hj; p.err = c->err; p.der = c->der; p.gn = c->gn;
   p.sd0 = c->sd0; p.sd1 = c->sd1; p.sd2 = c->sd2; p.sid = c->sid;
   p.stage_bulk = (c->opt_stage_bulk < 0 ? (long long)c->rb * c->cb < NID_SMALL_CELL_PX : c->opt_stage_bulk) ? 1 : 0;
-  p.sl_off = c->sl_off; p.sl_task = c->sl_task; p.sl_desc = c->sl_desc; p.task_cls = c->task_cls; p.sl_cell = c->sl_cell; p.nslices = c->nslices;
+  p.sl_off = c->sl_off; p.sl_desc = c->sl_desc; p.sl_cell = c->sl_cell; p.nslices = c->nslices;
   p.sell_cap = c->sell_cap; p.max_slices = c->max_slices; p.Twc0 = c->Twc0;
   p.tasks = c->tasks; p.ntasks = c->ntasks; p.cell_task_start = c->cell_task_start; p.cell_slice_start = c->cell_slice_start;
   p.cls_task_start = c->cls_task_start; p.span_start = c->span_start; p.wv = c->wv;
-  p.max_tasks = c->max_tasks; p.g_stride = (int)c->g_stride;
-  p.G = c->G; p.fp1 = c->fp1; p.tex2 = c->d_tex2; p.k1tex = c->d_k1tex;
+  p.max_tasks = c->max_tasks; p.hpart_slices = (int)c->hpart_slices;
+  p.hpart = c->hpart; p.fp1 = c->fp1; p.tex2 = c->d_tex2; p.k1tex = c->d_k1tex;
   return p;
 }
 
@@ -90,13 +90,13 @@
   const size_t hs = (size_t)c->bins * c->bins + c->bins;
   if (c->opt_keep_hist && !c->hist) OKR(dalloc(&c->hist, J * NC * hs, "hist"));
   if (use_sorted(c)) {
-    const size_t need = (size_t)std::max(c->max_ntasks_prepared, 1);
-    if (c->g_stride < need) {
+    const size_t need = (size_t)std::max(c->max_nslices_prepared, 1);
+    if (c->hpart_slices < need) {
       CU(cudaStreamSynchronize(c->stream), "sync before growing job buffers");
-      if (c->G) cudaFree(c->G);
-      c->G = nullptr;
-      OKR(dalloc(&c->G, J * need * c->bins, "G"));
-      c->g_stride = need;
+      if (c->hpart) cudaFree(c->hpart);
+      c->hpart = nullptr;
+      OKR(dalloc(&c->hpart, J * need * hs, "hpart"));
+      c->hpart_slices = need;
     }
     if (!c->jpart_s) OKR(dalloc(&c->jpart_s, J * (size_t)c->max_slices * 6, "jpart_s"));
     if (!c->wv) {
@@ -236,9 +236,7 @@
   c->sell_cap = (N + 3 * (size_t)c->max_tasks + NC * 32 * (size_t)(NID_TASK_PX_MAX + 4) + 255) / 128 * 128;
   OKR(dalloc(&c->depth, P * N, "depth"));
   OKR(dalloc(&c->sl_off, P * ((size_t)c->max_slices + 1), "sl_off"));
-  OKR(dalloc(&c->sl_task, P * (size_t)c->max_slices * 32, "sl_task"));
   OKR(dalloc(&c->sl_desc, P * (size_t)c->max_slices * 32, "sl_desc"));
-  OKR(dalloc(&c->task_cls, P * (size_t)c->max_tasks, "task_cls"));
   OKR(dalloc(&c->sl_cell, P * (size_t)c->max_slices, "sl_cell"));
   OKR(dalloc(&c->task_pos, P * (size_t)c->max_tasks, "task_pos"));
   OKR(dalloc(&c->nslices, P, "nslices"));
@@ -340,8 +338,8 @@
   void* ptrs[] = {c->pwx, c->pwy, c->pwz, c->im0, c->im1, c->inb0, c->n_c, c->href, c->cam, c->Twc0, c->cnt, c->d_depth,
                   c->d_img64, c->d_flag, c->d_pix, c->d_pix4, c->d_pix4_jobs, c->chunk_cnt, c->d_bsv, c->d_bsi, c->lut_w, c->lut_k, c->poses,
                   c->job_pair, c->aux_pose, c->part, c->jpart, c->hist, c->ht, c->hj, c->err, c->der, c->gn, c->hard,
-                  c->depth, c->sd0, c->sd1, c->sd2, c->sid, c->sl_off, c->sl_task, c->sl_desc, c->task_cls, c->sl_cell, c->nslices, c->task_pos,
-                  c->lay_tot, c->lay_base, c->prep_poses, c->depth16, c->depth_factor, c->d_tex2, c->d_pack, c->tasks, c->ntasks, c->cell_task_start, c->cell_slice_start, c->G, c->jpart_s, c->fp1, c->cls_task_start, c->span_start, c->wv};
+                  c->depth, c->sd0, c->sd1, c->sd2, c->sid, c->sl_off, c->sl_desc, c->sl_cell, c->nslices, c->task_pos,
+                  c->lay_tot, c->lay_base, c->prep_poses, c->depth16, c->depth_factor, c->d_tex2, c->d_pack, c->tasks, c->ntasks, c->cell_task_start, c->cell_slice_start, c->hpart, c->jpart_s, c->fp1, c->cls_task_start, c->span_start, c->wv};
   for (auto t : c->h_k1tex) if (t) cudaDestroyTextureObject(t);
   for (auto arr : c->k1_arrays) if (arr) cudaFreeArray(arr);
   if (c->d_k1tex) cudaFree(c->d_k1tex);
diff --git a/nid-pose-estimation_b200/csrc/nid_ctx.h b/nid-pose-estimation_b200/csrc/nid_ctx.h
--- a/nid-pose-estimation_b200/csrc/nid_ctx.h
+++ b/nid-pose-estimation_b200/csrc/nid_ctx.h
@@ -51,9 +51,7 @@
   const unsigned* sid;
   int stage_bulk;
   const int* sl_off;
-  const int* sl_task;
   const int* sl_desc;
-  const unsigned short* task_cls;
   const int* sl_cell;
   const int* nslices;
   size_t sell_cap;
@@ -67,8 +65,8 @@
   const int* span_start;
   double* wv;
   int max_tasks;
-  int g_stride;
-  double* G;
+  int hpart_slices;
+  double* hpart;
   const unsigned* fp1;
   const cudaTextureObject_t* tex2;
   const cudaTextureObject_t* k1tex;
@@ -112,8 +110,7 @@
   unsigned* sid = nullptr;
   size_t sell_cap = 0;
   int* sl_desc = nullptr;
-  unsigned short* task_cls = nullptr;
-  int *sl_off = nullptr, *sl_task = nullptr, *sl_cell = nullptr, *nslices = nullptr, *task_pos = nullptr;
+  int *sl_off = nullptr, *sl_cell = nullptr, *nslices = nullptr, *task_pos = nullptr;
   int max_slices = 0;
   std::vector<int> h_nslices;
   int max_nslices_prepared = 0;
@@ -129,7 +126,7 @@
   int max_tasks = 0;
   std::vector<int> h_ntasks;
   int max_ntasks_prepared = 0;
-  double *G = nullptr, *jpart_s = nullptr;
+  double *hpart = nullptr, *jpart_s = nullptr;
   std::vector<cudaArray_t> tex2_arrays;
   std::vector<cudaTextureObject_t> h_tex2;
   cudaTextureObject_t* d_tex2 = nullptr;
@@ -141,7 +138,7 @@
   unsigned* fp1 = nullptr;
   std::vector<double> h_Twc0, h_cam;
   unsigned* d_pack = nullptr;
-  size_t g_stride = 0;
+  size_t hpart_slices = 0;
   int opt_path = 0;
   int opt_keep_hist = 0;
   std::vector<char> pair_set, pair_prepared, pair_sorted;
diff --git a/nid-pose-estimation_b200/csrc/nid_sorted.cu b/nid-pose-estimation_b200/csrc/nid_sorted.cu
--- a/nid-pose-estimation_b200/csrc/nid_sorted.cu
+++ b/nid-pose-estimation_b200/csrc/nid_sorted.cu
@@ -261,8 +261,7 @@
 
 __global__ void __launch_bounds__(NID_LAYOUT_THREADS) k_layout_write(EvalParams p, int pair0, int L, const unsigned* __restrict__ cnt,
                                                                      const int* __restrict__ base, int2* __restrict__ tasks,
-                                                                     int* __restrict__ task_pos, int* __restrict__ sl_task,
-                                                                     int* __restrict__ sl_off, int* __restrict__ sl_cell,
+                                                                     int* __restrict__ task_pos, int* __restrict__ sl_off, int* __restrict__ sl_cell,
                                                                      int* __restrict__ cls_task_start) {
   __shared__ CellLayoutSm s;
   const int c = blockIdx.x, pair = pair0 + blockIdx.y;
@@ -274,9 +273,7 @@
     cls_task_start[((size_t)pair * p.ncell + c) * (NID_NCLS + 1) + v] = tb + s.ts[v];
   int2* tk = tasks + (size_t)pair * p.max_tasks + tb;
   int* tp = task_pos + (size_t)pair * p.max_tasks + tb;
-  int* st = sl_task + ((size_t)pair * p.max_slices + sb) * 32;
   int* sd = const_cast<int*>(p.sl_desc) + ((size_t)pair * p.max_slices + sb) * 32;
-  unsigned short* tc = const_cast<unsigned short*>(p.task_cls) + (size_t)pair * p.max_tasks + tb;
   for (int t = threadIdx.x; t < s.T; t += blockDim.x) {
     int lo = 0, hi = NID_NCLS;
     while (hi - lo > 1) {
@@ -291,11 +288,9 @@
     const int off = slice < s.SF ? slice * 32 * L : s.tail_off[slice - s.SF];
     tk[t] = make_int2(i * L, len | (v << 9) | (c << 18));
     tp[t] = pb + off + 4 * ln;
-    st[rank] = tb + t;
     sd[rank] = len | (v << 9) | (c << 18);
-    tc[t] = (unsigned short)v;
-  }
-  for (int q = s.T + threadIdx.x; q < s.S * 32; q += blockDim.x) { st[q] = -1; sd[q] = 0; }
+  }
+  for (int q = s.T + threadIdx.x; q < s.S * 32; q += blockDim.x) sd[q] = 0;
   for (int sl = threadIdx.x; sl < s.S; sl += blockDim.x) {
     sl_off[(size_t)pair * (p.max_slices + 1) + sb + sl] = pb + (sl < s.SF ? sl * 32 * L : s.tail_off[sl - s.SF]);
     sl_cell[(size_t)pair * p.max_slices + sb + sl] = c;
@@ -599,47 +594,85 @@
   }
 }
 
-template <int T>
-__device__ __forceinline__ void store_task_rows(double* hw, int B, int lane, int task, double* __restrict__ Gj, size_t gstride) {
+#define NID_HROW 32
+
+__device__ __forceinline__ void dmma_f64(double& d0, double& d1, double a, double b) {
+  asm volatile("mma.sync.aligned.m8n8k4.row.col.f64.f64.f64.f64 {%0,%1}, {%2}, {%3}, {%0,%1};" : "+d"(d0), "+d"(d1) : "d"(a), "d"(b));
+}
+template <int RT, int TC>
+__device__ __forceinline__ void slice_partial_tiles(double* hw, int B, int lane, int krl, double2 wl01, double2 wl23, double vl,
+                                                    double* __restrict__ out) {
+  const int q = lane & 3, rr = lane >> 2;
+  for (int t0 = 0; t0 < B; t0 += 8 * TC) {
+    double acc[RT][TC][2];
+#pragma unroll
+    for (int rt = 0; rt < RT; rt++)
+#pragma unroll
+      for (int tc = 0; tc < TC; tc++) { acc[rt][tc][0] = 0.0; acc[rt][tc][1] = 0.0; }
+    const double* hp[TC];
+    int rot[TC];
+#pragma unroll
+    for (int tc = 0; tc < TC; tc++) {
+      const int t = min(t0 + 8 * tc + rr, B - 1);
+      hp[tc] = hw + t * NID_HROW;
+      rot[tc] = 4 * (t & 7);
+    }
+#pragma unroll 2
+    for (int ks = 0; ks < 8; ks++) {
+      const int j = 4 * ks + q;
+      double bv[TC];
+#pragma unroll
+      for (int tc = 0; tc < TC; tc++) bv[tc] = hp[tc][(j + rot[tc]) & 31];
+      const int kr = __shfl_sync(0xffffffffu, krl, j);
+      const double w0 = __shfl_sync(0xffffffffu, wl01.x, j), w1 = __shfl_sync(0xffffffffu, wl01.y, j);
+      const double w2 = __shfl_sync(0xffffffffu, wl23.x, j), w3 = __shfl_sync(0xffffffffu, wl23.y, j);
+      const double v = __shfl_sync(0xffffffffu, vl, j);
+#pragma unroll
+      for (int rt = 0; rt < RT; rt++) {
+        const int r = 8 * rt + rr, m = r - kr;
+        double a = m == 0 ? w0 : (m == 1 ? w1 : (m == 2 ? w2 : (m == 3 ? w3 : 0.0)));
+        a = r == B ? v : (r > B ? 0.0 : a);
+#pragma unroll
+        for (int tc = 0; tc < TC; tc++) dmma_f64(acc[rt][tc][0], acc[rt][tc][1], a, bv[tc]);
+      }
+    }
+#pragma unroll
+    for (int rt = 0; rt < RT; rt++)
+#pragma unroll
+      for (int tc = 0; tc < TC; tc++)
+#pragma unroll
+        for (int i = 0; i < 2; i++) {
+          const int r = 8 * rt + rr, t = t0 + 8 * tc + 2 * q + i;
+          if (r <= B && t < B) out[r * B + t] = acc[rt][tc][i];
+        }
+  }
+}
+__device__ __forceinline__ void slice_partial(double* hw, int B, int lane, int desc, const int* __restrict__ lut_k,
+                                              const double* __restrict__ lut_w, double* __restrict__ out) {
+  const int cls = (desc >> 9) & 0x1ff;
+  const bool ref = desc != 0 && cls < 256;
+  const int krl = ref ? __ldg(lut_k + cls) : -8;
+  const double2 wl01 = ref ? __ldg(reinterpret_cast<const double2*>(lut_w) + 2 * cls) : make_double2(0.0, 0.0);
+  const double2 wl23 = ref ? __ldg(reinterpret_cast<const double2*>(lut_w) + 2 * cls + 1) : make_double2(0.0, 0.0);
+  const double vl = desc != 0 ? 1.0 : 0.0;
   for (int b0 = 0; b0 < B; b0 += 8) {
     double v[8];
 #pragma unroll
-    for (int i = 0; i < 8; i++) v[i] = (b0 + i < B) ? hw[(b0 + i) * T + lane] : 0.0;
+    for (int i = 0; i < 8; i++) v[i] = (b0 + i < B) ? hw[(b0 + i) * NID_HROW + lane] : 0.0;
     __syncwarp();
 #pragma unroll
     for (int i = 0; i < 8; i++)
-      if (b0 + i < B) hw[(b0 + i) * T + ((lane + b0 + i) & 31)] = v[i];
+      if (b0 + i < B) hw[(b0 + i) * NID_HROW + ((lane + 4 * ((b0 + i) & 7)) & 31)] = v[i];
   }
   __syncwarp();
-  const int BP2 = B <= 8 ? 8 : (B <= 16 ? 16 : 32);
-  const int rpi = 32 / BP2;
-  const int b = lane & (BP2 - 1), sub = lane / BP2;
-  {
-    const double* src = hw + min(b, B - 1) * T;
-    double* dst = Gj + b;
-    const int nit = 32 / rpi;
-    for (int i0 = 0; i0 < nit; i0 += 8) {
-      double v[8];
-      int tk[8];
-#pragma unroll
-      for (int i = 0; i < 8; i++) {
-        const int tl = (i0 + i) * rpi + sub;
-        tk[i] = __shfl_sync(0xffffffffu, task, tl);
-        v[i] = src[(tl + b) & 31];
-      }
-#pragma unroll
-      for (int i = 0; i < 8; i++)
-        if (b < B && tk[i] >= 0) dst[(size_t)tk[i] * gstride] = v[i];
-    }
-  }
-  for (int b1 = BP2; b1 < B; b1 += BP2) {
-    for (int t0 = 0; t0 < 32; t0 += rpi) {
-      const int tl = t0 + sub, bb = b1 + b;
-      const int tk = __shfl_sync(0xffffffffu, task, tl);
-      if (bb < B && tk >= 0) Gj[(size_t)tk * gstride + bb] = hw[bb * T + ((tl + bb) & 31)];
-    }
-  }
-  __syncwarp();
+  switch ((B + 8) >> 3) {
+    case 1: slice_partial_tiles<1, 1>(hw, B, lane, krl, wl01, wl23, vl, out); break;
+    case 2: slice_partial_tiles<2, 2>(hw, B, lane, krl, wl01, wl23, vl, out); break;
+    case 3: slice_partial_tiles<3, 2>(hw, B, lane, krl, wl01, wl23, vl, out); break;
+    case 4: slice_partial_tiles<4, 2>(hw, B, lane, krl, wl01, wl23, vl, out); break;
+    case 5: slice_partial_tiles<5, 2>(hw, B, lane, krl, wl01, wl23, vl, out); break;
+    default: slice_partial_tiles<6, 2>(hw, B, lane, krl, wl01, wl23, vl, out); break;
+  }
 }
 
 #ifndef NID_HIST_W
@@ -683,9 +716,10 @@
   if (slice >= p.nslices[pair]) return;
   const int* so = p.sl_off + (size_t)pair * (p.max_slices + 1) + slice;
   const int off0 = so[0], ngroups = (so[1] - off0) >> 7;
-  const int task = p.sl_task[((size_t)pair * p.max_slices + slice) * 32 + lane];
-  double* h = sm + threadIdx.x;
-  for (int b = 0; b < B; b++) h[b * T] = 0.0;
+  const int desc = p.sl_desc[((size_t)pair * p.max_slices + slice) * 32 + lane];
+  double* hw = sm + (size_t)warp * NID_HROW * B;
+  double* h = hw + lane;
+  for (int b = 0; b < B; b++) h[b * NID_HROW] = 0.0;
   const size_t sbase = (size_t)pair * p.sell_cap + off0 + lane * 4;
   const double* q0 = p.sd0 + sbase;
   const double* q1 = PTS ? p.sd1 + sbase : nullptr;
@@ -710,40 +744,43 @@
     const size_t go = (size_t)gi * 128;
     const GroupAddr ga{q0 + go, PTS ? q1 + go : nullptr, PTS ? q2 + go : nullptr, qi + go};
 #pragma unroll
-    for (int j0 = 0; j0 < 4; j0 += NID_HIST_W) hist_pixels<PTS, NID_HIST_W, T>(g, xs, p.rows, p.cols, G, j0, ga, fp, s, NS, h, n0);
+    for (int j0 = 0; j0 < 4; j0 += NID_HIST_W) hist_pixels<PTS, NID_HIST_W, NID_HROW>(g, xs, p.rows, p.cols, G, j0, ga, fp, s, NS, h, n0);
     G = Gn;
   }
-  fold_row(h, T, B, (double)n0);
+  fold_row(h, NID_HROW, B, (double)n0);
   __syncwarp();
-  store_task_rows<T>(sm + (threadIdx.x & ~31), B, lane, task, p.G + (size_t)job * p.g_stride * B, B);
+  slice_partial(hw, B, lane, desc, p.lut_k, p.lut_w, p.hpart + ((size_t)job * p.hpart_slices + slice) * (size_t)(B * B + B));
 }
 
 #ifndef NID_ASM_THREADS
 #define NID_ASM_THREADS 256
 #endif
-#define NID_ASM_SMALL 128
-#ifndef NID_ASM_BATCH
-#define NID_ASM_BATCH 12
-#endif
-#ifndef NID_ASM_CHUNK
-#define NID_ASM_CHUNK 16
-#endif
+#define NID_ASM_INFLIGHT 8
 #ifndef NID_ASM_MINB
 #define NID_ASM_MINB 4
 #endif
+template <int INFLIGHT>
+__device__ __forceinline__ double sum_slices(const double* __restrict__ src, int E, int ns) {
+  double a = 0.0;
+  int s = 0;
+  for (; s + INFLIGHT <= ns; s += INFLIGHT, src += (size_t)INFLIGHT * E) {
+    double v[INFLIGHT];
+#pragma unroll
+    for (int u = 0; u < INFLIGHT; u++) v[u] = __ldcs(src + (size_t)u * E);
+#pragma unroll
+    for (int u = 0; u < INFLIGHT; u++) a += v[u];
+  }
+  for (; s < ns; s++, src += E) a += __ldcs(src);
+  return a;
+}
 template <int NT>
 __device__ __forceinline__ void assemble_body(const EvalParams& p, int want_jac) {
   extern __shared__ __align__(16) double sm[];
   __shared__ double scratch[8];
-  __shared__ int s_cts[NID_NCLS + 1];
-  __shared__ int s_bnd[NT / 3 + 2];
-  __shared__ int s_span[NID_SORTED_MAX_BINS];
-  const int B = p.bins, BB = B * B, NS = B - 3;
+  const int B = p.bins, BB = B * B, E = BB + B;
   double* Pall = sm;
-  double* red = sm + BB + B;
-  double* hvs = red + NT;
-  double* part = hvs + NID_NCLS * B;
-  double* wl = part + 4 * BB;
+  double* ent = sm + E;
+  double* tab = ent + E;
   const int c = blockIdx.x, job = job_at(p, blockIdx.y);
   const int pair = p.job_pair[job];
   const int nc = p.n_c[pair * p.ncell + c];
@@ -753,191 +790,23 @@
     return;
   }
   {
-    const int* cts = p.cls_task_start + ((size_t)pair * p.ncell + c) * (NID_NCLS + 1);
-    for (int i = threadIdx.x; i <= NID_NCLS; i += blockDim.x) s_cts[i] = cts[i];
-    for (int i = threadIdx.x; i <= NS; i += blockDim.x) s_span[i] = p.span_start[i];
-    if (NID_FEW_BINS(B)) for (int i = threadIdx.x; i < 1024; i += blockDim.x) wl[i] = p.lut_w[i];
-    __syncthreads();
-    const bool pairs = (B & 1) == 0;
-    const int tpr = pairs ? B >> 1 : B;
-    const int ng = NT / tpr;
-    const int tfirst = s_cts[0], tlast = s_cts[NID_NCLS], ntask = tlast - tfirst;
-    if ((int)threadIdx.x <= ng) {
-      int bnd = tlast;
-      if ((int)threadIdx.x < ng) {
-        const int target = tfirst + (int)(((long long)threadIdx.x * ntask) / ng);
-        int lo = 0, hi = NID_NCLS;
-        while (hi - lo > 1) {
-          const int mid = (lo + hi) >> 1;
-          if (s_cts[mid] <= target) lo = mid; else hi = mid;
-        }
-        bnd = s_cts[lo] + ((target - s_cts[lo]) / NID_ASM_CHUNK) * NID_ASM_CHUNK;
-      }
-      s_bnd[threadIdx.x] = bnd;
-    }
-    for (int i = threadIdx.x; i < NID_NCLS * B; i += blockDim.x) {
-      const int v = (int)(((unsigned)i * ((1048576u + (unsigned)B - 1u) / (unsigned)B)) >> 20);
-      if (s_cts[v + 1] == s_cts[v]) hvs[i] = 0.0;
-    }
-    __syncthreads();
-    const int g = threadIdx.x / tpr, tt = (threadIdx.x % tpr) * (pairs ? 2 : 1);
-    double* Gjob = p.G + (size_t)job * p.g_stride * B;
-    if (g < ng && s_bnd[g] < s_bnd[g + 1]) {
-      int t = s_bnd[g];
-      const int tend = s_bnd[g + 1];
-      int v;
-      {
-        int lo = 0, hi = NID_NCLS;
-        while (hi - lo > 1) {
-          const int mid = (lo + hi) >> 1;
-          if (s_cts[mid] <= t) lo = mid; else hi = mid;
-        }
-        v = lo;
-      }
-      int cend = s_cts[v + 1];
-      bool multi = cend - s_cts[v] > NID_ASM_CHUNK;
-      int seg0 = t, nxt = min(cend, seg0 + NID_ASM_CHUNK);
-      const double* gp = Gjob + (size_t)t * B + tt;
-      double a0 = 0.0, a1 = 0.0;
-      auto close_segment = [&]() {
-        double* dst = multi ? Gjob + (size_t)seg0 * B + tt : hvs + v * B + tt;
-        if (pairs) *reinterpret_cast<double2*>(dst) = make_double2(a0, a1);
-        else *dst = a0;
-        a0 = 0.0; a1 = 0.0;
-      };
-      auto next_segment = [&]() {
-        seg0 = nxt;
-        if (nxt == cend) {
-          do v++; while (s_cts[v + 1] == s_cts[v]);
-          cend = s_cts[v + 1];
-          multi = cend - s_cts[v] > NID_ASM_CHUNK;
-        }
-        nxt = min(cend, seg0 + NID_ASM_CHUNK);
-      };
-      if (pairs) {
-        while (t < tend) {
-          const int rem = tend - t;
-          double2 x[8];
-#pragma unroll
-          for (int i = 0; i < 8; i++) x[i] = (i < rem) ? *reinterpret_cast<const double2*>(gp + i * B) : make_double2(0.0, 0.0);
-#pragma unroll
-          for (int i = 0; i < 8; i++) {
-            if (i < rem) {
-              if (t + i >= nxt) { close_segment(); next_segment(); }
-              a0 += x[i].x; a1 += x[i].y;
-            }
-          }
-          t += 8;
-          gp += 8 * B;
-        }
-      } else {
-        while (t < tend) {
-          const int rem = tend - t;
-          double x[NID_ASM_BATCH];
-#pragma unroll
-          for (int i = 0; i < NID_ASM_BATCH; i++) x[i] = (i < rem) ? __ldcs(gp + i * B) : 0.0;
-#pragma unroll
-          for (int i = 0; i < NID_ASM_BATCH; i++) {
-            if (i < rem) {
-              if (t + i >= nxt) { close_segment(); next_segment(); }
-              a0 += x[i];
-            }
-          }
-          t += NID_ASM_BATCH;
-          gp += NID_ASM_BATCH * B;
-        }
-      }
-      close_segment();
-    }
-    __syncthreads();
-    if (g < ng) {
-      for (int v = g; v < NID_NCLS; v += ng) {
-        const int m = s_cts[v + 1] - s_cts[v];
-        if (m <= NID_ASM_CHUNK) continue;
-        const int nch = (m + NID_ASM_CHUNK - 1) / NID_ASM_CHUNK;
-        const double* gp = Gjob + (size_t)s_cts[v] * B + tt;
-        double a0 = 0.0, a1 = 0.0;
-        for (int j0 = 0; j0 < nch; j0 += 8) {
-          double2 x[8];
-#pragma unroll
-          for (int i = 0; i < 8; i++) {
-            x[i] = make_double2(0.0, 0.0);
-            if (j0 + i < nch) {
-              const double* q = gp + (size_t)(j0 + i) * NID_ASM_CHUNK * B;
-              if (pairs) x[i] = __ldcg(reinterpret_cast<const double2*>(q));
-              else x[i].x = __ldcg(q);
-            }
-          }
-#pragma unroll
-          for (int i = 0; i < 8; i++)
-            if (j0 + i < nch) { a0 += x[i].x; a1 += x[i].y; }
-        }
-        if (pairs) *reinterpret_cast<double2*>(hvs + v * B + tt) = make_double2(a0, a1);
-        else hvs[v * B + tt] = a0;
-      }
-    }
-  }
-  __syncthreads();
-  {
-    const unsigned mdiv = (1048576u + (unsigned)B - 1u) / (unsigned)B;
-    for (int item = threadIdx.x; item < 4 * BB; item += blockDim.x) {
-      const int kk = item / BB, idx = item - kk * BB;
-      {
-        const int r = (int)(((unsigned)idx * mdiv) >> 20), tt = idx - r * B;
-        const int k = r - kk;
-        double a = 0.0;
-        if (k >= 0 && k < NS) {
-          const int vlo = s_span[k], vhi = s_span[k + 1];
-          const double* ph = hvs + vlo * B + tt;
-          int n = vhi - vlo;
-          if (NID_FEW_BINS(B)) {
-            const double* pw = wl + 4 * vlo + kk;
-            for (; n >= 4; n -= 4, pw += 16, ph += 4 * B) {
-              a = fma(pw[0], ph[0], a); a = fma(pw[4], ph[B], a); a = fma(pw[8], ph[2 * B], a); a = fma(pw[12], ph[3 * B], a);
-            }
-            for (; n > 0; n--, pw += 4, ph += B) a = fma(pw[0], ph[0], a);
-          } else {
-            const double* pw = p.lut_w + 4 * vlo + kk;
-            for (; n > 0; n--, pw += 4, ph += B) a = fma(__ldg(pw), ph[0], a);
-          }
-        }
-        part[kk * BB + idx] = a;
-      }
-    }
-  }
-  const int ngt = max(1, 128 / B);
-  if ((int)threadIdx.x < ngt * B) {
-    const int g = threadIdx.x / B, tt = threadIdx.x % B;
-    double a = 0.0;
-    for (int v = g; v < NID_NCLS; v += ngt) a += hvs[v * B + tt];
-    red[threadIdx.x] = a;
-  }
-  __syncthreads();
-  for (int idx = threadIdx.x; idx < BB; idx += blockDim.x) {
-    const double a = ((part[idx] + part[BB + idx]) + part[2 * BB + idx]) + part[3 * BB + idx];
-    const double q = a / (double)nc;
-    Pall[idx] = q;
-    const double lg = (q < kSigma) ? 0.0 : log2(q);
-    part[BB + idx] = -(q * lg);
-    part[idx] = (q < kSigma) ? 0.0 : 1.0 + lg;
-  }
-  if ((int)threadIdx.x >= NT - B) {
-    const int tt = threadIdx.x - (NT - B);
-    double a = 0.0;
-    for (int g = 0; g < ngt; g++) a += red[g * B + tt];
-    const double q = a / (double)nc;
-    Pall[BB + tt] = q;
-    const double lg = (q < kSigma) ? 0.0 : log2(q);
-    red[B + tt] = -(q * lg);
-    red[tt] = (q < kSigma) ? 0.0 : 1.0 + lg;
+    const int s0 = p.cell_slice_start[pair * (p.ncell + 1) + c], s1 = p.cell_slice_start[pair * (p.ncell + 1) + c + 1];
+    const double* src = p.hpart + ((size_t)job * p.hpart_slices + s0) * E;
+    for (int i = threadIdx.x; i < E; i += NT) {
+      const double q = sum_slices<NID_ASM_INFLIGHT>(src + i, E, s1 - s0) / (double)nc;
+      Pall[i] = q;
+      const double lg = (q < kSigma) ? 0.0 : log2(q);
+      ent[i] = -(q * lg);
+      tab[i] = (q < kSigma) ? 0.0 : 1.0 + lg;
+    }
   }
   __syncthreads();
   {
     double ej = 0.0, et = 0.0;
     if (threadIdx.x < 128) {
-      for (int idx = threadIdx.x; idx < BB; idx += 128) ej += part[BB + idx];
+      for (int idx = threadIdx.x; idx < BB; idx += 128) ej += ent[idx];
       if (threadIdx.x < 32)
-        for (int tt = threadIdx.x; tt < B; tt += 32) et += red[B + tt];
+        for (int tt = threadIdx.x; tt < B; tt += 32) et += ent[BB + tt];
 #pragma unroll
       for (int off = 16; off > 0; off >>= 1) {
         ej += __shfl_xor_sync(0xffffffffu, ej, off);
@@ -955,8 +824,7 @@
     p.ht[o] = Ht; p.hj[o] = Hj;
     p.err[o] = (2 * Hj - Href - Ht) / Hj;
   }
-  __syncthreads();
-  if (p.hist) for (int i = threadIdx.x; i < BB + B; i += blockDim.x) p.hist[o * (BB + B) + i] = Pall[i];
+  if (p.hist) for (int i = threadIdx.x; i < E; i += blockDim.x) p.hist[o * E + i] = Pall[i];
   if (want_jac) {
     const double s_over = ((double)(B - 3) / 255.0) / ((double)nc * Hj * Hj);
     const double coefJ = -s_over * (Ht + Href);
@@ -964,19 +832,15 @@
     const int BP = wv_row(B);
     const unsigned mdiv = (1048576u + (unsigned)B - 1u) / (unsigned)B;
     double* wv = p.wv + o * (size_t)wv_stride(B);
-    for (int i = threadIdx.x; i < BB; i += blockDim.x) {
+    for (int i = threadIdx.x; i < E; i += blockDim.x) {
       const int r = (int)(((unsigned)i * mdiv) >> 20);
-      wv[r * BP + (i - r * B)] = part[i] * coefJ;
-    }
-    if ((int)threadIdx.x < B) wv[B * BP + threadIdx.x] = red[threadIdx.x] * coefT;
+      wv[r * BP + (i - r * B)] = tab[i] * (i < BB ? coefJ : coefT);
+    }
   }
 }
 
 __global__ void __launch_bounds__(NID_ASM_THREADS, NID_ASM_MINB) k_assemble(EvalParams p, int want_jac) {
   assemble_body<NID_ASM_THREADS>(p, want_jac);
-}
-__global__ void __launch_bounds__(NID_ASM_SMALL, 2 * NID_ASM_MINB) k_assemble_small(EvalParams p, int want_jac) {
-  assemble_body<NID_ASM_SMALL>(p, want_jac);
 }
 #define NID_ASM_WIDE 1024
 __global__ void __launch_bounds__(NID_ASM_WIDE, 1) k_assemble_wide(EvalParams p, int want_jac) {
@@ -996,7 +860,7 @@
 template <int BATCH>
 __global__ void __launch_bounds__(NID_ASMW_WARPS * 32, BATCH > 8 ? 1 : NID_ASMW_MINB) k_assemble_warp(EvalParams p, int want_jac, int n_jobs) {
   extern __shared__ __align__(16) double sm[];
-  const int B = p.bins, BB = B * B;
+  const int B = p.bins, BB = B * B, E = BB + B;
   const int lane = threadIdx.x & 31, warp = threadIdx.x >> 5;
   const int unit = blockIdx.x * NID_ASMW_WARPS + warp;
   if (unit >= n_jobs * p.ncell) return;
@@ -1008,72 +872,20 @@
     if (lane == 0) { p.ht[o] = nan(""); p.hj[o] = nan(""); p.err[o] = nan(""); }
     return;
   }
-  const int NG = 32 / B;
-  const int g = lane / B, t = lane - g * B;
-  const bool mine = g < NG;
-  const int stride = BB + B;
-  double* cp = sm + (size_t)warp * NG * stride;
-  for (int i = lane; i < NG * stride; i += 32) cp[i] = 0.0;
-  __syncwarp();
-  double* Pj = cp + (mine ? g : 0) * stride + t;
-  double pt = 0.0;
-  double acc[4] = {0.0, 0.0, 0.0, 0.0};
-  int cur = -1;
-  const int t0 = p.cell_task_start[pair * (p.ncell + 1) + c], t1 = p.cell_task_start[pair * (p.ncell + 1) + c + 1];
-  const unsigned short* tcp = p.task_cls + (size_t)pair * p.max_tasks + t0 + g;
-  const double* gp = p.G + ((size_t)job * p.g_stride + t0 + g) * B + t;
-  const int rstep = NG * B;
-  for (int tb = t0; tb < t1; tb += BATCH * NG, tcp += BATCH * NG, gp += BATCH * rstep) {
-    double x[BATCH];
-    int cls[BATCH];
-#pragma unroll
-    for (int i = 0; i < BATCH; i++) {
-      const bool in = mine && tb + i * NG + g < t1;
-      x[i] = in ? __ldcs(gp + i * rstep) : 0.0;
-      cls[i] = in ? (int)__ldg(tcp + i * NG) : 256;
-    }
-#pragma unroll
-    for (int i = 0; i < BATCH; i++) {
-      pt += x[i];
-      if (cls[i] < 256) {
-        const int k = __ldg(p.lut_k + cls[i]);
-        if (k != cur) {
-          if (cur >= 0) {
-            double* q = Pj + cur * B;
-#pragma unroll
-            for (int m = 0; m < 4; m++) { q[m * B] += acc[m]; acc[m] = 0.0; }
-          }
-          cur = k;
-        }
-        const double2* w = reinterpret_cast<const double2*>(p.lut_w + 4 * cls[i]);
-        const double2 w01 = __ldg(w), w23 = __ldg(w + 1);
-        acc[0] = fma(w01.x, x[i], acc[0]); acc[1] = fma(w01.y, x[i], acc[1]);
-        acc[2] = fma(w23.x, x[i], acc[2]); acc[3] = fma(w23.y, x[i], acc[3]);
-      }
-    }
-  }
-  if (cur >= 0) {
-    double* q = Pj + cur * B;
-#pragma unroll
-    for (int m = 0; m < 4; m++) q[m * B] += acc[m];
-  }
-  if (mine) cp[g * stride + BB + t] = pt;
-  __syncwarp();
-  for (int i = lane; i < stride; i += 32) {
-    double a = cp[i];
-    for (int k = 1; k < NG; k++) a += cp[k * stride + i];
-    cp[i] = a;
-  }
-  __syncwarp();
+  const int s0 = p.cell_slice_start[pair * (p.ncell + 1) + c], s1 = p.cell_slice_start[pair * (p.ncell + 1) + c + 1];
+  const double* src = p.hpart + ((size_t)job * p.hpart_slices + s0) * E;
   double ej = 0.0, et = 0.0;
   const double dn = (double)nc;
-  double* hist = p.hist ? p.hist + o * (size_t)(BB + B) : nullptr;
-  for (int i = lane; i < stride; i += 32) {
-    const double q = cp[i] / dn;
-    const double lg = (q < kSigma) ? 0.0 : log2(q);
-    if (i < BB) ej -= q * lg; else et -= q * lg;
-    cp[i] = (q < kSigma) ? 0.0 : 1.0 + lg;
-    if (hist) hist[i] = q;
+  double* hist = p.hist ? p.hist + o * (size_t)E : nullptr;
+  double* tab = sm + (size_t)warp * E;
+  for (int i = lane; i < E; i += 32) {
+    {
+      const double q = sum_slices<BATCH>(src + i, E, s1 - s0) / dn;
+      const double lg = (q < kSigma) ? 0.0 : log2(q);
+      if (i < BB) ej -= q * lg; else et -= q * lg;
+      tab[i] = (q < kSigma) ? 0.0 : 1.0 + lg;
+      if (hist) hist[i] = q;
+    }
   }
 #pragma unroll
   for (int off = 16; off > 0; off >>= 1) {
@@ -1086,7 +898,6 @@
     p.ht[o] = Ht; p.hj[o] = Hj;
     p.err[o] = (2 * Hj - Href - Ht) / Hj;
   }
-  __syncwarp();
   if (want_jac) {
     const double s_over = ((double)(B - 3) / 255.0) / ((double)nc * Hj * Hj);
     const double coefJ = -s_over * (Ht + Href);
@@ -1094,9 +905,9 @@
     const int BP = wv_row(B);
     const unsigned mdiv = (1048576u + (unsigned)B - 1u) / (unsigned)B;
     double* wv = p.wv + o * (size_t)wv_stride(B);
-    for (int i = lane; i < stride; i += 32) {
+    for (int i = lane; i < E; i += 32) {
       const int r = (int)(((unsigned)i * mdiv) >> 20);
-      wv[r * BP + (i - r * B)] = cp[i] * (i < BB ? coefJ : coefT);
+      wv[r * BP + (i - r * B)] = tab[i] * (i < BB ? coefJ : coefT);
     }
   }
 }
@@ -1515,8 +1326,8 @@
   k_layout_scan<<<n, 256, 0, c->stream>>>(p, pair0, c->lay_tot, c->lay_base, c->cell_task_start, c->cell_slice_start, c->ntasks,
                                          c->nslices, c->sl_off, c->d_flag + 1);
   NID_LAUNCH_CHECK(c, "k_layout_scan");
-  k_layout_write<<<gcell, NID_LAYOUT_THREADS, 0, c->stream>>>(p, pair0, L, c->cnt, c->lay_base, c->tasks, c->task_pos, c->sl_task,
-                                                             c->sl_off, c->sl_cell, c->cls_task_start);
+  k_layout_write<<<gcell, NID_LAYOUT_THREADS, 0, c->stream>>>(p, pair0, L, c->cnt, c->lay_base, c->tasks, c->task_pos, c->sl_off,
+                                                              c->sl_cell, c->cls_task_start);
   NID_LAUNCH_CHECK(c, "k_layout_write");
   const size_t sb = (size_t)pair0 * c->sell_cap;
   cudaError_t e = cudaMemsetAsync(c->sid + sb, 0xFF, sizeof(unsigned) * c->sell_cap * n, c->stream);
@@ -1550,7 +1361,7 @@
   return NID_OK;
 }
 
-size_t hist_sell_smem(const nid_ctx* c, int T = 256) { return sizeof(double) * ((size_t)c->bins * T); }
+size_t hist_sell_smem(const nid_ctx* c, int T = 256) { return sizeof(double) * ((size_t)c->bins * NID_HROW * (T / 32)); }
 size_t jac_sell_smem(const nid_ctx* c, int T = 128) {
   const size_t B = c->bins;
   return sizeof(double) * (B * T + (NID_FEW_BINS(c->bins) ? (size_t)(T / 32) * (wv_stride(c->bins) + 1) : 0));
@@ -1567,11 +1378,9 @@
 static bool assemble_small(const nid_ctx* c) { return (long long)c->rb * c->cb < NID_ASM_SMALL_PX; }
 static bool assemble_warp(const nid_ctx* c) { return assemble_small(c) && c->bins <= 32; }
 static size_t assemble_warp_smem(const nid_ctx* c) {
-  return sizeof(double) * (size_t)NID_ASMW_WARPS * (32 / c->bins) * ((size_t)c->bins * c->bins + c->bins);
-}
-size_t assemble_smem(const nid_ctx* c, int threads) {
-  return sizeof(double) * ((size_t)5 * c->bins * c->bins + c->bins + threads + (size_t)NID_NCLS * c->bins + (NID_FEW_BINS(c->bins) ? 1024 : 0));
-}
+  return sizeof(double) * (size_t)NID_ASMW_WARPS * ((size_t)c->bins * c->bins + c->bins);
+}
+size_t assemble_smem(const nid_ctx* c) { return sizeof(double) * 3 * ((size_t)c->bins * c->bins + c->bins); }
 
 template <int NG>
 static void fill_geo(const nid_ctx* c, GeoTable<NG>& gt, int first, int n, bool pass1, const int* h_list = nullptr) {
@@ -1706,11 +1515,9 @@
       k_assemble_warp<NID_ASMW_BATCH_LAT><<<(units + NID_ASMW_WARPS - 1) / NID_ASMW_WARPS, NID_ASMW_WARPS * 32, assemble_warp_smem(c), c->stream>>>(p, tables, n);
     else
       k_assemble_warp<NID_ASMW_BATCH><<<(units + NID_ASMW_WARPS - 1) / NID_ASMW_WARPS, NID_ASMW_WARPS * 32, assemble_warp_smem(c), c->stream>>>(p, tables, n);
-  } else if (c->opt_asm_wide && (c->ncell * n <= c->sm_count || c->opt_asm_wide == 2 ||
-                                 (!assemble_small(c) && assemble_smem(c, NID_ASM_THREADS) > (size_t)100 * 1024))) {
-    k_assemble_wide<<<dim3(c->ncell, n), NID_ASM_WIDE, assemble_smem(c, NID_ASM_WIDE), c->stream>>>(p, tables);
-  } else if (assemble_small(c)) k_assemble_small<<<dim3(c->ncell, n), NID_ASM_SMALL, assemble_smem(c, NID_ASM_THREADS), c->stream>>>(p, tables);
-  else k_assemble<<<dim3(c->ncell, n), NID_ASM_THREADS, assemble_smem(c, NID_ASM_THREADS), c->stream>>>(p, tables);
+  } else if (c->opt_asm_wide && (c->ncell * n <= c->sm_count || c->opt_asm_wide == 2)) {
+    k_assemble_wide<<<dim3(c->ncell, n), NID_ASM_WIDE, assemble_smem(c), c->stream>>>(p, tables);
+  } else k_assemble<<<dim3(c->ncell, n), NID_ASM_THREADS, assemble_smem(c), c->stream>>>(p, tables);
   NID_LAUNCH_CHECK(c, "k_assemble");
   ktime_mark(c, 2);
   return NID_OK;
@@ -1951,9 +1758,8 @@
   NID_SMEM_ATTR_PX(true, NID_GEO_LARGE)
   NID_SMEM_ATTR_PX(false, NID_GEO_LARGE)
 #undef NID_SMEM_ATTR_PX
-  NID_SMEM_ATTR(k_assemble, assemble_smem(c, NID_ASM_THREADS));
-  NID_SMEM_ATTR(k_assemble_small, assemble_smem(c, NID_ASM_THREADS));
-  NID_SMEM_ATTR(k_assemble_wide, assemble_smem(c, NID_ASM_WIDE));
+  NID_SMEM_ATTR(k_assemble, assemble_smem(c));
+  NID_SMEM_ATTR(k_assemble_wide, assemble_smem(c));
   if (c->bins <= 32) {
     NID_SMEM_ATTR(k_assemble_warp<NID_ASMW_BATCH>, assemble_warp_smem(c));
     NID_SMEM_ATTR(k_assemble_warp<NID_ASMW_BATCH_LAT>, assemble_warp_smem(c));
```

Result: no change. 152,200 (median of 6 runs) (+0.5%).
